# zouyunkai/MedicalSemSeg

Measured on AMD Instinct MI355X. Metric: 96^3 vols/sec fwd+bwd (train), higher is better.
Workload: dtype bf16; 1 GPU; UNet base (MONAI BasicUNet 32-32-64-128-256-32) 1->3cls, 96^3 patches, DiceCE + AdamW, per-GPU batch 2; global_batch=2, parallelism=dp1, grad_sync=none (single rank)

## Files before the change

### include/msseg.h

```cpp
#ifndef MSSEG_H_
#define MSSEG_H_

#include <stddef.h>
#include <stdint.h>

#ifdef __cplusplus
extern "C" {
#endif

#define MSSEG_ABI_VERSION 1

#define MSSEG_OK 0
#define MSSEG_EINVAL (-1)
#define MSSEG_ELAUNCH (-2)
#define MSSEG_EWORKSPACE (-3)

#define MSSEG_F32 0
#define MSSEG_BF16 1

typedef void* msseg_stream_t;

int msseg_abi_version(void);
const char* msseg_last_error(void);
int msseg_num_cus(void);

int msseg_ktimer_enable(int on);
int msseg_ktimer_reset(void);
int msseg_ktimer_count(void);
int msseg_ktimer_get(int i, char* name, int cap, float* ms);

size_t msseg_packed_weight_bytes(int M, int T, int K, int cout_block, int dtype);
int msseg_pack_weights(const float* src, void* dst, int dtype, int M, int M0, int T, int K, int K0,
                       long long s_m1, long long s_m0, long long s_t, long long s_k1, long long s_k0,
                       int flip, int cout_block, msseg_stream_t stream);
typedef struct msseg_pack_job {
    const float* src;
    void* dst;
    long long s_m1, s_m0, s_t, s_k1, s_k0;
    long long total;
    int M, M0, T, K, K0, flip, cout_block, nkb;
} msseg_pack_job;
int msseg_pack_weights_batch(const msseg_pack_job* jobs_dev, int njobs, long long max_total, long long sum_total, int dtype,
                             msseg_stream_t stream);
int msseg_cout_block(int M);
int msseg_conv3d_k3_cout_block(int N, int D, int H, int W, int Cout);
int msseg_conv3d_k3_variant(int N, int D, int H, int W, int Cout);
int msseg_conv3d_k3_kernel(int N, int D, int H, int W, int Cin, int Cout, int dtype);

int msseg_conv3d_k3_fwd(const void* x, long long ldx, const void* wp, const float* bias, void* y, long long ldy,
                        int N, int D, int H, int W, int Cin, int Cout, float* stats ,
                        void* scratch, size_t scratch_bytes, int dtype, msseg_stream_t stream);
int msseg_conv3d_k3_fwd_accumulate(const void* x, long long ldx, const void* wp, void* y, long long ldy, int N, int D, int H,
                                   int W, int Cin, int Cout, float* stats, void* scratch, size_t scratch_bytes, int dtype,
                                   msseg_stream_t stream);
int msseg_conv3d_k3_dgrad_inbwd(const void* dy, long long lddy, const void* wp, void* da, long long ldda, int N, int D,
                                int H, int W, int Cin, int Cout, const void* yraw, long long ldyraw, const void* act,
                                long long ldact, const float* fwd_stats, float slope, float eps, float* red,
                                float* dgamma, float* dbeta, int accumulate, void* scratch, size_t scratch_bytes,
                                int dtype, msseg_stream_t stream);
int msseg_conv3d_k3s2_fwd(const void* x, long long ldx, const void* wp, const float* bias, void* y, long long ldy,
                          int N, int ID, int IH, int IW, int Cin, int Cout, int dtype, msseg_stream_t stream);
int msseg_zero_stuff2(const void* dy, long long lddy, void* out, long long ldo, int N, int OD, int OH, int OW, int ID,
                      int IH, int IW, int C, int dtype, msseg_stream_t stream);
int msseg_conv3d_stem_fwd(const void* x, long long ldx, const void* wp, const float* bias, void* y, long long ldy,
                          int N, int D, int H, int W, int Cout, float* stats, void* scratch, size_t scratch_bytes,
                          int dtype, msseg_stream_t stream);
int msseg_conv3d_stem_k1_fwd(const void* x, long long ldx, const void* wp, const float* bias, void* y, long long ldy,
                             int N, int D, int H, int W, int Cout, float* stats, void* scratch, size_t scratch_bytes,
                             int dtype, msseg_stream_t stream);
int msseg_conv3d_stem_norm_fwd(const void* x, long long ldx, const void* wp, const float* bias, const float* stats,
                               const float* gamma, const float* beta, float eps, float slope, void* y, long long ldy, int N,
                               int D, int H, int W, int Cout, int dtype, msseg_stream_t stream);
int msseg_conv3d_k1_fwd(const void* x, long long ldx, const void* wp, const float* bias, void* y, long long ldy,
                        long long NV, int Cin, int Cout, int dtype, msseg_stream_t stream);
int msseg_conv3d_k1_head_fwd(const void* x, long long ldx, const float* w, const float* bias, void* y, long long ldy,
                             long long NV, int Cin, int Cout, int dtype, msseg_stream_t stream);
int msseg_conv3d_k1_head_dgrad_inbwd(const void* dy, long long lddy, const float* w, void* da, long long ldda, int N,
                                     long long S, int C, int Cout, const void* yraw, long long ldyraw,
                                     const float* fwd_stats, const float* gamma, const float* beta, float slope, float eps,
                                     float* red, float* dgamma, float* dbeta, int accumulate, void* scratch,
                                     size_t scratch_bytes, int dtype, msseg_stream_t stream);
int msseg_conv3d_k1_head_norm_fwd(const void* x, long long ldx, const float* stats, const float* gamma, const float* beta,
                                  float slope, float eps, const float* w, const float* bias, void* y, long long ldy, int N,
                                  long long S, int Cin, int Cout, int dtype, msseg_stream_t stream);
int msseg_conv3d_k1_head_bwd_fused(const void* dy, long long lddy, const float* w, void* da, long long ldda, int N,
                                   long long S, int C, int Cout, const void* yraw, long long ldyraw, const float* fwd_stats,
                                   const float* gamma, const float* beta, float slope, float eps, float* red, float* dgamma,
                                   float* dbeta, int accumulate, float* dw, int dw_accumulate, void* scratch,
                                   size_t scratch_bytes, int dtype, msseg_stream_t stream);

int msseg_conv3d_gather_fwd(const void* x, long long ldx, const void* wp, const float* bias, void* y, long long ldy,
                            int N, int ID, int IH, int IW, int Cin, int Cout, int k, int s, int p, int dtype,
                            msseg_stream_t stream);
int msseg_deconv_k2s2_fwd(const void* x, long long ldx, const void* wp, const float* bias, void* y, long long ldy,
                          int N, int D, int H, int W, int Cin, int Cout, int dtype, msseg_stream_t stream);
int msseg_deconv_k2s2_bwd_data(const void* dy, long long lddy, const void* wp, void* dx, long long lddx,
                               int N, int D, int H, int W, int Cin, int Cout, int dtype, msseg_stream_t stream);
int msseg_deconv_k4s4_fwd(const void* x, long long ldx, const void* wp, const float* bias, void* y, long long ldy,
                          int N, int D, int H, int W, int Cin, int Cout, int dtype, msseg_stream_t stream);
int msseg_deconv_k4s4_bwd_data(const void* dy, long long lddy, const void* wp, void* dx, long long lddx,
                               int N, int D, int H, int W, int Cin, int Cout, int dtype, msseg_stream_t stream);
int msseg_conv3d_k1_dgrad_inbwd(const void* dy, long long lddy, const void* wp, void* da, long long ldda, int N,
                                long long S, int Cin, int Cout, const void* yraw, long long ldyraw, const void* act,
                                long long ldact, const float* fwd_stats, float slope, float eps, float* red,
                                float* dgamma, float* dbeta, int accumulate, void* scratch, size_t scratch_bytes,
                                int dtype, msseg_stream_t stream);
int msseg_deconv_k2s2_bwd_data_inbwd(const void* dy, long long lddy, const void* wp, void* dx, long long lddx, int N,
                                     int D, int H, int W, int Cin, int Cout, const void* yraw, long long ldyraw,
                                     const void* act, long long ldact, const float* fwd_stats, float slope, float eps,
                                     float* red, float* dgamma, float* dbeta, int accumulate, void* scratch,
                                     size_t scratch_bytes, int dtype, msseg_stream_t stream);
int msseg_deconv_k2s2_bwd_fused(const void* dy, long long lddy, const void* wp, void* dx, long long lddx, int N,
                                int D, int H, int W, int Cin, int Cout, const void* yraw, long long ldyraw,
                                const void* act, long long ldact, const float* fwd_stats, float slope, float eps,
                                float* red, float* dgamma, float* dbeta, int accumulate, float* dbias, int dbias_accumulate,
                                void* scratch, size_t scratch_bytes, int dtype, msseg_stream_t stream);

int msseg_deconv_k2s2_bwd_partials_ok(int Cin, int Cout, int dtype);
int msseg_deconv_k2s2_bwd_partials(const void* dy, long long lddy, const void* wp, float* part, size_t part_bytes, int N,
                                   int D, int H, int W, int Cin, int Cout, int dtype, msseg_stream_t stream);


size_t msseg_wgrad_workspace_bytes(int M, int T, int K);
int msseg_conv3d_k3_wgrad_kernel(int N, int D, int H, int W, int Cin, int Cout, int dtype);
int msseg_conv3d_k3_wgrad(const void* x, long long ldx, const void* dy, long long lddy, float* dw,
                          int N, int D, int H, int W, int Cin, int Cout, int accumulate,
                          void* workspace, size_t workspace_bytes, int dtype, msseg_stream_t stream);
int msseg_conv3d_k1_wgrad(const void* x, long long ldx, const void* dy, long long lddy, float* dw,
                          long long NV, int Cin, int Cout, int accumulate,
                          void* workspace, size_t workspace_bytes, int dtype, msseg_stream_t stream);
int msseg_linear_wgrad_ok(long long NV, int Cin, int Cout, int dtype);
int msseg_linear_wgrad(const void* x, long long ldx, const void* dy, long long lddy, float* dw, float* dbias, long long NV,
                       int Cin, int Cout, int accumulate_w, int accumulate_b, void* workspace, size_t workspace_bytes,
                       int dtype, msseg_stream_t stream);
int msseg_conv3d_gather_wgrad(const void* x, long long ldx, const void* dy, long long lddy, float* dw,
                              int N, int ID, int IH, int IW, int Cin, int Cout, int k, int s, int p, int accumulate,
                              void* workspace, size_t workspace_bytes, int dtype, msseg_stream_t stream);
int msseg_deconv_k2s2_wgrad(const void* x, long long ldx, const void* dy, long long lddy, float* dw,
                            int N, int D, int H, int W, int Cin, int Cout, int accumulate,
                            void* workspace, size_t workspace_bytes, int dtype, msseg_stream_t stream);
int msseg_deconv_k4s4_wgrad(const void* x, long long ldx, const void* dy, long long lddy, float* dw,
                            int N, int D, int H, int W, int Cin, int Cout, int accumulate,
                            void* workspace, size_t workspace_bytes, int dtype, msseg_stream_t stream);

int msseg_conv3d_k3_small_ok(int N, int D, int H, int W, int Cin, int Cout, int dtype);
int msseg_conv3d_k3_small_stage_groups(int N, int D, int H, int W, int Cin, int Cout);
size_t msseg_conv3d_k3_small_workspace_bytes(int N, int D, int H, int W, int Cin, int Cout);
int msseg_conv3d_k3_small_partials(const void* x, long long ldx, const void* wp, float* part, size_t part_bytes, int N,
                                   int D, int H, int W, int Cin, int Cout, msseg_stream_t stream);
int msseg_conv3d_k3_small_fwd_finish(const float* part, int nstages, const float* bias, const float* gamma,
                                     const float* beta, float eps, float slope, void* yraw, long long ldy, void* act,
                                     long long lda, void* pooled, long long ldp, float* stats, int N, int D, int H, int W,
                                     int Cout, msseg_stream_t stream);
int msseg_conv3d_k3_small_fwd_finish_res(const float* part, int nstages, const float* bias, const float* gamma,
                                         const float* beta, float eps, float slope, void* yraw, long long ldy, void* act,
                                         long long lda, const void* residual, long long ldr, void* pooled, long long ldp,
                                         float* stats, int N, int D, int H, int W, int Cout, msseg_stream_t stream);
int msseg_conv3d_k3_small_bwd_finish(const float* part, int nstages, void* dx, long long lddx, const void* unit_yraw,
                                     long long lduy, const float* unit_stats, const float* unit_gamma,
                                     const float* unit_beta, float eps, float slope, float* dgamma, float* dbeta,
                                     int accumulate, int N, int D, int H, int W, int Cin, msseg_stream_t stream);

int msseg_dwconv3d_k3_fwd(const void* x, long long ldx, const void* w_taps, const float* bias, void* y, long long ldy, int N,
                          int D, int H, int W, int C, int flip, int dtype, msseg_stream_t stream);
int msseg_avgpool3d_k3(const void* x, long long ldx, void* y, long long ldy, int N, int D, int H, int W, int C, int dtype,
                       msseg_stream_t stream);
int msseg_dwconv3d_k3_wgrad(const void* x, long long ldx, const void* dy, long long lddy, float* dw, float* dbias,
                            int accumulate_w, int accumulate_b, int N, int D, int H, int W, int C, void* scratch,
                            size_t scratch_bytes, int dtype, msseg_stream_t stream);

int msseg_interp_trilinear_fwd(const void* x, long long ldx, void* y, long long ldy, int N, int ID, int IH, int IW, int OD,
                               int OH, int OW, int C, int dtype, msseg_stream_t stream);
size_t msseg_interp_trilinear_bwd_workspace_bytes(int N, int ID, int IH, int IW, int OD, int OH, int OW, int C);
int msseg_interp_trilinear_bwd(const void* dy, long long lddy, void* dx, long long lddx, int N, int ID, int IH, int IW, int OD,
                               int OH, int OW, int C, void* workspace, size_t workspace_bytes, int dtype, msseg_stream_t stream);
int msseg_kv_attention_fwd(const void* q, const void* kv, void* o, float* lse, int B, int N, int M, int heads, int head_dim,
                           float scale, int dtype, msseg_stream_t stream);
size_t msseg_kv_attention_bwd_workspace_bytes(int B, int N, int M, int heads, int head_dim);
int msseg_kv_attention_bwd(const void* q, const void* kv, const void* o, const float* lse, const void* dout, void* dq, void* dkv,
                           int B, int N, int M, int heads, int head_dim, float scale, void* workspace, size_t workspace_bytes,
                           int dtype, msseg_stream_t stream);
int msseg_scale_channels(const void* x, const float* scale, void* y, int N, long long S, int C, int dtype, msseg_stream_t stream);

size_t msseg_reduce_scratch_bytes(void);
int msseg_channel_stats(const void* x, long long ldx, float* stats, int N, long long S, int C, void* scratch,
                        size_t scratch_bytes, int dtype, msseg_stream_t stream);
int msseg_instnorm_act_fwd(const void* x, long long ldx, const float* stats, const float* gamma, const float* beta,
                           const void* residual, long long ldr, void* y, long long ldy, int N, long long S, int C,
                           float eps, float slope, int dtype, msseg_stream_t stream);
int msseg_instnorm_act_pool_fwd(const void* x, long long ldx, const float* stats, const float* gamma, const float* beta,
                                void* y, long long ldy, void* pooled, long long ldp, int N, int D, int H, int W, int C,
                                float eps, float slope, int dtype, msseg_stream_t stream);
int msseg_instnorm_act_poolbwd_reduce(const void* x, long long ldx, const float* stats, const float* gamma,
                                      const float* beta, const void* skip, long long lds, const void* g, long long ldg,
                                      void* da, long long ldda, float* red, float* dgamma, float* dbeta, int accumulate,
                                      int N, int D, int H, int W, int C, float eps, float slope, void* scratch,
                                      size_t scratch_bytes, int dtype, msseg_stream_t stream);
int msseg_instnorm_act_bwd_reduce(const void* x, long long ldx, const float* stats, const float* gamma,
                                  const float* beta, const void* y, long long ldy,
                                  const void* dy, long long lddy, float* red, float* dgamma, float* dbeta,
                                  int accumulate, int N, long long S, int C, float eps, float slope, void* scratch,
                                  size_t scratch_bytes, int dtype, msseg_stream_t stream);
int msseg_instnorm_act_bwd_apply(const void* x, long long ldx, const float* stats, const float* gamma,
                                 const float* beta, const void* y, long long ldy, const void* dy, long long lddy, const float* red, void* dx,
                                 long long lddx, void* dres, long long lddres, int N, long long S, int C, float eps,
                                 float slope, int dtype, msseg_stream_t stream);
int msseg_maxpool2_fwd(const void* x, long long ldx, void* y, long long ldy, int N, int D, int H, int W, int C,
                       int dtype, msseg_stream_t stream);
int msseg_maxpool2_bwd(const void* x, long long ldx, const void* dy, long long lddy, void* dx, long long lddx,
                       int N, int D, int H, int W, int C, int accumulate, int dtype, msseg_stream_t stream);
int msseg_ncdhw_to_ndhwc(const void* src, int src_dtype, void* dst, long long ldd, int dst_dtype, int N, int C,
                         long long S, msseg_stream_t stream);
int msseg_ndhwc_to_ncdhw(const void* src, long long lds, int src_dtype, void* dst, int dst_dtype, int N, int C,
                         long long S, msseg_stream_t stream);
int msseg_channel_sum(const void* x, long long ldx, float* out, long long rows, int C, int accumulate, void* scratch,
                      size_t scratch_bytes, int dtype, msseg_stream_t stream);
int msseg_add(const void* a, long long lda, const void* b, long long ldb, void* y, long long ldy, long long rows,
              int C, int dtype, msseg_stream_t stream);
int msseg_axpy_rows(const void* a, const void* b, const float* scale, void* y, int N, long long elems_per_sample, int dtype,
                    msseg_stream_t stream);


int msseg_window_attention_fwd(const void* qkv, const float* qkv_bias, const float* table, void* out, float* lse, int B,
                               int S, int H, int W, int C, int heads, int ws, int shift, int dtype,
                               msseg_stream_t stream);
int msseg_window_attention_bwd(const void* qkv, const float* qkv_bias, const float* table, const void* out,
                               const float* lse, const void* dout, void* dqkv, float* dtable, int B, int S, int H, int W,
                               int C, int heads, int ws, int shift, int dtype, msseg_stream_t stream);
size_t msseg_window_attention_bwd_workspace_bytes(int B, int S, int H, int W, int C, int heads, int ws, int shift, int dtype);
int msseg_window_attention_fwd2(const void* qkv, const float* qkv_bias, const float* table, void* out, float* lse, int B,
                                int S, int H, int W, int C, int heads, int ws, int shift, int bias_ws, int dtype,
                                msseg_stream_t stream);
int msseg_window_attention_bwd2(const void* qkv, const float* qkv_bias, const float* table, const void* out,
                                const float* lse, const void* dout, void* dqkv, float* dtable, int B, int S, int H, int W,
                                int C, int heads, int ws, int shift, int bias_ws, int dtype, void* workspace,
                                size_t workspace_bytes, msseg_stream_t stream);
int msseg_window_attention_bwd_ws(const void* qkv, const float* qkv_bias, const float* table, const void* out,
                                  const float* lse, const void* dout, void* dqkv, float* dtable, int B, int S, int H, int W,
                                  int C, int heads, int ws, int shift, int dtype, void* workspace, size_t workspace_bytes,
                                  msseg_stream_t stream);
int msseg_window_attention_fwd3(const void* qkv, const float* qkv_bias, const float* table, void* out, float* lse, int B,
                                int S, int H, int W, int C, int heads, int ws, int shift, int bias_ws, long long table_stride,
                                int dtype, msseg_stream_t stream);
int msseg_window_attention_bwd3(const void* qkv, const float* qkv_bias, const float* table, const void* out,
                                const float* lse, const void* dout, void* dqkv, float* dtable, int B, int S, int H, int W,
                                int C, int heads, int ws, int shift, int bias_ws, long long table_stride, int dtype,
                                void* workspace, size_t workspace_bytes, msseg_stream_t stream);
size_t msseg_window_attention_bwd3_workspace_bytes(int B, int S, int H, int W, int C, int heads, int ws, int shift,
                                                   int bias_ws, long long table_stride, int dtype);
int msseg_rel_bias_affine_fold(const float* table, const float* emb, const float* lin_w, const float* lin_b,
                               const float* aff, float* T, int B, int M3, int heads, msseg_stream_t stream);
size_t msseg_rel_bias_affine_grad_workspace_bytes(int M3, int heads);
#define MSSEG_AFFINE_ACC_TABLE 1
#define MSSEG_AFFINE_ACC_EMB 2
#define MSSEG_AFFINE_ACC_LIN_W 4
#define MSSEG_AFFINE_ACC_LIN_B 8
int msseg_rel_bias_affine_grad(const float* dT, const float* emb, const float* lin_w, const float* aff, float* dtable,
                               float* demb, float* dlin_w, float* dlin_b, int B, int M3, int heads, int flags,
                               void* workspace, size_t workspace_bytes, msseg_stream_t stream);
int msseg_layernorm_fwd(const void* x, long long ldx, const float* gamma, const float* beta, void* y, long long ldy,
                        float* mean, float* rstd, long long rows, int C, float eps, int dtype, msseg_stream_t stream);
int msseg_layernorm_bwd(const void* x, long long ldx, const float* gamma, const float* mean, const float* rstd,
                        const void* dy, long long lddy, void* dx, long long lddx, long long rows, int C, int dtype,
                        msseg_stream_t stream);
int msseg_layernorm_bwd_add(const void* x, long long ldx, const float* gamma, const float* mean, const float* rstd,
                            const void* dy, long long lddy, const void* add, long long ldadd, void* dx, long long lddx,
                            long long rows, int C, int dtype, msseg_stream_t stream);
int msseg_layernorm_param_grad(const void* x, long long ldx, const float* mean, const float* rstd, const void* dy,
                               long long lddy, float* dgamma, float* dbeta, int accumulate, long long rows, int C,
                               void* scratch, size_t scratch_bytes, int dtype, msseg_stream_t stream);
int msseg_gelu_fwd(const void* x, void* y, long long n, int dtype, msseg_stream_t stream);
int msseg_gelu_bwd(const void* x, const void* dy, void* dx, long long n, int dtype, msseg_stream_t stream);
int msseg_linear_gelu_ok(long long NV, int Cin, int Cout, int dtype);
int msseg_linear_gelu_fwd(const void* x, long long ldx, const void* wp, const float* bias, void* pre, long long ldpre, void* act,
                          long long ldact, long long NV, int Cin, int Cout, int dtype, msseg_stream_t stream);
int msseg_linear_gelu_bwd(const void* dy, long long lddy, const void* wp, const void* pre, long long ldpre, void* dpre,
                          long long lddpre, long long NV, int Cin, int Cout, int dtype, msseg_stream_t stream);
int msseg_linear_add_ok(long long NV, int Cin, int Cout, int dtype);
int msseg_linear_add_fwd(const void* x, long long ldx, const void* wp, const float* bias, const void* res, long long ldres,
                         void* y, long long ldy, long long NV, int Cin, int Cout, int dtype, msseg_stream_t stream);
// ... 74 lines not shown
```

### medicalsemseg_amd/csrc/conv3d_k3_wgrad_pp.hip

```cpp
#include "k3pp.h"

#include <stdlib.h>

#include <type_traits>

namespace {

constexpr int TD = 4, TH = 4, TW = 16;
constexpr int PD = TD + 2, PH = TH + 2, PW = TW + 2;
constexpr int PWP = PW;
constexpr int HV = PD * PH * PWP;
constexpr int TV = TD * TH * TW;
constexpr int Q_BYTES = HV * 64;
constexpr int P_BYTES = TV * 64;
constexpr int GRP_BYTES = Q_BYTES + P_BYTES;
constexpr int NIQ = (HV + 15) / 16;
constexpr int NIP = TV / 16;
constexpr int NIQ_W = (NIQ + 3) / 4, NIP_W = NIP / 4;
constexpr int NKS = TV / 16;
constexpr int TAPW = 7;
constexpr int NTHREADS = 512;
constexpr int SLAB_FLOATS = 27 * 32 * 32;

__device__ u32x4_t g_wg_zero_chunk;
__device__ unsigned long long g_k3wg_cycles[8];

MSSEG_DEVFN void glds16(const void* g, void* l) {
    __builtin_amdgcn_global_load_lds((const __attribute__((address_space(1))) void*)g,
                                     (__attribute__((address_space(3))) void*)l, 16, 0, 0);
}

typedef __attribute__((address_space(3))) unsigned char lds_u8;
typedef __attribute__((ext_vector_type(16))) float f32x16_t;

MSSEG_DEVFN bf16x4_t lds_tr(lds_u8* p) {
    return __builtin_amdgcn_ds_read_tr16_b64_v4bf16((__attribute__((address_space(3))) bf16x4_t*)p);
}

MSSEG_DEVFN u32x4_t tr_frag(lds_u8* r0, lds_u8* r1) {
    const bf16x4_t lo = lds_tr(r0), hi = lds_tr(r1);
    const bf16x8_t f = {lo[0], lo[1], lo[2], lo[3], hi[0], hi[1], hi[2], hi[3]};
    return __builtin_bit_cast(u32x4_t, f);
}

struct TileCo { int n, d0, h0, w0; };

constexpr int ks_row(int ks) { return ((ks / TH) * PH + ks % TH) * PWP; }

template <int TIMING>
__global__ __launch_bounds__(NTHREADS, 1) void k3wg_pp_kernel(const K3WgParams p) {
    extern __shared__ __attribute__((aligned(256))) unsigned char smem[];
    const int tid = threadIdx.x, lane = tid & 63;
    const int wave = __builtin_amdgcn_readfirstlane(tid >> 6);
    const int grp = wave >> 2, wq = wave & 3;
    lds_u8* smem3 = (lds_u8*)smem;
    unsigned char* ldsQ = smem + grp * GRP_BYTES;
    unsigned char* ldsP = ldsQ + Q_BYTES;
    const int mblk = blockIdx.y / p.kblks, kblk = blockIdx.y % p.kblks;
    const unsigned char* pg = (const unsigned char*)p.pten + mblk * 64;
    const unsigned char* qg = (const unsigned char*)p.qten + kblk * 64;

    const int tiles_w = (p.W + TW - 1) / TW, tiles_h = (p.H + TH - 1) / TH, tiles_d = (p.D + TD - 1) / TD;
    const int ntiles = p.N * tiles_d * tiles_h * tiles_w;
    int t_first, t_step, t_end;
    if ((gridDim.x & 7) == 0) {
        const int chunk = (ntiles + 7) >> 3, xcd = blockIdx.x & 7;
        t_first = xcd * chunk + (blockIdx.x >> 3);
        t_step = gridDim.x >> 3;
        t_end = min(ntiles, (xcd + 1) * chunk);
    } else {
        t_first = blockIdx.x; t_step = gridDim.x; t_end = ntiles;
    }
    const int n_my = t_first < t_end ? (t_end - t_first + t_step - 1) / t_step : 0;
    auto tile_of = [&](int k) {
        int t = t_first + k * t_step;
        TileCo tc;
        tc.w0 = (t % tiles_w) * TW; t /= tiles_w;
        tc.h0 = (t % tiles_h) * TH; t /= tiles_h;
        tc.d0 = (t % tiles_d) * TD; t /= tiles_d;
        tc.n = t;
        return tc;
    };

    const int lrow = lane >> 2;
    const int lchunk = lane & 3;
    constexpr unsigned SKIP = 0xffffffffu;
    unsigned q_off[NIQ_W], p_off[NIP_W];
#pragma unroll
    for (int j = 0; j < NIQ_W; ++j) {
        const int hv = (wq + 4 * j) * 16 + lrow;
        const int hd = hv / (PH * PWP), rem = hv - hd * (PH * PWP), hh = rem / PWP, hw = rem - hh * PWP;
        q_off[j] = (hv < HV && hw < PW) ? (unsigned)((((long long)hd * p.H + hh) * p.W + hw) * p.ldq * 2 + lchunk * 16) : SKIP;
    }
#pragma unroll
    for (int j = 0; j < NIP_W; ++j) {
        const int tv = (wq + 4 * j) * 16 + lrow;
        const int td = tv / (TH * TW), th = (tv / TW) % TH, tw = tv % TW;
        p_off[j] = (unsigned)((((long long)td * p.H + th) * p.W + tw) * p.ldp * 2 + lchunk * 16);
    }
    const bool p_cok = mblk * 32 + lchunk * 8 < p.M, q_cok = kblk * 32 + lchunk * 8 < p.K;
    const bool chunks_full = (mblk + 1) * 32 <= p.M && (kblk + 1) * 32 <= p.K;
    auto load_tile = [&](const TileCo& tc) {
        const int dB = tc.d0 - 1, hB = tc.h0 - 1, wB = tc.w0 - 1;
        const long long qvox = (((long long)tc.n * p.D + dB) * p.H + hB) * p.W + wB;
        const long long pvox = (((long long)tc.n * p.D + tc.d0) * p.H + tc.h0) * p.W + tc.w0;
        const unsigned char* qb = qg + qvox * p.ldq * 2;
        const unsigned char* pb = pg + pvox * p.ldp * 2;
        const bool interior = chunks_full && dB >= 0 && dB + PD <= p.D && hB >= 0 && hB + PH <= p.H && wB >= 0 && wB + PW <= p.W;
        if (interior) {
#pragma unroll
            for (int j = 0; j < NIQ_W; ++j) {
                if (q_off[j] != SKIP) glds16(qb + q_off[j], ldsQ + (wq + 4 * j) * 1024);
            }
#pragma unroll
            for (int j = 0; j < NIP_W; ++j) glds16(pb + p_off[j], ldsP + (wq + 4 * j) * 1024);
        } else {
            const unsigned char* zsrc = (const unsigned char*)&g_wg_zero_chunk;
#pragma unroll
            for (int j = 0; j < NIQ_W; ++j) {
                const int it = wq + 4 * j;
                const int hv = it * 16 + lrow;
                const int hd = hv / (PH * PWP), rem = hv - hd * (PH * PWP), hh = rem / PWP, hw = rem - hh * PWP;
                const bool inb = q_cok && (unsigned)(dB + hd) < (unsigned)p.D && (unsigned)(hB + hh) < (unsigned)p.H &&
                                 (unsigned)(wB + hw) < (unsigned)p.W;
                const unsigned char* src = inb ? qb + q_off[j] : zsrc;
                if (q_off[j] != SKIP) glds16(src, ldsQ + it * 1024);
            }
#pragma unroll
            for (int j = 0; j < NIP_W; ++j) {
                const int tv = (wq + 4 * j) * 16 + lrow;
                const int td = tv / (TH * TW), th = (tv / TW) % TH, tw = tv % TW;
                const bool inb = p_cok && tc.d0 + td < p.D && tc.h0 + th < p.H && tc.w0 + tw < p.W;
                const unsigned char* src = inb ? pb + p_off[j] : zsrc;
                glds16(src, ldsP + (wq + 4 * j) * 1024);
            }
        }
    };

    const int G = lane >> 4, qr = (lane >> 2) & 3, pc = lane & 3;
    const unsigned qbase = grp * GRP_BYTES, pbase = qbase + Q_BYTES;
    unsigned p_rd[2], q_rd[TAPW][2];
#pragma unroll
    for (int i = 0; i < 2; ++i) {
        const int lrow = 8 * (G >> 1) + 4 * i + qr;
        p_rd[i] = pbase + lrow * 64 + ((G & 1) << 5) + pc * 8;
#pragma unroll
        for (int tt = 0; tt < TAPW; ++tt) {
            int tap = wq * TAPW + tt;
            if (tap > 26) tap = 26;
            const int row = ((tap / 9) * PH + ((tap / 3) % 3)) * PWP + (tap % 3) + lrow;
            q_rd[tt][i] = qbase + row * 64 + ((G & 1) << 5) + pc * 8;
        }
    }

    f32x16_t acc[TAPW];
#pragma unroll
    for (int t = 0; t < TAPW; ++t)
#pragma unroll
        for (int e = 0; e < 16; ++e) acc[t][e] = 0.f;

    auto compute = [&]() {
        constexpr int NSTEP = NKS * TAPW;
        constexpr int QA = 2;
        u32x4_t pf[2], qf[QA + 1];
        auto ldp = [&](int ks) { pf[ks & 1] = tr_frag(smem3 + p_rd[0] + ks * 1024, smem3 + p_rd[1] + ks * 1024); };
        auto ldq = [&](int s) {
            const int ks = s / TAPW, tt = s % TAPW;
            qf[s % (QA + 1)] = tr_frag(smem3 + q_rd[tt][0] + ks_row(ks) * 64, smem3 + q_rd[tt][1] + ks_row(ks) * 64);
        };
        ldp(0);
#pragma unroll
        for (int s = 0; s < QA; ++s) ldq(s);
#pragma unroll
        for (int ks = 0; ks < NKS; ++ks) {
#pragma unroll
            for (int tt = 0; tt < TAPW; ++tt) {
                const int s = ks * TAPW + tt;
                if (s + QA < NSTEP) ldq(s + QA);
                if (tt == 0 && ks + 1 < NKS) ldp(ks + 1);
                __builtin_amdgcn_sched_barrier(0);
                acc[tt] = __builtin_amdgcn_mfma_f32_32x32x16_bf16(__builtin_bit_cast(bf16x8_t, pf[ks & 1]),
                                                                  __builtin_bit_cast(bf16x8_t, qf[s % (QA + 1)]),
                                                                  acc[tt], 0, 0, 0);
                __builtin_amdgcn_sched_barrier(0);
            }
        }
    };

    if (grp == 0 && n_my > 0) load_tile(tile_of(0));
    asm volatile("s_waitcnt vmcnt(0)" ::: "memory");
    __syncthreads();

    unsigned long long tcyc[4] = {0, 0, 0, 0};
    for (int ph = 0; ph < n_my; ++ph) {
        unsigned long long t0 = 0;
        if constexpr (TIMING) t0 = __builtin_readcyclecounter();
        if ((ph & 1) == grp) {
            compute();
            if constexpr (TIMING) tcyc[0] += __builtin_readcyclecounter() - t0;
        } else {
            if (ph + 1 < n_my && !(TIMING && p.dbg_noload)) load_tile(tile_of(ph + 1));
            if constexpr (TIMING) tcyc[1] += __builtin_readcyclecounter() - t0;
        }
        if constexpr (TIMING) t0 = __builtin_readcyclecounter();
        asm volatile("s_waitcnt vmcnt(0)" ::: "memory");
        if constexpr (TIMING) { tcyc[2] += __builtin_readcyclecounter() - t0; t0 = __builtin_readcyclecounter(); }
        __syncthreads();
        if constexpr (TIMING) tcyc[3] += __builtin_readcyclecounter() - t0;
    }
    if constexpr (TIMING) {
        if (blockIdx.x == 0 && blockIdx.y == 0 && lane == 0 && wave == 0) {
#pragma unroll
            for (int k = 0; k < 4; ++k) g_k3wg_cycles[k] = tcyc[k];
        }
    }

    float* xch = (float*)smem;
    const int col = lane & 31, rb = 4 * (lane >> 5);
    const int tap0 = wq * TAPW;
    if (grp == 1) {
#pragma unroll
        for (int tt = 0; tt < TAPW; ++tt) {
            if (tap0 + tt < 27) {
#pragma unroll
                for (int e = 0; e < 16; ++e)
                    xch[((tap0 + tt) * 32 + (e & 3) + 8 * (e >> 2) + rb) * 32 + col] = acc[tt][e];
            }
        }
    }
    __syncthreads();
    if (grp == 0) {
        float* slab = p.slabs + ((long long)blockIdx.y * gridDim.x + blockIdx.x) * SLAB_FLOATS;
#pragma unroll
        for (int tt = 0; tt < TAPW; ++tt) {
            if (tap0 + tt < 27) {
#pragma unroll
                for (int e = 0; e < 16; ++e) {
                    const int idx = ((tap0 + tt) * 32 + (e & 3) + 8 * (e >> 2) + rb) * 32 + col;
                    slab[idx] = acc[tt][e] + xch[idx];
                }
            }
        }
    }
}

}

bool msseg_k3wg_pp_eligible(const K3WgParams& p) {
    static const bool off = getenv("MSSEG_NO_K3PP") != nullptr;
    if (off) return false;
    if (p.M % 8 || p.K % 8) return false;
    if ((p.ldp % 8) || (p.ldq % 8) || ((uintptr_t)p.pten & 15) || ((uintptr_t)p.qten & 15)) return false;
    const long long ldm = p.ldp > p.ldq ? p.ldp : p.ldq;
    if ((long long)(PD + 1) * p.H * p.W * ldm * 2 >= 0x7fffffffLL) return false;
    const long long tiles = (long long)p.N * ceil_div(p.D, TD) * ceil_div(p.H, TH) * ceil_div(p.W, TW);
    if (tiles > 0x7fffffffLL) return false;
    return tiles * ceil_div(p.M, 32) * ceil_div(p.K, 32) >= 2LL * msseg_num_cus();
}

int msseg_k3wg_pp_grid(const K3WgParams& p) {
    const int pairs = ceil_div(p.M, 32) * ceil_div(p.K, 32);
    const int tiles = p.N * ceil_div(p.D, TD) * ceil_div(p.H, TH) * ceil_div(p.W, TW);
    int gx = msseg_num_cus() / pairs;
    gx &= ~7;
    if (gx < 8) gx = 8;
    if (gx > tiles) gx = tiles;
    return gx;
}

int msseg_k3wg_pp_launch(const K3WgParams& p, int gx, hipStream_t stream) {
    static const bool timing = getenv("MSSEG_K3PP_TIMING") != nullptr;
    static const bool noload = getenv("MSSEG_K3PP_NOLOAD") != nullptr;
    K3WgParams pl = p;
    pl.dbg_noload = noload ? 1 : 0;
    const int lds = 2 * GRP_BYTES;
    static msseg_lds_attr_once attr[2];
    if (!attr[0].ensure((const void*)k3wg_pp_kernel<0>, lds) || !attr[1].ensure((const void*)k3wg_pp_kernel<1>, lds))
        MSSEG_FAIL(MSSEG_ELAUNCH, "conv3d_k3_wgrad_pp: cannot set dynamic LDS size %d", lds);
    const int pairs = ceil_div(p.M, 32) * ceil_div(p.K, 32);
    if (timing) hipLaunchKernelGGL(k3wg_pp_kernel<1>, dim3(gx, pairs, 1), dim3(NTHREADS), lds, stream, pl);
    else MSSEG_KTIMED("k3wg_pp_kernel", stream, hipLaunchKernelGGL(k3wg_pp_kernel<0>, dim3(gx, pairs, 1), dim3(NTHREADS), lds, stream, pl));
    MSSEG_CHECK_LAUNCH("conv3d_k3_wgrad_pp");
    return MSSEG_OK;
}

extern "C" int msseg_debug_k3wg_cycles(unsigned long long* out4) {
    return hipMemcpyFromSymbol(out4, HIP_SYMBOL(g_k3wg_cycles), 4 * sizeof(unsigned long long)) == hipSuccess ? 0 : -1;
}
```

### medicalsemseg_amd/csrc/elementwise.hip

```cpp
#include "common.h"

#include <stdarg.h>
#include <string.h>

static thread_local char g_err[512] = "";
void msseg_set_error(const char* fmt, ...) {
    va_list ap;
    va_start(ap, fmt);
    vsnprintf(g_err, sizeof(g_err), fmt, ap);
    va_end(ap);
}

extern "C" {
int msseg_abi_version(void) { return MSSEG_ABI_VERSION; }
const char* msseg_last_error(void) { return g_err; }
int msseg_num_cus(void) {
    static int cus = 0;
    if (cus == 0) {
        int dev = 0;
        hipDeviceProp_t prop;
        if (hipGetDevice(&dev) == hipSuccess && hipGetDeviceProperties(&prop, dev) == hipSuccess)
            cus = prop.multiProcessorCount;
        if (cus <= 0) cus = 256;
    }
    return cus;
}
}

namespace {

template <typename T> struct Chunk {
    static constexpr int EPC = DT<T>::EPC;
    float v[EPC];
    MSSEG_DEVFN void load(const T* p) {
        if constexpr (sizeof(T) == 4) {
            f32x4_t t = *(const f32x4_t*)p;
#pragma unroll
            for (int e = 0; e < 4; ++e) v[e] = t[e];
        } else {
            bf16x8_t t = *(const bf16x8_t*)p;
#pragma unroll
            for (int e = 0; e < 8; ++e) v[e] = (float)t[e];
        }
    }
    MSSEG_DEVFN void store(T* p) const {
        if constexpr (sizeof(T) == 4) {
            f32x4_t t = {v[0], v[1], v[2], v[3]};
            *(f32x4_t*)p = t;
        } else {
            bf16x8_t t;
#pragma unroll
            for (int e = 0; e < 8; ++e) t[e] = (bf16_t)v[e];
            *(bf16x8_t*)p = t;
        }
    }
};

inline bool vec_ok(const void* p, long long ld, int C, int esz) {
    const int epc = 16 / esz;
    return (C % epc) == 0 && (ld % epc) == 0 && (((uintptr_t)p) & 15) == 0;
}

struct RowMap {
    int groups;
    int rows_par;
};
inline RowMap row_map(int C, int width, int nthr = 256) {
    RowMap m;
    m.groups = ceil_div(C, width);
    if (m.groups > nthr) m.groups = nthr;
    m.rows_par = nthr / m.groups;
    if (m.rows_par < 1) m.rows_par = 1;
    return m;
}

MSSEG_DEVFN void finalize_channels(const float* ws, int N, int nblk, int C, int nper, int mode, float* out,
                                   float* dp0, float* dp1, int accumulate) {
    __shared__ float fin[256];
    const int L = C * nper;
    const int cols = L < 256 ? L : 256;
    const int G = 256 / cols;
    const int col = threadIdx.x % cols, rg = threadIdx.x / cols;
    const bool in256 = threadIdx.x < 256;
    const int n_step = mode == 0 ? (int)gridDim.y : 1, n_first = mode == 0 ? (int)blockIdx.y : 0;
    for (int c0 = blockIdx.x * cols; c0 < L; c0 += gridDim.x * cols) {
        const int o = c0 + col;
        const bool ok = in256 && o < L && rg < G;
        float tot = 0.f;
        for (int n = n_first; n < N; n += n_step) {
            float s = 0.f;
            if (ok) {
                const float* src = ws + (long long)n * nblk * L + o;
#pragma unroll 16
                for (int bb = rg; bb < nblk; bb += G) s += src[(long long)bb * L];
            }
            __syncthreads();
            if (in256) fin[threadIdx.x] = s;
            __syncthreads();
            if (ok && rg == 0) {
                float t = 0.f;
                for (int g = 0; g < G; ++g) t += fin[g * cols + col];
                if (mode != 1) out[(long long)n * L + o] = t;
                tot += t;
            }
        }
        if (ok && rg == 0) {
            if (mode == 1) {
                out[o] = accumulate ? out[o] + tot : tot;
            } else if (mode == 2) {
                const int c = o / nper, k = o % nper;
                float* dp = (k == 0) ? dp0 : dp1;
                if (dp) dp[c] = accumulate ? dp[c] + tot : tot;
            }
        }
    }
}

struct FinalizeArgs {
    const float* ws; int N, nblk, C, nper, mode; float* out; float* dp0; float* dp1; int accumulate;
};
__global__ __launch_bounds__(256) void channels_finalize_kernel(const FinalizeArgs a) {
    finalize_channels(a.ws, a.N, a.nblk, a.C, a.nper, a.mode, a.out, a.dp0, a.dp1, a.accumulate);
}

static inline dim3 channels_finalize_grid(const FinalizeArgs& a) {
    const int L = a.C * a.nper;
    int gx = (L + 255) / 256;
    if (gx > 64) gx = 64;
    if (gx < 1) gx = 1;
    return dim3((unsigned)gx, a.mode == 0 ? (unsigned)(a.N < 1 ? 1 : a.N) : 1u);
}

constexpr int RED_THREADS = 512;
constexpr int RED_STAGE2 = 16;

template <int W>
MSSEG_DEVFN void block_rows_reduce(float* red, int groups, int rows_par, int g, int rl, bool act) {
    if (act && rl < RED_STAGE2 && rl < rows_par) {
#pragma unroll
        for (int e = 0; e < W; ++e) {
            float a = 0.f, b = 0.f;
            for (int k = rl; k < rows_par; k += RED_STAGE2) {
                a += red[((k * groups + g) * W + e) * 2 + 0];
                b += red[((k * groups + g) * W + e) * 2 + 1];
            }
            red[((rl * groups + g) * W + e) * 2 + 0] = a;
            red[((rl * groups + g) * W + e) * 2 + 1] = b;
        }
    }
    __syncthreads();
}

template <typename T, bool VEC>
// ... 44 lines not shown
#pragma unroll
            for (int e = 0; e < W; ++e) {
                float a = 0.f, b = 0.f;
                for (int k = 0; k < kmax; ++k) {
                    a += red[((k * groups + g) * W + e) * 2 + 0];
                    b += red[((k * groups + g) * W + e) * 2 + 1];
                }
                const int c = gg * W + e;
                wsb[c * nacc + 0] = a;
                if (nacc == 2) wsb[c * nacc + 1] = b;
            }
        }
    }
}

template <typename T, bool VEC>
__global__ __launch_bounds__(256) void ln_param_grad_kernel(const T* __restrict__ x, long long ldx,
                                                            const T* __restrict__ dy, long long lddy,
                                                            const float* __restrict__ mean, const float* __restrict__ rstd,
                                                            long long rows, int C, int groups, int rows_par,
                                                            long long rows_per_block, float* ws, unsigned int* counter,
                                                            float* dgamma, float* dbeta, int accumulate) {
    constexpr int W = VEC ? DT<T>::EPC : 1;
    __shared__ float red[256 * 2 * (VEC ? DT<T>::EPC : 1)];
    __shared__ int lflag;
    const int g = threadIdx.x % groups, rl = threadIdx.x / groups;
    const long long r0 = (long long)blockIdx.x * rows_per_block;
    long long r1 = r0 + rows_per_block;
    if (r1 > rows) r1 = rows;
    float* wsb = ws + (long long)blockIdx.x * C * 2;
    for (int gbase = 0; gbase * W < C; gbase += groups) {
        const int gg = gbase + g;
        const bool act = gg * W < C;
        float s[W], s2[W];
#pragma unroll
        for (int e = 0; e < W; ++e) s[e] = s2[e] = 0.f;
        if (act && rl < rows_par) {
#pragma unroll 4
            for (long long r = r0 + rl; r < r1; r += rows_par) {
                const float mu = mean[r], rs = rstd[r];
                if constexpr (VEC) {
                    Chunk<T> cx, cd;
                    cx.load(x + r * ldx + gg * W);
                    cd.load(dy + r * lddy + gg * W);
#pragma unroll
                    for (int e = 0; e < W; ++e) { s[e] += cd.v[e] * (cx.v[e] - mu) * rs; s2[e] += cd.v[e]; }
                } else {
                    const float d = DT<T>::ld(dy + r * lddy + gg);
                    s[0] += d * (DT<T>::ld(x + r * ldx + gg) - mu) * rs;
                    s2[0] += d;
                }
            }
        }
        __syncthreads();
#pragma unroll
        for (int e = 0; e < W; ++e) {
            red[(threadIdx.x * W + e) * 2 + 0] = s[e];
            red[(threadIdx.x * W + e) * 2 + 1] = s2[e];
        }
        __syncthreads();
        if (act && rl == 0) {
#pragma unroll
            for (int e = 0; e < W; ++e) {
                float a = 0.f, b = 0.f;
                for (int k = 0; k < rows_par; ++k) {
                    a += red[((k * groups + g) * W + e) * 2 + 0];
                    b += red[((k * groups + g) * W + e) * 2 + 1];
                }
                wsb[(gg * W + e) * 2 + 0] = a;
                wsb[(gg * W + e) * 2 + 1] = b;
            }
        }
    }
}

inline long long reduce_blocks(long long S, int rows_par, int N, int C, int nper);

template <typename T>
int launch_ln_param_grad(const void* x, long long ldx, const void* dy, long long lddy, const float* mean, const float* rstd,
                         float* dgamma, float* dbeta, int accumulate, long long rows, int C, void* scratch, hipStream_t st) {
    const bool vec = vec_ok(x, ldx, C, sizeof(T)) && vec_ok(dy, lddy, C, sizeof(T));
    const RowMap m = row_map(C, vec ? DT<T>::EPC : 1);
    long long blocks = reduce_blocks(rows, m.rows_par, 1, C, 2);
    const long long rpb = ceil_div_ll(rows, blocks);
    blocks = ceil_div_ll(rows, rpb);
    unsigned int* counter = (unsigned int*)scratch;
    float* ws = (float*)((unsigned char*)scratch + MSSEG_SCRATCH_COUNTER_BYTES);
    if (vec)
        hipLaunchKernelGGL((ln_param_grad_kernel<T, true>), dim3((unsigned)blocks), dim3(256), 0, st, (const T*)x, ldx,
                           (const T*)dy, lddy, mean, rstd, rows, C, m.groups, m.rows_par, rpb, ws, counter, dgamma, dbeta, accumulate);
    else
        hipLaunchKernelGGL((ln_param_grad_kernel<T, false>), dim3((unsigned)blocks), dim3(256), 0, st, (const T*)x, ldx,
                           (const T*)dy, lddy, mean, rstd, rows, C, m.groups, m.rows_par, rpb, ws, counter, dgamma, dbeta, accumulate);
    MSSEG_CHECK_LAUNCH("ln_param_grad");
    {
        FinalizeArgs a{ws, 1, (int)blocks, C, 2, 2, ws + blocks * C * 2, dgamma, dbeta, accumulate};
        hipLaunchKernelGGL(channels_finalize_kernel, channels_finalize_grid(a), dim3(256), 0, st, a);
        MSSEG_CHECK_LAUNCH("channels_finalize");
    }
    return MSSEG_OK;
}

inline long long reduce_blocks(long long S, int rows_par, int N, int C, int nper) {
    long long blocks = ceil_div_ll(S, (long long)rows_par * 8);
    long long cap = (long long)msseg_num_cus() / (N > 0 ? N : 1);
    if (cap < 1) cap = 1;
    const long long fit = (long long)(((size_t)16 << 20) / ((size_t)N * C * nper * 4));
    if (cap > fit) cap = fit;
    if (blocks > cap) blocks = cap;
    if (blocks < 1) blocks = 1;
    return blocks;
}

template <typename T>
int launch_stats(const void* x, long long ldx, float* out, int N, long long S, int C, int nacc, int accumulate,
                 void* scratch, hipStream_t st) {
    const bool vec = vec_ok(x, ldx, C, sizeof(T));
    const RowMap m = row_map(C, vec ? DT<T>::EPC : 1, RED_THREADS);
    long long blocks = reduce_blocks(S, m.rows_par, N, C, nacc);
    const long long rpb = ceil_div_ll(S, blocks);
    blocks = ceil_div_ll(S, rpb);
    dim3 grid((unsigned)blocks, N);
    unsigned int* counter = (unsigned int*)scratch;
    float* ws = (float*)((unsigned char*)scratch + MSSEG_SCRATCH_COUNTER_BYTES);
    if (vec)
        hipLaunchKernelGGL((channel_stats_kernel<T, true>), grid, dim3(RED_THREADS), 0, st, (const T*)x, ldx, out, S, C,
                           m.groups, m.rows_par, rpb, nacc, accumulate, ws, counter);
    else
        hipLaunchKernelGGL((channel_stats_kernel<T, false>), grid, dim3(RED_THREADS), 0, st, (const T*)x, ldx, out, S, C,
                           m.groups, m.rows_par, rpb, nacc, accumulate, ws, counter);
    MSSEG_CHECK_LAUNCH("channel_stats");
    {
        FinalizeArgs a{ws, N, (int)blocks, C, nacc, nacc == 2 ? 0 : 1, out, nullptr, nullptr, accumulate};
        hipLaunchKernelGGL(channels_finalize_kernel, channels_finalize_grid(a), dim3(256), 0, st, a);
        MSSEG_CHECK_LAUNCH("channels_finalize");
    }
    return MSSEG_OK;
}

struct NormParams {
    const void* x; long long ldx;
    const float* stats; const float* gamma; const float* beta;
    const void* res; long long ldr;
    void* y; long long ldy;
    const void* dy; long long lddy;
    float* red;
    void* dx; long long lddx;
    void* dres; long long lddres;
    long long S; int C; float eps, slope;
    long long rows_per_block; int groups, rows_par;
    float* ws; unsigned int* counter; float* dgamma; float* dbeta; int accumulate;
};

MSSEG_DEVFN void mean_rstd(const float* stats, int n, int C, int c, long long S, float eps, float& mean, float& rstd) {
    const float inv = 1.0f / (float)S;
    const float s = stats[((long long)n * C + c) * 2 + 0], s2 = stats[((long long)n * C + c) * 2 + 1];
    mean = s * inv;
    float var = s2 * inv - mean * mean;
    var = var > 0.f ? var : 0.f;
    rstd = rsqrtf(var + eps);
}

template <typename T, bool VEC, int MODE>
__global__ __launch_bounds__(MODE == 1 ? RED_THREADS : 256) void instnorm_kernel(const NormParams p) {
    constexpr int W = VEC ? DT<T>::EPC : 1;
    __shared__ float red[(MODE == 1) ? RED_THREADS * 2 * W : 1];
    __shared__ int lflag;
    const int n = blockIdx.y;
    const int g = threadIdx.x % p.groups, rl = threadIdx.x / p.groups;
    const long long r0 = (long long)blockIdx.x * p.rows_per_block;
    long long r1 = r0 + p.rows_per_block;
    if (r1 > p.S) r1 = p.S;
    const T* xn = (const T*)p.x + (long long)n * p.S * p.ldx;
    const T* yn = (MODE != 0 && p.y != nullptr) ? (const T*)p.y + (long long)n * p.S * p.ldy : nullptr;
    T* yo = (MODE == 0) ? (T*)p.y + (long long)n * p.S * p.ldy : nullptr;
    const T* dyn = (MODE != 0) ? (const T*)p.dy + (long long)n * p.S * p.lddy : nullptr;
    const T* resn = (MODE == 0 && p.res) ? (const T*)p.res + (long long)n * p.S * p.ldr : nullptr;
    T* dxn = (MODE == 2) ? (T*)p.dx + (long long)n * p.S * p.lddx : nullptr;
    T* drn = (MODE == 2 && p.dres) ? (T*)p.dres + (long long)n * p.S * p.lddres : nullptr;
    const float invS = 1.0f / (float)p.S;

    for (int gbase = 0; gbase * W < p.C; gbase += p.groups) {
        const int gg = gbase + g;
        const bool act = gg * W < p.C;
        float mean[W], rstd[W], sc[W], sh[W], k0[W], k1[W], a0[W], a1[W];
#pragma unroll
        for (int e = 0; e < W; ++e) {
            const int c = act ? gg * W + e : 0;
            mean_rstd(p.stats, n, p.C, c, p.S, p.eps, mean[e], rstd[e]);
            const float ga = p.gamma ? p.gamma[c] : 1.f;
            sc[e] = rstd[e] * ga;
            sh[e] = (p.beta ? p.beta[c] : 0.f) - mean[e] * sc[e];
            a0[e] = a1[e] = 0.f;
            if constexpr (MODE == 2) {
                k0[e] = p.red[((long long)n * p.C + c) * 2 + 0] * invS;
                k1[e] = p.red[((long long)n * p.C + c) * 2 + 1] * invS;
            }
        }
        if (act && rl < p.rows_par) {
#pragma unroll 4
            for (long long r = r0 + rl; r < r1; r += p.rows_par) {
                float xv[W], o[W], yv[W], dv[W];
                if constexpr (VEC) {
                    Chunk<T> c; c.load(xn + r * p.ldx + gg * W);
#pragma unroll
                    for (int e = 0; e < W; ++e) xv[e] = c.v[e];
                } else {
                    xv[0] = DT<T>::ld(xn + r * p.ldx + gg);
                }
                if constexpr (MODE == 0) {
                    float rv[W];
#pragma unroll
                    for (int e = 0; e < W; ++e) rv[e] = 0.f;
                    if (resn) {
                        if constexpr (VEC) {
                            Chunk<T> c; c.load(resn + r * p.ldr + gg * W);
#pragma unroll
                            for (int e = 0; e < W; ++e) rv[e] = c.v[e];
                        } else {
                            rv[0] = DT<T>::ld(resn + r * p.ldr + gg);
                        }
                    }
#pragma unroll
                    for (int e = 0; e < W; ++e) {
                        const float z = xv[e] * sc[e] + sh[e] + rv[e];
                        o[e] = z > 0.f ? z : z * p.slope;
                    }
                    if constexpr (VEC) {
                        Chunk<T> c;
#pragma unroll
                        for (int e = 0; e < W; ++e) c.v[e] = o[e];
                        c.store(yo + r * p.ldy + gg * W);
                    } else {
                        DT<T>::st(yo + r * p.ldy + gg, o[0]);
                    }
                } else {
                    if constexpr (VEC) {
                        Chunk<T> d; d.load(dyn + r * p.lddy + gg * W);
#pragma unroll
                        for (int e = 0; e < W; ++e) dv[e] = d.v[e];
                        if (yn != nullptr) {
                            Chunk<T> c; c.load(yn + r * p.ldy + gg * W);
#pragma unroll
                            for (int e = 0; e < W; ++e) yv[e] = c.v[e];
                        } else {
#pragma unroll
                            for (int e = 0; e < W; ++e) yv[e] = xv[e] * sc[e] + sh[e];
                        }
                    } else {
                        dv[0] = DT<T>::ld(dyn + r * p.lddy + gg);
                        yv[0] = (yn != nullptr) ? DT<T>::ld(yn + r * p.ldy + gg) : xv[0] * sc[0] + sh[0];
                    }
#pragma unroll
                    for (int e = 0; e < W; ++e) {
                        const float dz = yv[e] > 0.f ? dv[e] : dv[e] * p.slope;
                        const float xh = (xv[e] - mean[e]) * rstd[e];
                        if constexpr (MODE == 1) {
                            a0[e] += dz;
                            a1[e] += dz * xh;
                        } else {
                            o[e] = sc[e] * (dz - k0[e] - xh * k1[e]);
                            dv[e] = dz;
                        }
                    }
                    if constexpr (MODE == 2) {
                        if constexpr (VEC) {
                            Chunk<T> c;
#pragma unroll
                            for (int e = 0; e < W; ++e) c.v[e] = o[e];
                            c.store(dxn + r * p.lddx + gg * W);
                            if (drn) {
#pragma unroll
                                for (int e = 0; e < W; ++e) c.v[e] = dv[e];
                                c.store(drn + r * p.lddres + gg * W);
                            }
                        } else {
                            DT<T>::st(dxn + r * p.lddx + gg, o[0]);
                            if (drn) DT<T>::st(drn + r * p.lddres + gg, dv[0]);
                        }
                    }
                }
            }
        }
        if constexpr (MODE == 1) {
            __syncthreads();
#pragma unroll
            for (int e = 0; e < W; ++e) {
                red[(threadIdx.x * W + e) * 2 + 0] = a0[e];
                red[(threadIdx.x * W + e) * 2 + 1] = a1[e];
            }
            __syncthreads();
            block_rows_reduce<W>(red, p.groups, p.rows_par, g, rl, act);
            if (act && rl == 0) {
                const int kmax = p.rows_par < RED_STAGE2 ? p.rows_par : RED_STAGE2;
#pragma unroll
                for (int e = 0; e < W; ++e) {
                    float a = 0.f, b = 0.f;
                    for (int k = 0; k < kmax; ++k) {
                        a += red[((k * p.groups + g) * W + e) * 2 + 0];
                        b += red[((k * p.groups + g) * W + e) * 2 + 1];
                    }
                    const int c = gg * W + e;
                    float* wsb = p.ws + ((long long)n * gridDim.x + blockIdx.x) * p.C * 2;
                    wsb[c * 2 + 0] = a;
                    wsb[c * 2 + 1] = b;
                }
            }
        }
    }
}

struct NormPoolParams {
    const void* x; long long ldx;
    const float* stats; const float* gamma; const float* beta;
    void* y; long long ldy;
    void* pooled; long long ldp;
    int N, D, H, W, C; float eps, slope;
};

template <typename T>
__global__ __launch_bounds__(256) void instnorm_pool_fwd_kernel(const NormPoolParams p) {
    constexpr int WD = DT<T>::EPC;
    const int OD = p.D / 2, OH = p.H / 2, OW = p.W / 2;
    const unsigned ug = (unsigned)(p.C / WD);
    const unsigned total = (unsigned)((long long)p.N * OD * OH * OW * ug);
    const long long S = (long long)p.D * p.H * p.W;
    for (unsigned i = blockIdx.x * 256u + threadIdx.x; i < total; i += gridDim.x * 256u) {
        unsigned t = i / ug;
        const int g = (int)(i - t * ug);
        unsigned t2 = t / (unsigned)OW;
        const int ow = (int)(t - t2 * (unsigned)OW);
        t = t2 / (unsigned)OH;
        const int oh = (int)(t2 - t * (unsigned)OH);
        const int n = (int)(t / (unsigned)OD);
        const int od = (int)(t - (unsigned)n * (unsigned)OD);
        float sc[WD], sh[WD], best[WD];
#pragma unroll
        for (int e = 0; e < WD; ++e) {
            const int c = g * WD + e;
            float mean, rstd;
            mean_rstd(p.stats, n, p.C, c, S, p.eps, mean, rstd);
            sc[e] = rstd * (p.gamma ? p.gamma[c] : 1.f);
            sh[e] = (p.beta ? p.beta[c] : 0.f) - mean * sc[e];
            best[e] = -INFINITY;
        }
        Chunk<T> in[8];
#pragma unroll
        for (int k = 0; k < 8; ++k) {
            const long long vox = (((long long)n * p.D + 2 * od + (k >> 2)) * p.H + 2 * oh + ((k >> 1) & 1)) * p.W + 2 * ow + (k & 1);
            in[k].load((const T*)p.x + vox * p.ldx + g * WD);
        }
#pragma unroll
        for (int k = 0; k < 8; ++k) {
            const long long vox = (((long long)n * p.D + 2 * od + (k >> 2)) * p.H + 2 * oh + ((k >> 1) & 1)) * p.W + 2 * ow + (k & 1);
            Chunk<T> o;
#pragma unroll
            for (int e = 0; e < WD; ++e) {
                const float z = in[k].v[e] * sc[e] + sh[e];
                const float a = (float)(T)(z > 0.f ? z : z * p.slope);
                o.v[e] = a;
                if (a > best[e] || a != a) best[e] = a;
            }
            o.store((T*)p.y + vox * p.ldy + g * WD);
        }
        Chunk<T> b;
#pragma unroll
        for (int e = 0; e < WD; ++e) b.v[e] = best[e];
        const long long ovox = (((long long)n * OD + od) * OH + oh) * OW + ow;
        b.store((T*)p.pooled + ovox * p.ldp + g * WD);
    }
}

struct NormPoolBwdParams {
    const void* x; long long ldx;
    const float* stats; const float* gamma; const float* beta;
    const void* skip; long long lds;
    const void* g; long long ldg;
    void* da; long long ldda;
    int N, D, H, W, C; float eps, slope;
    int groups, rows_par; long long cells_per_block;
    float* ws;
};

template <typename T>
__global__ __launch_bounds__(RED_THREADS) void instnorm_poolbwd_reduce_kernel(const NormPoolBwdParams p) {
    constexpr int WD = DT<T>::EPC;
    __shared__ float red[RED_THREADS * 2 * WD];
    const int n = blockIdx.y;
    const int g = threadIdx.x % p.groups, rl = threadIdx.x / p.groups;
    const int OD = p.D / 2, OH = p.H / 2, OW = p.W / 2;
    const long long cells = (long long)OD * OH * OW, S = (long long)p.D * p.H * p.W;
    const long long c0 = (long long)blockIdx.x * p.cells_per_block;
    long long c1 = c0 + p.cells_per_block;
    if (c1 > cells) c1 = cells;
    const T* xn = (const T*)p.x + (long long)n * S * p.ldx;
    const T* sn = (const T*)p.skip + (long long)n * S * p.lds;
    const T* gn = (const T*)p.g + (long long)n * cells * p.ldg;
    T* dn = (T*)p.da + (long long)n * S * p.ldda;
    for (int gbase = 0; gbase * WD < p.C; gbase += p.groups) {
        const int gg = gbase + g;
        const bool act = gg * WD < p.C;
        float mean[WD], rstd[WD], sc[WD], sh[WD], a0[WD], a1[WD];
#pragma unroll
        for (int e = 0; e < WD; ++e) {
            const int c = act ? gg * WD + e : 0;
            mean_rstd(p.stats, n, p.C, c, S, p.eps, mean[e], rstd[e]);
            sc[e] = rstd[e] * (p.gamma ? p.gamma[c] : 1.f);
            sh[e] = (p.beta ? p.beta[c] : 0.f) - mean[e] * sc[e];
            a0[e] = a1[e] = 0.f;
        }
        if (act && rl < p.rows_par) {
            for (long long cell = c0 + rl; cell < c1; cell += p.rows_par) {
                const int ow = (int)(cell % OW), oh = (int)((cell / OW) % OH), od = (int)(cell / ((long long)OW * OH));
                Chunk<T> xin[8], gv;
// ... 1082 lines not shown
```

### medicalsemseg_amd/csrc/igemm_wgrad.hip

```cpp
#include "common.h"
#include "k3pp.h"

#include <stdlib.h>

namespace {

enum { Q_DIRECT = 0, Q_GATHER = 1, Q_DECONV = 2 };

struct WgradParams {
    const void* pten;
    long long ldp;
    const void* qten;
    long long ldq;
    float* slabs;
    int N, D, H, W;
    int ID, IH, IW;
    int OD, OH, OW;
    int M, K;
    int mblks, kblks;
    int tiles_d, tiles_h, tiles_w, ntiles;
    int cin, k, s, p;
    int creal;
    int rel32_ok;
};
// ... 407 lines not shown
    const int nk = min(32, p.K - kb * 32);
    float* dst = p.dw + (long long)m * p.s_m0 + (long long)kb * 32 * T;
    for (int o = threadIdx.x; o < nk * T; o += 256) {
        const int k = o / T, t = o - k * T;
        dst[o] = p.accumulate ? dst[o] + tile[t][k] : tile[t][k];
    }
}

int launch_reduce(const ReduceParams& rp, hipStream_t stream) {
    const long long total = (long long)rp.M * rp.T * rp.K;
    if (total >= 0x7fffffffLL) MSSEG_FAIL(MSSEG_EINVAL, "wgrad: weight tensor too large");
    const bool conv_layout = rp.s_t == 1 && rp.s_k0 == rp.T && rp.K0 == rp.K && rp.M0 == rp.M && rp.T > 1 && rp.T <= 32 &&
                             rp.s_m0 == (long long)rp.K * rp.T && (rp.cbw == 32 || rp.cbw == 16);
    static const bool no_rows = getenv("MSSEG_NO_REDUCE_ROWS") != nullptr;
    if (rp.nslots <= 32 && conv_layout && !no_rows && ceil_div(rp.K, 32) <= 65535) {
        hipLaunchKernelGGL(wgrad_reduce_rows_kernel, dim3(rp.M, ceil_div(rp.K, 32)), dim3(256), 0, stream, rp);
    } else if (rp.nslots <= 32) {
        int rb = (int)((total + 255) / 256);
        if (rb > 8192) rb = 8192;
        hipLaunchKernelGGL(wgrad_reduce_small_kernel, dim3(rb), dim3(256), 0, stream, rp);
    } else {
        int rb = (int)((total + 31) / 32);
        if (rb > 4096) rb = 4096;
        hipLaunchKernelGGL(wgrad_reduce_kernel, dim3(rb), dim3(256), 0, stream, rp);
    }
    MSSEG_CHECK_LAUNCH("wgrad_reduce");
    return MSSEG_OK;
}

template <typename T, int NTAPS, int QSRC, int TD, int TH, int TW>
int launch_wg(WgradParams& p, ReduceParams& rp, void* workspace, size_t ws_bytes, hipStream_t stream) {
    using C = WgCfg<T, NTAPS, TD, TH, TW>;
    p.tiles_d = ceil_div(p.D, TD);
    p.tiles_h = ceil_div(p.H, TH);
    p.tiles_w = ceil_div(p.W, TW);
    const long long nt = (long long)p.N * p.tiles_d * p.tiles_h * p.tiles_w;
    if (nt > 0x7fffffffLL) MSSEG_FAIL(MSSEG_EINVAL, "wgrad: too many tiles");
    p.ntiles = (int)nt;
    p.mblks = ceil_div(p.M, C::CBW);
    p.kblks = ceil_div(p.K, C::CBW);
    {
        const long long ldm = p.ldp > p.ldq ? p.ldp : p.ldq;
        p.rel32_ok = ((long long)(C::PD + 1) * p.H * p.W * ldm < 0x7fffffffLL) ? 1 : 0;
    }
    const int pairs = p.mblks * p.kblks;
    const int wave_slots = 1;
    const size_t slab_bytes = (size_t)C::SLAB_FLOATS * 4;
    long long gx = msseg_num_cus() * ((C::LDS_BYTES > 80 * 1024) ? 1 : 2);
    static const int flat_per_cu = getenv("MSSEG_WG_FLAT_PER_CU") ? atoi(getenv("MSSEG_WG_FLAT_PER_CU")) : 3;
    if (NTAPS == 1 && C::LDS_BYTES * flat_per_cu <= 160 * 1024) gx = (long long)msseg_num_cus() * flat_per_cu;
    static const int wgs_env = getenv("MSSEG_WG_TOTAL") ? atoi(getenv("MSSEG_WG_TOTAL")) : 0;
    if (NTAPS == 27 && (long long)p.ntiles * pairs <= 4LL * msseg_num_cus()) gx = wgs_env > 0 ? wgs_env : msseg_num_cus() / 2;
    if (pairs > 1) gx = (gx + pairs - 1) / pairs;
    if (gx > p.ntiles) gx = p.ntiles;
    const long long fit = (long long)(ws_bytes / (slab_bytes * pairs * wave_slots));
    if (fit < 1) MSSEG_FAIL(MSSEG_EWORKSPACE, "wgrad: workspace %zu B too small (need >= %zu)", ws_bytes,
                            slab_bytes * pairs * wave_slots);
    if (gx > fit) gx = fit;
    if (gx < 1) gx = 1;
    p.slabs = (float*)workspace;
    auto kern = igemm_wgrad_kernel<T, NTAPS, QSRC, TD, TH, TW>;
    static msseg_lds_attr_once attr;
    if (!attr.ensure((const void*)kern, C::LDS_BYTES)) MSSEG_FAIL(MSSEG_ELAUNCH, "wgrad: cannot set dynamic LDS size %d", C::LDS_BYTES);
    MSSEG_KTIMED(NTAPS == 27 ? "igemm_wgrad_kernel<27>" : "igemm_wgrad_kernel<flat>", stream,
                 hipLaunchKernelGGL(kern, dim3((unsigned)gx, pairs, 1), dim3(256), C::LDS_BYTES, stream, p));
    MSSEG_CHECK_LAUNCH("igemm_wgrad");
    rp.slabs = p.slabs;
    rp.mblks = p.mblks; rp.kblks = p.kblks; rp.nslots = (int)gx * wave_slots; rp.cbw = C::CBW;
    return launch_reduce(rp, stream);
}

template <typename T> int launch_wg_k3(WgradParams& p, ReduceParams& rp, void* ws, size_t wsb, hipStream_t st) {
    if constexpr (sizeof(T) == 2) {
        K3WgParams pp{};
        pp.pten = p.pten; pp.ldp = p.ldp; pp.qten = p.qten; pp.ldq = p.ldq;
        pp.N = p.N; pp.D = p.D; pp.H = p.H; pp.W = p.W; pp.M = p.M; pp.K = p.K; pp.kblks = ceil_div(p.K, 32);
        static const int pp_min_dim = getenv("MSSEG_K3WG_MINDIM") ? atoi(getenv("MSSEG_K3WG_MINDIM")) : 8;
        const int mnd = p.D < p.H ? (p.D < p.W ? p.D : p.W) : (p.H < p.W ? p.H : p.W);
        if (mnd >= pp_min_dim && msseg_k3wg_pp_eligible(pp)) {
            const int pairs = ceil_div(p.M, 32) * ceil_div(p.K, 32);
            int gx = msseg_k3wg_pp_grid(pp);
            const long long fit = (long long)(wsb / ((size_t)27 * 32 * 32 * 4 * pairs));
            if (fit >= 8) {
                if (gx > fit) gx = (int)(fit & ~7LL);
                pp.slabs = (float*)ws;
                const int rc = msseg_k3wg_pp_launch(pp, gx, st);
                if (rc) return rc;
                rp.slabs = pp.slabs;
                rp.mblks = ceil_div(p.M, 32); rp.kblks = ceil_div(p.K, 32); rp.nslots = gx; rp.cbw = 32;
                return launch_reduce(rp, st);
            }
        }
    }
    const int mn = p.D < p.H ? (p.D < p.W ? p.D : p.W) : (p.H < p.W ? p.H : p.W);
    if (mn >= 32) {
        static const bool two_wg = getenv("MSSEG_WGRAD_2WG") != nullptr;
        if (two_wg) return launch_wg<T, 27, Q_DIRECT, 2, 8, 16>(p, rp, ws, wsb, st);
        return launch_wg<T, 27, Q_DIRECT, 4, 8, 16>(p, rp, ws, wsb, st);
    }
    if (mn >= 12) return launch_wg<T, 27, Q_DIRECT, 4, 4, 8>(p, rp, ws, wsb, st);
    return launch_wg<T, 27, Q_DIRECT, 2, 4, 8>(p, rp, ws, wsb, st);
}

int wg_check(const void* a, long long lda, const void* b, long long ldb, const void* dw, const void* ws, int dtype) {
    if (!a || !b || !dw || !ws) MSSEG_FAIL(MSSEG_EINVAL, "wgrad: null pointer");
    if (dtype != MSSEG_F32 && dtype != MSSEG_BF16) MSSEG_FAIL(MSSEG_EINVAL, "wgrad: bad dtype");
    const int esz = dtype == MSSEG_F32 ? 4 : 2;
    if ((((uintptr_t)a | (uintptr_t)b | (uintptr_t)ws) & 15) || (lda * esz) % 16 || (ldb * esz) % 16)
        MSSEG_FAIL(MSSEG_EINVAL, "wgrad: operands must be 16-byte aligned with 16-byte row strides");
    return MSSEG_OK;
}

}

bool msseg_lwg_deconv_ok(int dtype, long long NV, int Cin, int Cout, const void* x, long long ldx, const void* dy, long long lddy);
int msseg_lwg_deconv_wgrad(const void* x, long long ldx, const void* dy, long long lddy, float* dw, int N, int D, int H, int W,
                           int Cin, int Cout, int accumulate, void* workspace, size_t workspace_bytes, hipStream_t stream);

extern "C" {

size_t msseg_wgrad_workspace_bytes(int M, int T, int K) {
    const size_t padM = (size_t)((M + 31) / 32) * 32, padK = (size_t)((K + 31) / 32) * 32;
    const size_t per_slot = padM * padK * (size_t)T * 4;
    size_t slots = 256;
    while (slots > 8 && per_slot * slots * (T == 1 ? 4 : 1) > ((size_t)256 << 20)) slots /= 2;
    return per_slot * slots * (T == 1 ? 4 : 1);
}

int msseg_conv3d_k3_wgrad_kernel(int N, int D, int H, int W, int Cin, int Cout, int dtype) {
    if (dtype != MSSEG_BF16) return 0;
    K3WgParams pp{};
    pp.pten = (const void*)256; pp.ldp = Cout; pp.qten = (const void*)256; pp.ldq = Cin;
    pp.N = N; pp.D = D; pp.H = H; pp.W = W; pp.M = Cout; pp.K = Cin; pp.kblks = ceil_div(Cin, 32);
    return msseg_k3wg_pp_eligible(pp) ? 3 : 0;
}

int msseg_conv3d_k3_wgrad(const void* x, long long ldx, const void* dy, long long lddy, float* dw, int N, int D, int H,
                          int W, int Cin, int Cout, int accumulate, void* workspace, size_t workspace_bytes, int dtype,
                          msseg_stream_t stream) {
    int rc = wg_check(x, ldx, dy, lddy, dw, workspace, dtype);
    if (rc) return rc;
    const int esz = dtype == MSSEG_F32 ? 4 : 2;
    if (Cin % (16 / esz)) MSSEG_FAIL(MSSEG_EINVAL, "conv3d_k3_wgrad: Cin %% %d != 0", 16 / esz);
    WgradParams p{};
    p.pten = dy; p.ldp = lddy; p.qten = x; p.ldq = ldx;
    p.N = N; p.D = D; p.H = H; p.W = W; p.M = Cout; p.K = Cin;
    ReduceParams rp{};
    rp.dw = dw; rp.M = Cout; rp.M0 = Cout; rp.T = 27; rp.K = Cin; rp.K0 = Cin;
    rp.s_m1 = 0; rp.s_m0 = (long long)Cin * 27; rp.s_t = 1; rp.s_k1 = 0; rp.s_k0 = 27; rp.accumulate = accumulate;
    return dtype == MSSEG_F32 ? launch_wg_k3<float>(p, rp, workspace, workspace_bytes, (hipStream_t)stream)
                              : launch_wg_k3<bf16_t>(p, rp, workspace, workspace_bytes, (hipStream_t)stream);
}

int msseg_conv3d_k1_wgrad(const void* x, long long ldx, const void* dy, long long lddy, float* dw, long long NV, int Cin,
                          int Cout, int accumulate, void* workspace, size_t workspace_bytes, int dtype,
                          msseg_stream_t stream) {
    int rc = wg_check(x, ldx, dy, lddy, dw, workspace, dtype);
    if (rc) return rc;
    const int esz = dtype == MSSEG_F32 ? 4 : 2;
    if (Cin % (16 / esz) || NV < 1 || NV > 0x7fffffffLL) MSSEG_FAIL(MSSEG_EINVAL, "conv3d_k1_wgrad: bad shape");
    WgradParams p{};
    p.pten = dy; p.ldp = lddy; p.qten = x; p.ldq = ldx;
    p.N = 1; p.D = 1; p.H = 1; p.W = (int)NV; p.M = Cout; p.K = Cin;
    ReduceParams rp{};
    rp.dw = dw; rp.M = Cout; rp.M0 = Cout; rp.T = 1; rp.K = Cin; rp.K0 = Cin;
    rp.s_m0 = Cin; rp.s_k0 = 1; rp.accumulate = accumulate;
    return dtype == MSSEG_F32
               ? launch_wg<float, 1, Q_DIRECT, 1, 1, 256>(p, rp, workspace, workspace_bytes, (hipStream_t)stream)
               : launch_wg<bf16_t, 1, Q_DIRECT, 1, 1, 256>(p, rp, workspace, workspace_bytes, (hipStream_t)stream);
}

int msseg_conv3d_gather_wgrad(const void* x, long long ldx, const void* dy, long long lddy, float* dw, int N, int ID,
                              int IH, int IW, int Cin, int Cout, int k, int s, int pd, int accumulate, void* workspace,
                              size_t workspace_bytes, int dtype, msseg_stream_t stream) {
    if (!x || !dy || !dw || !workspace) MSSEG_FAIL(MSSEG_EINVAL, "conv3d_gather_wgrad: null pointer");
    if (dtype != MSSEG_F32 && dtype != MSSEG_BF16) MSSEG_FAIL(MSSEG_EINVAL, "conv3d_gather_wgrad: bad dtype");
    const int esz = dtype == MSSEG_F32 ? 4 : 2;
    if (((uintptr_t)dy & 15) || (lddy * esz) % 16) MSSEG_FAIL(MSSEG_EINVAL, "conv3d_gather_wgrad: dy alignment");
    if (k < 1 || s < 1 || pd < 0) MSSEG_FAIL(MSSEG_EINVAL, "conv3d_gather_wgrad: bad kernel");
    const int OD = (ID + 2 * pd - k) / s + 1, OH = (IH + 2 * pd - k) / s + 1, OW = (IW + 2 * pd - k) / s + 1;
    const long long NV = (long long)N * OD * OH * OW;
    if (OD < 1 || OH < 1 || OW < 1 || NV > 0x7fffffffLL) MSSEG_FAIL(MSSEG_EINVAL, "conv3d_gather_wgrad: bad shape");
    const int KT = k * k * k;
    if (msseg_stem_eligible(dtype, Cin, Cout, k, s, pd, ldx, lddy, dy) && (lddy % 8) == 0 &&
        workspace_bytes >= (size_t)8 * 4096 * ceil_div(Cout, 32)) {
        StemWgParams sp{};
        sp.x = x; sp.ldx = ldx; sp.dy = dy; sp.lddy = lddy; sp.N = N; sp.D = ID; sp.H = IH; sp.W = IW; sp.M = Cout;
        int gx = msseg_stem_wgrad_grid(sp);
        const long long fit = (long long)(workspace_bytes / ((size_t)4096 * ceil_div(Cout, 32)));
        if (gx > fit) gx = (int)(fit & ~7LL);
        sp.slabs = (float*)workspace;
        int rc = msseg_stem_wgrad_launch(sp, gx, (hipStream_t)stream);
        if (rc) return rc;
        ReduceParams rq{};
        rq.dw = dw; rq.M = Cout; rq.M0 = Cout; rq.T = 1; rq.K = KT; rq.K0 = 1;
        rq.s_m0 = KT; rq.s_k1 = 1; rq.s_k0 = KT; rq.accumulate = accumulate;
        rq.slabs = sp.slabs + (k == 1 ? 13 : 0); rq.mblks = ceil_div(Cout, 32); rq.kblks = 1; rq.nslots = gx; rq.cbw = 32;
        return launch_reduce(rq, (hipStream_t)stream);
    }
    WgradParams p{};
    p.pten = dy; p.ldp = lddy; p.qten = x; p.ldq = ldx;
    p.N = 1; p.D = 1; p.H = 1; p.W = (int)NV; p.M = Cout; p.K = Cin * KT;
    p.ID = ID; p.IH = IH; p.IW = IW; p.OD = OD; p.OH = OH; p.OW = OW; p.cin = Cin; p.k = k; p.s = s; p.p = pd;
    ReduceParams rp{};
    rp.dw = dw; rp.M = Cout; rp.M0 = Cout; rp.T = 1; rp.K = Cin * KT; rp.K0 = Cin;
    rp.s_m0 = (long long)Cin * KT; rp.s_k1 = 1; rp.s_k0 = KT; rp.accumulate = accumulate;
    return dtype == MSSEG_F32
               ? launch_wg<float, 1, Q_GATHER, 1, 1, 256>(p, rp, workspace, workspace_bytes, (hipStream_t)stream)
               : launch_wg<bf16_t, 1, Q_GATHER, 1, 1, 256>(p, rp, workspace, workspace_bytes, (hipStream_t)stream);
}

int msseg_deconv_k2s2_wgrad(const void* x, long long ldx, const void* dy, long long lddy, float* dw, int N, int D, int H,
                            int W, int Cin, int Cout, int accumulate, void* workspace, size_t workspace_bytes,
                            int dtype, msseg_stream_t stream) {
    int rc = wg_check(x, ldx, dy, lddy, dw, workspace, dtype);
    if (rc) return rc;
    const int esz = dtype == MSSEG_F32 ? 4 : 2;
    const long long NV = (long long)N * D * H * W;
    if (Cout % (16 / esz) || NV < 1 || NV > 0x7fffffffLL / 8) MSSEG_FAIL(MSSEG_EINVAL, "deconv_k2s2_wgrad: bad shape");
    if (msseg_lwg_deconv_ok(dtype, NV, Cin, Cout, x, ldx, dy, lddy))
        return msseg_lwg_deconv_wgrad(x, ldx, dy, lddy, dw, N, D, H, W, Cin, Cout, accumulate, workspace, workspace_bytes,
                                      (hipStream_t)stream);
    WgradParams p{};
    p.pten = x; p.ldp = ldx; p.qten = dy; p.ldq = lddy;
    p.N = 1; p.D = 1; p.H = 1; p.W = (int)NV; p.M = Cin; p.K = 8 * Cout;
    p.OD = D; p.OH = H; p.OW = W; p.creal = Cout;
    ReduceParams rp{};
    rp.dw = dw; rp.M = Cin; rp.M0 = Cin; rp.T = 1; rp.K = 8 * Cout; rp.K0 = Cout;
    rp.s_m0 = (long long)Cout * 8; rp.s_k1 = 1; rp.s_k0 = 8; rp.accumulate = accumulate;
    return dtype == MSSEG_F32
               ? launch_wg<float, 1, Q_DECONV, 1, 1, 256>(p, rp, workspace, workspace_bytes, (hipStream_t)stream)
               : launch_wg<bf16_t, 1, Q_DECONV, 1, 1, 256>(p, rp, workspace, workspace_bytes, (hipStream_t)stream);
}

}
```

### medicalsemseg_amd/csrc/k3pp.h

```cpp
#pragma once
#include "common.h"

struct K3ppParams {
    const void* x;
    long long ldx;
    const void* wp;
    const float* bias;
    void* y;
    long long ldy;
    int N, D, H, W, K, M;
    float* stats;
    float* stats_ws;
    unsigned int* counter;
    const void* nb_y; long long nb_ldy;
    const void* nb_a; long long nb_lda;
    const float* nb_stats;
    float nb_slope, nb_eps; long long nb_S;
    float* nb_dgamma; float* nb_dbeta; int nb_acc;
    int accumulate;
};

bool msseg_k3pp_eligible(const K3ppParams& p);
int msseg_k3pp_launch(const K3ppParams& p, hipStream_t stream);

bool msseg_k3c48_shape_ok(int N, int D, int H, int W, int M);
bool msseg_k3c48_eligible(const K3ppParams& p);
int msseg_k3c48_launch(const K3ppParams& p, hipStream_t stream);

struct K3FinParams {
    const float* ws;
    int R, N, coutb, M;
    float* stats;
    const float* nb_stats;
    float nb_eps; long long nb_S;
    float* nb_dgamma; float* nb_dbeta; int nb_acc;
};
int msseg_k3_stats_finalize(const K3FinParams& f, int ncb, hipStream_t stream);

struct K3WgParams {
    const void* pten; long long ldp;
    const void* qten; long long ldq;
    float* slabs;
    int N, D, H, W, M, K, kblks;
    int dbg_noload;
};
bool msseg_k3wg_pp_eligible(const K3WgParams& p);
int msseg_k3wg_pp_grid(const K3WgParams& p);
int msseg_k3wg_pp_launch(const K3WgParams& p, int gx, hipStream_t stream);

struct StemParams {
    const void* x; long long ldx;
    const void* wp;
    const float* bias;
    void* y; long long ldy;
    int N, D, H, W, M;
    float* stats; float* stats_ws;
    int taps;
    const float* nstats; const float* gamma; const float* beta; float eps, slope;
};
struct StemWgParams {
    const void* x; long long ldx;
    const void* dy; long long lddy;
    float* slabs;
    int N, D, H, W, M;
};
bool msseg_stem_eligible(int dtype, int Cin, int Cout, int k, int s, int pd, long long ldx, long long ldy, const void* y);
int msseg_stem_fwd_launch(const StemParams& p, hipStream_t stream);
int msseg_stem_wgrad_grid(const StemWgParams& p);
int msseg_stem_wgrad_launch(const StemWgParams& p, int gx, hipStream_t stream);

bool msseg_deconv2_fast_eligible(int dtype, int Cin, int Cout, const void* coarse, long long ldc, const void* fine,
                                 long long ldf, const float* bias);
int msseg_deconv2_fwd_launch(const void* x, long long ldx, const void* wp, const float* bias, void* y, long long ldy, int N,
                             int D, int H, int W, int Cin, int Cout, hipStream_t stream);
int msseg_deconv2_bwd_launch(const void* dy, long long lddy, const void* wp, void* dx, long long lddx, int N, int D, int H,
                             int W, int Cin, int Cout, const void* yraw, long long ldyraw, const void* act, long long ldact,
                             const float* fwd_stats, float slope, float eps, float* red, float* dgamma, float* dbeta,
                             int accumulate, float* dbias, int dbias_accumulate, void* scratch, size_t scratch_bytes,
                             hipStream_t stream);

bool msseg_deconv2g_fwd_eligible(int dtype, int Cin, int Cout, const void* coarse, long long ldc, const void* fine,
                                 long long ldf, const float* bias);
int msseg_deconv2g_fwd_launch(const void* x, long long ldx, const void* wp, const float* bias, void* y, long long ldy, int N,
                              int D, int H, int W, int Cin, int Cout, hipStream_t stream);
bool msseg_deconv2g_bwd_eligible(int dtype, int Cin, int Cout, const void* coarse, long long ldc, const void* fine,
                                 long long ldf);
int msseg_deconv2g_bwd_launch(const void* dy, long long lddy, const void* wp, void* dx, long long lddx, float* part, int N,
                              int D, int H, int W, int Cin, int Cout, hipStream_t stream);
bool msseg_linear_regw_eligible(int dtype, long long NV, int Cin, int Cout, const void* x, long long ldx, const void* y,
                                long long ldy, const float* bias);
int msseg_linear_regw_launch(const void* x, long long ldx, const void* wp, const float* bias, void* y, long long ldy,
                             long long NV, int Cin, int Cout, hipStream_t stream);
```

### medicalsemseg_amd/csrc/stem_conv.hip

```cpp
#include "k3pp.h"

namespace {

constexpr int TD = 4, TH = 4, TW = 16;
constexpr int PD = TD + 2, PH = TH + 2, PW = TW + 2;
constexpr int HV = PD * PH * PW;

typedef __attribute__((address_space(3))) unsigned char lds_u8;
typedef __attribute__((ext_vector_type(16))) float f32x16_t;

struct TileCo { int n, d0, h0, w0; };

struct Sched {
    int tiles_w, tiles_h, tiles_d, t_first, t_step, n_my;
    MSSEG_DEVFN void init(int N, int D, int H, int W) {
        tiles_w = (W + TW - 1) / TW; tiles_h = (H + TH - 1) / TH; tiles_d = (D + TD - 1) / TD;
        const int ntiles = N * tiles_d * tiles_h * tiles_w;
        int t_end;
        if ((gridDim.x & 7) == 0) {
            const int chunk = (ntiles + 7) >> 3, xcd = blockIdx.x & 7;
            t_first = xcd * chunk + (blockIdx.x >> 3);
            t_step = gridDim.x >> 3;
            t_end = min(ntiles, (xcd + 1) * chunk);
        } else {
            t_first = blockIdx.x; t_step = gridDim.x; t_end = ntiles;
        }
        n_my = t_first < t_end ? (t_end - t_first + t_step - 1) / t_step : 0;
    }
    MSSEG_DEVFN TileCo tile(int k) const {
        int t = t_first + k * t_step;
        TileCo tc;
        tc.w0 = (t % tiles_w) * TW; t /= tiles_w;
        tc.h0 = (t % tiles_h) * TH; t /= tiles_h;
        tc.d0 = (t % tiles_d) * TD; t /= tiles_d;
        tc.n = t;
        return tc;
    }
};

constexpr int F_THREADS = 512;
template <int STATS, int JT, int NORM = 0>
__global__ __launch_bounds__(F_THREADS) void stem_fwd_kernel(const StemParams p) {
    constexpr int CBW = JT * 16;
    constexpr int F_STAT_FLOATS = 8 * MSSEG_STATS_NMAX * CBW * 2;
    __shared__ __attribute__((aligned(16))) unsigned short halo[2][HV + 8];
    __shared__ float ldsS[STATS ? F_STAT_FLOATS : 1];
    const int tid = threadIdx.x, lane = tid & 63;
    const int wave = __builtin_amdgcn_readfirstlane(tid >> 6);
    const int r = lane & 15, q = lane >> 4;
    const int coutblk = blockIdx.y;
    const unsigned short* __restrict__ xg = (const unsigned short*)p.x;
    bf16_t* __restrict__ yg = (bf16_t*)p.y;
    Sched sc;
    sc.init(p.N, p.D, p.H, p.W);

    u32x4_t wf[JT];
#pragma unroll
    for (int jt = 0; jt < JT; ++jt)
        wf[jt] = *(const u32x4_t*)((const unsigned char*)p.wp + (long long)coutblk * (4 * CBW * 16) + (q * CBW + jt * 16 + r) * 16);
    f32x4_t bv[JT];
#pragma unroll
    for (int jt = 0; jt < JT; ++jt) {
        bv[jt] = f32x4_t{0.f, 0.f, 0.f, 0.f};
        if (p.bias) bv[jt] = *(const f32x4_t*)(p.bias + coutblk * CBW + jt * 16 + q * 4);
    }
    const int ntaps = p.taps == 1 ? 1 : 27;
    int toff[8];
#pragma unroll
    for (int j = 0; j < 8; ++j) {
        const int k = q * 8 + j;
        toff[j] = ntaps == 1 ? (PH + 1) * PW + 1 : ((k < 27) ? ((k / 9) * PH + ((k / 3) % 3)) * PW + (k % 3) : 0);
    }
    if (STATS) {
        for (int i = tid; i < F_STAT_FLOATS; i += F_THREADS) ldsS[i] = 0.f;
    }
    float nsc[NORM ? JT : 1][4], nsh[NORM ? JT : 1][4];
    int n_n = -1;
    auto load_norm = [&](int n) {
        if constexpr (NORM != 0) {
            const float inv = 1.0f / (float)((long long)p.D * p.H * p.W);
#pragma unroll
            for (int jt = 0; jt < JT; ++jt)
#pragma unroll
                for (int e = 0; e < 4; ++e) {
                    const int c = coutblk * CBW + jt * 16 + q * 4 + e;
                    const float su = p.nstats[((long long)n * p.M + c) * 2 + 0], su2 = p.nstats[((long long)n * p.M + c) * 2 + 1];
                    const float mean = su * inv;
                    float var = su2 * inv - mean * mean;
                    var = var > 0.f ? var : 0.f;
                    const float rstd = rsqrtf(var + p.eps);
                    nsc[jt][e] = rstd * (p.gamma ? p.gamma[c] : 1.f);
                    nsh[jt][e] = (p.beta ? p.beta[c] : 0.f) - mean * nsc[jt][e];
                }
        }
    };
    float s1[JT][4], s2[JT][4];
    int s_n = -1;
#pragma unroll
    for (int jt = 0; jt < JT; ++jt)
#pragma unroll
        for (int e = 0; e < 4; ++e) s1[jt][e] = s2[jt][e] = 0.f;
    auto flush_stats = [&]() {
        if (s_n < 0) return;
        float* slot = ldsS + ((wave * MSSEG_STATS_NMAX + s_n) * CBW) * 2;
#pragma unroll
        for (int jt = 0; jt < JT; ++jt)
#pragma unroll
            for (int e = 0; e < 4; ++e) {
                float a = s1[jt][e], b = s2[jt][e];
#pragma unroll
                for (int o = 1; o < 16; o <<= 1) {
                    a += __shfl_xor(a, o);
                    b += __shfl_xor(b, o);
                }
                if (r == 0) {
                    float* sp = slot + (jt * 16 + q * 4 + e) * 2;
                    sp[0] += a;
                    sp[1] += b;
                }
                s1[jt][e] = s2[jt][e] = 0.f;
            }
    };

    unsigned short st[2];
    auto fetch = [&](const TileCo& tc) {
#pragma unroll
        for (int it = 0; it < 2; ++it) {
            const int hv = tid + it * F_THREADS;
            const int hd = hv / (PH * PW), rem = hv - hd * (PH * PW), hh = rem / PW, hw = rem - hh * PW;
            const int d = tc.d0 - 1 + hd, h = tc.h0 - 1 + hh, w = tc.w0 - 1 + hw;
            const bool inb = hv < HV && (unsigned)d < (unsigned)p.D && (unsigned)h < (unsigned)p.H && (unsigned)w < (unsigned)p.W;
            st[it] = inb ? xg[((((long long)tc.n * p.D + d) * p.H + h) * p.W + w) * p.ldx] : (unsigned short)0;
        }
    };
    auto commit = [&](int buf) {
#pragma unroll
        for (int it = 0; it < 2; ++it) {
            const int hv = tid + it * F_THREADS;
            if (hv < HV) halo[buf][hv] = st[it];
        }
    };

    if (sc.n_my > 0) {
        fetch(sc.tile(0));
        commit(0);
    }
    __syncthreads();
    const int dw = wave >> 1, h2 = (wave & 1) * 2;
    for (int k = 0; k < sc.n_my; ++k) {
        const TileCo tc = sc.tile(k);
        if (k + 1 < sc.n_my) fetch(sc.tile(k + 1));
        const unsigned short* hb = halo[k & 1];
        if constexpr (STATS != 0) {
            if (tc.n != s_n) { flush_stats(); s_n = tc.n; }
        }
        if constexpr (NORM != 0) {
            if (tc.n != n_n) { load_norm(tc.n); n_n = tc.n; }
        }
#pragma unroll
        for (int m = 0; m < 2; ++m) {
            const int hrow = h2 + m;
            const int base = (dw * PH + hrow) * PW + r;
            unsigned short v[8];
#pragma unroll
            for (int j = 0; j < 8; ++j) v[j] = hb[base + toff[j]];
            u32x4_t xf;
#pragma unroll
            for (int j = 0; j < 4; ++j) xf[j] = (unsigned)v[2 * j] | ((unsigned)v[2 * j + 1] << 16);
            const int d = tc.d0 + dw, h = tc.h0 + hrow, w = tc.w0 + r;
            const bool ok = d < p.D && h < p.H && w < p.W;
            const long long vox = (((long long)tc.n * p.D + d) * p.H + h) * p.W + w;
#pragma unroll
            for (int jt = 0; jt < JT; ++jt) {
                f32x4_t acc = {0.f, 0.f, 0.f, 0.f};
                mma_chunk<bf16_t>(acc, wf[jt], xf);
                const f32x4_t o = acc + bv[jt];
                const bf16x4_t ob = {(bf16_t)o[0], (bf16_t)o[1], (bf16_t)o[2], (bf16_t)o[3]};
                if constexpr (NORM != 0) {
                    bf16x4_t oa;
#pragma unroll
                    for (int e = 0; e < 4; ++e) {
                        const float z = (float)ob[e] * nsc[jt][e] + nsh[jt][e];
                        oa[e] = (bf16_t)(z > 0.f ? z : z * p.slope);
                    }
                    if (ok) *(bf16x4_t*)(yg + vox * p.ldy + coutblk * CBW + jt * 16 + q * 4) = oa;
                } else {
                    if (ok && yg != nullptr) *(bf16x4_t*)(yg + vox * p.ldy + coutblk * CBW + jt * 16 + q * 4) = ob;
                }
                if constexpr (STATS != 0) {
#pragma unroll
                    for (int e = 0; e < 4; ++e) {
                        const float rv = ok ? (float)ob[e] : 0.f;
                        s1[jt][e] += rv;
                        s2[jt][e] += rv * rv;
                    }
                }
            }
        }
        if (k + 1 < sc.n_my) commit((k + 1) & 1);
        __syncthreads();
    }
    if constexpr (STATS != 0) {
        flush_stats();
        __syncthreads();
        const int PN = p.N * CBW * 2;
        float* wsp = p.stats_ws + ((long long)blockIdx.y * gridDim.x + blockIdx.x) * PN;
        for (int i = tid; i < PN; i += F_THREADS) {
            float s = 0.f;
#pragma unroll
            for (int wv = 0; wv < 8; ++wv) s += ldsS[wv * MSSEG_STATS_NMAX * CBW * 2 + i];
            wsp[i] = s;
        }
    }
}

constexpr int W_THREADS = 256;
constexpr int XP = 24;
constexpr int XS_ELEMS = PD * PH * XP;
constexpr int P_BYTES = TD * TH * TW * 64;

__device__ u32x4_t g_stem_zero_chunk;

MSSEG_DEVFN void glds16(const void* g, void* l) {
    __builtin_amdgcn_global_load_lds((const __attribute__((address_space(1))) void*)g,
                                     (__attribute__((address_space(3))) void*)l, 16, 0, 0);
}
MSSEG_DEVFN bf16x4_t lds_tr(lds_u8* p) {
    return __builtin_amdgcn_ds_read_tr16_b64_v4bf16((__attribute__((address_space(3))) bf16x4_t*)p);
}

__global__ __launch_bounds__(W_THREADS) void stem_wgrad_kernel(const StemWgParams p) {
    extern __shared__ __attribute__((aligned(256))) unsigned char smem[];
    constexpr int BUF_BYTES = P_BYTES + 3 * XS_ELEMS * 2 + 64;
    lds_u8* smem3 = (lds_u8*)smem;
    const int tid = threadIdx.x, lane = tid & 63;
    const int wave = __builtin_amdgcn_readfirstlane(tid >> 6);
    const int mblk = blockIdx.y;
    const unsigned char* dyg = (const unsigned char*)p.dy + mblk * 64;
    const unsigned short* __restrict__ xg = (const unsigned short*)p.x;
    Sched sc;
    sc.init(p.N, p.D, p.H, p.W);

    unsigned p_off[4];
#pragma unroll
    for (int j = 0; j < 4; ++j) {
        const int tv = (wave + 4 * j) * 16 + (lane >> 2);
        const int td = tv / (TH * TW), th = (tv / TW) % TH, tw = tv % TW;
        p_off[j] = (unsigned)((((long long)td * p.H + th) * p.W + tw) * p.lddy * 2 + (lane & 3) * 16);
    }
    unsigned short st[3];
    auto load_tile = [&](const TileCo& tc, int buf) {
        unsigned char* base = smem + buf * BUF_BYTES;
        const long long pvox = (((long long)tc.n * p.D + tc.d0) * p.H + tc.h0) * p.W + tc.w0;
        const unsigned char* pb = dyg + pvox * p.lddy * 2;
        const bool full = tc.d0 + TD <= p.D && tc.h0 + TH <= p.H && tc.w0 + TW <= p.W;
        const unsigned char* zsrc = (const unsigned char*)&g_stem_zero_chunk;
        const bool ch_ok = mblk * 32 + (lane & 3) * 8 < p.M;
#pragma unroll
        for (int j = 0; j < 4; ++j) {
            const unsigned char* src = pb + p_off[j];
            if (!ch_ok) src = zsrc;
            if (!full) {
                const int tv = (wave + 4 * j) * 16 + (lane >> 2);
                const int td = tv / (TH * TW), th = (tv / TW) % TH, tw = tv % TW;
                if (!(tc.d0 + td < p.D && tc.h0 + th < p.H && tc.w0 + tw < p.W)) src = zsrc;
            }
            glds16(src, base + (wave + 4 * j) * 1024);
        }
#pragma unroll
        for (int it = 0; it < 3; ++it) {
            const int hv = tid + it * W_THREADS;
            const int hd = hv / (PH * PW), rem = hv - hd * (PH * PW), hh = rem / PW, hw = rem - hh * PW;
            const int d = tc.d0 - 1 + hd, h = tc.h0 - 1 + hh, w = tc.w0 - 1 + hw;
            const bool inb = hv < HV && (unsigned)d < (unsigned)p.D && (unsigned)h < (unsigned)p.H && (unsigned)w < (unsigned)p.W;
            st[it] = inb ? xg[((((long long)tc.n * p.D + d) * p.H + h) * p.W + w) * p.ldx] : (unsigned short)0;
        }
    };
    auto commit_x = [&](int buf) {
        unsigned short* xs = (unsigned short*)(smem + buf * BUF_BYTES + P_BYTES);
#pragma unroll
        for (int it = 0; it < 3; ++it) {
            const int hv = tid + it * W_THREADS;
            if (hv < HV) {
                const int hd = hv / (PH * PW), rem = hv - hd * (PH * PW), hh = rem / PW, hw = rem - hh * PW;
#pragma unroll
                for (int c = 0; c < 3; ++c) {
                    const int slot = hw - c;
                    if (slot >= 0 && slot < TW) xs[c * XS_ELEMS + (hd * PH + hh) * XP + slot] = st[it];
                }
            }
        }
    };

    const int G = lane >> 4, qr = (lane >> 2) & 3, pc = lane & 3;
    unsigned a_rd[2];
#pragma unroll
    for (int i = 0; i < 2; ++i) a_rd[i] = (8 * (G >> 1) + 4 * i + qr) * 64 + ((G & 1) << 5) + pc * 8;
    const int tap = lane & 31;
    const bool tap_ok = tap < 27;
    const int tkd = tap / 9, tkh = (tap / 3) % 3, tkw = tap % 3;
    const unsigned b_rd = tap_ok ? (unsigned)(P_BYTES + (tkw * XS_ELEMS + (tkd * PH + tkh) * XP + 8 * (lane >> 5)) * 2) : 0u;

    f32x16_t acc;
#pragma unroll
    for (int e = 0; e < 16; ++e) acc[e] = 0.f;

    if (sc.n_my > 0) {
        load_tile(sc.tile(0), 0);
        commit_x(0);
    }
    asm volatile("s_waitcnt vmcnt(0)" ::: "memory");
    __syncthreads();
    for (int k = 0; k < sc.n_my; ++k) {
        const int buf = k & 1;
        if (k + 1 < sc.n_my) load_tile(sc.tile(k + 1), buf ^ 1);
        lds_u8* bb = smem3 + buf * BUF_BYTES;
#pragma unroll
        for (int i4 = 0; i4 < 4; ++i4) {
            const int row = wave * 4 + i4;
            const int td = row >> 2, th = row & 3;
            const bf16x4_t lo = lds_tr(bb + a_rd[0] + row * 1024), hi = lds_tr(bb + a_rd[1] + row * 1024);
            const bf16x8_t af = {lo[0], lo[1], lo[2], lo[3], hi[0], hi[1], hi[2], hi[3]};
            u32x4_t bfr = *(const u32x4_t*)(smem + buf * BUF_BYTES + b_rd + ((td * PH + th) * XP) * 2);
            if (!tap_ok) bfr = u32x4_t{0u, 0u, 0u, 0u};
            acc = __builtin_amdgcn_mfma_f32_32x32x16_bf16(af, __builtin_bit_cast(bf16x8_t, bfr), acc, 0, 0, 0);
        }
        if (k + 1 < sc.n_my) commit_x(buf ^ 1);
        asm volatile("s_waitcnt vmcnt(0)" ::: "memory");
        __syncthreads();
    }
    float* xch = (float*)smem;
    const int col = lane & 31, rb = 4 * (lane >> 5);
#pragma unroll
    for (int e = 0; e < 16; ++e) xch[(wave * 32 + (e & 3) + 8 * (e >> 2) + rb) * 32 + col] = acc[e];
    __syncthreads();
    float* slab = p.slabs + ((long long)blockIdx.y * gridDim.x + blockIdx.x) * 1024;
    for (int i = tid; i < 1024; i += W_THREADS) slab[i] = xch[i] + xch[1024 + i] + xch[2048 + i] + xch[3072 + i];
}

}

bool msseg_stem_eligible(int dtype, int Cin, int Cout, int k, int s, int pd, long long ldx, long long ldy, const void* y) {
    static const bool off = getenv("MSSEG_NO_STEM") != nullptr;
    return !off && dtype == MSSEG_BF16 && Cin == 1 && ((k == 3 && pd == 1) || (k == 1 && pd == 0)) && s == 1 &&
           (Cout % 32 == 0 || Cout % 48 == 0) && Cout <= 256 &&
           ldx >= 1 && (ldy % 4) == 0 && (((uintptr_t)y) & 7) == 0;
}

int msseg_stem_fwd_launch(const StemParams& p, hipStream_t stream) {
    const int cbw = (p.M % 32 == 0) ? 32 : 48;
    const int ncb = p.M / cbw;
    const int tiles = p.N * ceil_div(p.D, TD) * ceil_div(p.H, TH) * ceil_div(p.W, TW);
    int gx = msseg_num_cus() * 2 / ncb;
    gx &= ~7;
    if (gx < 8) gx = 8;
    if (gx > tiles) gx = tiles;
    if (p.nstats != nullptr && p.stats != nullptr) MSSEG_FAIL(MSSEG_EINVAL, "stem_fwd: the normalised form emits no statistics");
    if (p.y == nullptr && p.stats == nullptr) MSSEG_FAIL(MSSEG_EINVAL, "stem_fwd: nothing to produce");
    if (cbw == 32) {
        if (p.nstats) hipLaunchKernelGGL((stem_fwd_kernel<0, 2, 1>), dim3(gx, ncb), dim3(F_THREADS), 0, stream, p);
        else if (p.stats) hipLaunchKernelGGL((stem_fwd_kernel<1, 2>), dim3(gx, ncb), dim3(F_THREADS), 0, stream, p);
        else hipLaunchKernelGGL((stem_fwd_kernel<0, 2>), dim3(gx, ncb), dim3(F_THREADS), 0, stream, p);
    } else {
        if (p.nstats) hipLaunchKernelGGL((stem_fwd_kernel<0, 3, 1>), dim3(gx, ncb), dim3(F_THREADS), 0, stream, p);
        else if (p.stats) hipLaunchKernelGGL((stem_fwd_kernel<1, 3>), dim3(gx, ncb), dim3(F_THREADS), 0, stream, p);
        else hipLaunchKernelGGL((stem_fwd_kernel<0, 3>), dim3(gx, ncb), dim3(F_THREADS), 0, stream, p);
    }
    MSSEG_CHECK_LAUNCH("stem_fwd");
    if (p.stats) {
        K3FinParams f{};
        f.ws = p.stats_ws; f.R = gx; f.N = p.N; f.coutb = cbw; f.M = p.M; f.stats = p.stats;
        return msseg_k3_stats_finalize(f, ncb, stream);
    }
    return MSSEG_OK;
}

int msseg_stem_wgrad_grid(const StemWgParams& p) {
    const int tiles = p.N * ceil_div(p.D, TD) * ceil_div(p.H, TH) * ceil_div(p.W, TW);
    int gx = msseg_num_cus() * 2 / ceil_div(p.M, 32);
    gx &= ~7;
    if (gx < 8) gx = 8;
    if (gx > tiles) gx = tiles;
    return gx;
}

int msseg_stem_wgrad_launch(const StemWgParams& p, int gx, hipStream_t stream) {
    const int lds = 2 * (P_BYTES + 3 * XS_ELEMS * 2 + 64);
    static msseg_lds_attr_once attr;
    if (!attr.ensure((const void*)stem_wgrad_kernel, lds)) MSSEG_FAIL(MSSEG_ELAUNCH, "stem_wgrad: cannot set dynamic LDS size %d", lds);
    hipLaunchKernelGGL(stem_wgrad_kernel, dim3(gx, ceil_div(p.M, 32)), dim3(W_THREADS), lds, stream, p);
    MSSEG_CHECK_LAUNCH("stem_wgrad");
    return MSSEG_OK;
}
```

### medicalsemseg_amd/hip.py

```python
from __future__ import annotations

import ctypes as C
import os
from typing import Optional

import torch

_HERE = os.path.dirname(os.path.abspath(__file__))
LIB_PATH = os.environ.get("MSSEG_LIB") or os.path.join(_HERE, "libmsseg_hip.so")

F32, BF16 = 0, 1
_DT = {torch.float32: F32, torch.bfloat16: BF16}
_LAB = {torch.float32: 0, torch.bfloat16: 1, torch.uint8: 2, torch.int64: 3}

_lib = None

_vp, _ll, _i, _f, _sz = C.c_void_p, C.c_longlong, C.c_int, C.c_float, C.c_size_t

SIGNATURES = {
    "msseg_abi_version": ([], _i),
    "msseg_last_error": ([], C.c_char_p),
    "msseg_num_cus": ([], _i),
    "msseg_packed_weight_bytes": ([_i, _i, _i, _i, _i], _sz),
    "msseg_pack_weights": ([_vp, _vp, _i, _i, _i, _i, _i, _i, _ll, _ll, _ll, _ll, _ll, _i, _i, _vp], _i),
    "msseg_pack_weights_batch": ([_vp, _i, _ll, _ll, _i, _vp], _i),
    "msseg_cout_block": ([_i], _i),
    "msseg_conv3d_k3_cout_block": ([_i, _i, _i, _i, _i], _i),
    "msseg_conv3d_k3_variant": ([_i, _i, _i, _i, _i], _i),
    "msseg_conv3d_k3_kernel": ([_i, _i, _i, _i, _i, _i, _i], _i),
    "msseg_conv3d_k3_fwd": ([_vp, _ll, _vp, _vp, _vp, _ll, _i, _i, _i, _i, _i, _i, _vp, _vp, _sz, _i, _vp], _i),
    "msseg_conv3d_k3_fwd_accumulate": ([_vp, _ll, _vp, _vp, _ll, _i, _i, _i, _i, _i, _i, _vp, _vp, _sz, _i, _vp], _i),
    "msseg_dwconv3d_k3_fwd": ([_vp, _ll, _vp, _vp, _vp, _ll, _i, _i, _i, _i, _i, _i, _i, _vp], _i),
    "msseg_dwconv3d_k3_wgrad": ([_vp, _ll, _vp, _ll, _vp, _vp, _i, _i, _i, _i, _i, _i, _i, _vp, _sz, _i, _vp], _i),
    "msseg_interp_trilinear_fwd": ([_vp, _ll, _vp, _ll, _i, _i, _i, _i, _i, _i, _i, _i, _i, _vp], _i),
    "msseg_interp_trilinear_bwd_workspace_bytes": ([_i, _i, _i, _i, _i, _i, _i, _i], _sz),
    "msseg_interp_trilinear_bwd": ([_vp, _ll, _vp, _ll, _i, _i, _i, _i, _i, _i, _i, _i, _vp, _sz, _i, _vp], _i),
    "msseg_kv_attention_fwd": ([_vp, _vp, _vp, _vp, _i, _i, _i, _i, _i, _f, _i, _vp], _i),
    "msseg_kv_attention_bwd_workspace_bytes": ([_i, _i, _i, _i, _i], _sz),
    "msseg_kv_attention_bwd": ([_vp, _vp, _vp, _vp, _vp, _vp, _vp, _i, _i, _i, _i, _i, _f, _vp, _sz, _i, _vp], _i),
    "msseg_scale_channels": ([_vp, _vp, _vp, _i, _ll, _i, _i, _vp], _i),
    "msseg_reduce_scratch_bytes": ([], _sz),
    "msseg_conv3d_k3_dgrad_inbwd": ([_vp, _ll, _vp, _vp, _ll, _i, _i, _i, _i, _i, _i, _vp, _ll, _vp, _ll, _vp, _f, _f, _vp,
                                     _vp, _vp, _i, _vp, _sz, _i, _vp], _i),
    "msseg_conv3d_k1_dgrad_inbwd": ([_vp, _ll, _vp, _vp, _ll, _i, _ll, _i, _i, _vp, _ll, _vp, _ll, _vp, _f, _f, _vp,
                                     _vp, _vp, _i, _vp, _sz, _i, _vp], _i),
    "msseg_deconv_k2s2_bwd_data_inbwd": ([_vp, _ll, _vp, _vp, _ll, _i, _i, _i, _i, _i, _i, _vp, _ll, _vp, _ll, _vp, _f, _f,
                                          _vp, _vp, _vp, _i, _vp, _sz, _i, _vp], _i),
    "msseg_deconv_k2s2_bwd_fused": ([_vp, _ll, _vp, _vp, _ll, _i, _i, _i, _i, _i, _i, _vp, _ll, _vp, _ll, _vp, _f, _f,
                                     _vp, _vp, _vp, _i, _vp, _i, _vp, _sz, _i, _vp], _i),
    "msseg_conv3d_k3s2_fwd": ([_vp, _ll, _vp, _vp, _vp, _ll, _i, _i, _i, _i, _i, _i, _i, _vp], _i),
    "msseg_zero_stuff2": ([_vp, _ll, _vp, _ll, _i, _i, _i, _i, _i, _i, _i, _i, _i, _vp], _i),
    "msseg_window_attention_fwd": ([_vp, _vp, _vp, _vp, _vp, _i, _i, _i, _i, _i, _i, _i, _i, _i, _vp], _i),
    "msseg_window_attention_bwd": ([_vp, _vp, _vp, _vp, _vp, _vp, _vp, _vp, _i, _i, _i, _i, _i, _i, _i, _i, _i, _vp], _i),
    "msseg_window_attention_bwd_ws": ([_vp, _vp, _vp, _vp, _vp, _vp, _vp, _vp, _i, _i, _i, _i, _i, _i, _i, _i, _i, _vp,
                                       _sz, _vp], _i),
    "msseg_window_attention_fwd2": ([_vp, _vp, _vp, _vp, _vp, _i, _i, _i, _i, _i, _i, _i, _i, _i, _i, _vp], _i),
    "msseg_window_attention_bwd2": ([_vp, _vp, _vp, _vp, _vp, _vp, _vp, _vp, _i, _i, _i, _i, _i, _i, _i, _i, _i, _i, _vp,
                                     _sz, _vp], _i),
    "msseg_window_attention_bwd_workspace_bytes": ([_i, _i, _i, _i, _i, _i, _i, _i, _i], _sz),
    "msseg_window_attention_fwd3": ([_vp, _vp, _vp, _vp, _vp, _i, _i, _i, _i, _i, _i, _i, _i, _i, _ll, _i, _vp], _i),
    "msseg_window_attention_bwd3": ([_vp, _vp, _vp, _vp, _vp, _vp, _vp, _vp, _i, _i, _i, _i, _i, _i, _i, _i, _i, _ll, _i,
                                     _vp, _sz, _vp], _i),
    "msseg_window_attention_bwd3_workspace_bytes": ([_i, _i, _i, _i, _i, _i, _i, _i, _i, _ll, _i], _sz),
    "msseg_rel_bias_affine_fold": ([_vp, _vp, _vp, _vp, _vp, _vp, _i, _i, _i, _vp], _i),
    "msseg_rel_bias_affine_grad_workspace_bytes": ([_i, _i], _sz),
    "msseg_rel_bias_affine_grad": ([_vp, _vp, _vp, _vp, _vp, _vp, _vp, _vp, _i, _i, _i, _i, _vp, _sz, _vp], _i),
    "msseg_layernorm_fwd": ([_vp, _ll, _vp, _vp, _vp, _ll, _vp, _vp, _ll, _i, _f, _i, _vp], _i),
    "msseg_layernorm_bwd": ([_vp, _ll, _vp, _vp, _vp, _vp, _ll, _vp, _ll, _ll, _i, _i, _vp], _i),
    "msseg_layernorm_bwd_add": ([_vp, _ll, _vp, _vp, _vp, _vp, _ll, _vp, _ll, _vp, _ll, _ll, _i, _i, _vp], _i),
    "msseg_layernorm_param_grad": ([_vp, _ll, _vp, _vp, _vp, _ll, _vp, _vp, _i, _ll, _i, _vp, _sz, _i, _vp], _i),
    "msseg_gelu_fwd": ([_vp, _vp, _ll, _i, _vp], _i),
    "msseg_gelu_bwd": ([_vp, _vp, _vp, _ll, _i, _vp], _i),
    "msseg_linear_wgrad_ok": ([_ll, _i, _i, _i], _i),
    "msseg_linear_wgrad": ([_vp, _ll, _vp, _ll, _vp, _vp, _ll, _i, _i, _i, _i, _vp, _sz, _i, _vp], _i),
    "msseg_linear_gelu_ok": ([_ll, _i, _i, _i], _i),
    "msseg_linear_gelu_fwd": ([_vp, _ll, _vp, _vp, _vp, _ll, _vp, _ll, _ll, _i, _i, _i, _vp], _i),
    "msseg_linear_gelu_bwd": ([_vp, _ll, _vp, _vp, _ll, _vp, _ll, _ll, _i, _i, _i, _vp], _i),
    "msseg_linear_add_ok": ([_ll, _i, _i, _i], _i),
    "msseg_linear_add_fwd": ([_vp, _ll, _vp, _vp, _vp, _ll, _vp, _ll, _ll, _i, _i, _i, _vp], _i),
    "msseg_conv3d_stem_fwd": ([_vp, _ll, _vp, _vp, _vp, _ll, _i, _i, _i, _i, _i, _vp, _vp, _sz, _i, _vp], _i),
    "msseg_conv3d_stem_k1_fwd": ([_vp, _ll, _vp, _vp, _vp, _ll, _i, _i, _i, _i, _i, _vp, _vp, _sz, _i, _vp], _i),
    "msseg_conv3d_stem_norm_fwd": ([_vp, _ll, _vp, _vp, _vp, _vp, _vp, _f, _f, _vp, _ll, _i, _i, _i, _i, _i, _i, _vp], _i),
    "msseg_conv3d_k1_head_dgrad_inbwd": ([_vp, _ll, _vp, _vp, _ll, _i, _ll, _i, _i, _vp, _ll, _vp, _vp, _vp, _f, _f, _vp, _vp,
                                          _vp, _i, _vp, _sz, _i, _vp], _i),
    "msseg_conv3d_k1_head_norm_fwd": ([_vp, _ll, _vp, _vp, _vp, _f, _f, _vp, _vp, _vp, _ll, _i, _ll, _i, _i, _i, _vp], _i),
    "msseg_conv3d_k1_head_bwd_fused": ([_vp, _ll, _vp, _vp, _ll, _i, _ll, _i, _i, _vp, _ll, _vp, _vp, _vp, _f, _f, _vp, _vp,
                                        _vp, _i, _vp, _i, _vp, _sz, _i, _vp], _i),
    "msseg_conv3d_k1_head_fwd": ([_vp, _ll, _vp, _vp, _vp, _ll, _ll, _i, _i, _i, _vp], _i),
    "msseg_conv3d_k1_fwd": ([_vp, _ll, _vp, _vp, _vp, _ll, _ll, _i, _i, _i, _vp], _i),
    "msseg_conv3d_gather_fwd": ([_vp, _ll, _vp, _vp, _vp, _ll, _i, _i, _i, _i, _i, _i, _i, _i, _i, _i, _vp], _i),
    "msseg_deconv_k2s2_fwd": ([_vp, _ll, _vp, _vp, _vp, _ll, _i, _i, _i, _i, _i, _i, _i, _vp], _i),
    "msseg_deconv_k2s2_bwd_data": ([_vp, _ll, _vp, _vp, _ll, _i, _i, _i, _i, _i, _i, _i, _vp], _i),
    "msseg_deconv_k4s4_fwd": ([_vp, _ll, _vp, _vp, _vp, _ll, _i, _i, _i, _i, _i, _i, _i, _vp], _i),
    "msseg_deconv_k4s4_bwd_data": ([_vp, _ll, _vp, _vp, _ll, _i, _i, _i, _i, _i, _i, _i, _vp], _i),
    "msseg_wgrad_workspace_bytes": ([_i, _i, _i], _sz),
    "msseg_conv3d_k3_wgrad_kernel": ([_i, _i, _i, _i, _i, _i, _i], _i),
    "msseg_conv3d_k3_wgrad": ([_vp, _ll, _vp, _ll, _vp, _i, _i, _i, _i, _i, _i, _i, _vp, _sz, _i, _vp], _i),
    "msseg_conv3d_k1_wgrad": ([_vp, _ll, _vp, _ll, _vp, _ll, _i, _i, _i, _vp, _sz, _i, _vp], _i),
    "msseg_conv3d_gather_wgrad": ([_vp, _ll, _vp, _ll, _vp, _i, _i, _i, _i, _i, _i, _i, _i, _i, _i, _vp, _sz, _i, _vp], _i),
    "msseg_deconv_k2s2_wgrad": ([_vp, _ll, _vp, _ll, _vp, _i, _i, _i, _i, _i, _i, _i, _vp, _sz, _i, _vp], _i),
    "msseg_deconv_k4s4_wgrad": ([_vp, _ll, _vp, _ll, _vp, _i, _i, _i, _i, _i, _i, _i, _vp, _sz, _i, _vp], _i),
    "msseg_channel_stats": ([_vp, _ll, _vp, _i, _ll, _i, _vp, _sz, _i, _vp], _i),
    "msseg_instnorm_act_fwd": ([_vp, _ll, _vp, _vp, _vp, _vp, _ll, _vp, _ll, _i, _ll, _i, _f, _f, _i, _vp], _i),
    "msseg_instnorm_act_poolbwd_reduce": ([_vp, _ll, _vp, _vp, _vp, _vp, _ll, _vp, _ll, _vp, _ll, _vp, _vp, _vp, _i,
                                           _i, _i, _i, _i, _i, _f, _f, _vp, _sz, _i, _vp], _i),
    "msseg_instnorm_act_pool_fwd": ([_vp, _ll, _vp, _vp, _vp, _vp, _ll, _vp, _ll, _i, _i, _i, _i, _i, _f, _f, _i, _vp], _i),
    "msseg_instnorm_act_bwd_reduce": ([_vp, _ll, _vp, _vp, _vp, _vp, _ll, _vp, _ll, _vp, _vp, _vp, _i, _i, _ll, _i, _f, _f, _vp, _sz, _i, _vp], _i),
    "msseg_instnorm_act_bwd_apply": ([_vp, _ll, _vp, _vp, _vp, _vp, _ll, _vp, _ll, _vp, _vp, _ll, _vp, _ll, _i, _ll, _i, _f, _f, _i, _vp], _i),
    "msseg_maxpool2_fwd": ([_vp, _ll, _vp, _ll, _i, _i, _i, _i, _i, _i, _vp], _i),
    "msseg_maxpool2_bwd": ([_vp, _ll, _vp, _ll, _vp, _ll, _i, _i, _i, _i, _i, _i, _i, _vp], _i),
    "msseg_ncdhw_to_ndhwc": ([_vp, _i, _vp, _ll, _i, _i, _i, _ll, _vp], _i),
    "msseg_ndhwc_to_ncdhw": ([_vp, _ll, _i, _vp, _i, _i, _i, _ll, _vp], _i),
    "msseg_channel_sum": ([_vp, _ll, _vp, _ll, _i, _i, _vp, _sz, _i, _vp], _i),
    "msseg_axpy_rows": ([_vp, _vp, _vp, _vp, _i, _ll, _i, _vp], _i),
    "msseg_add": ([_vp, _ll, _vp, _ll, _vp, _ll, _ll, _i, _i, _vp], _i),
    "msseg_dice_ce_partials": ([_vp, _ll, _i, _vp, _i, _vp, _vp, _i, _ll, _i, _vp], _i),
    "msseg_dice_ce_fwd": ([_vp, _ll, _i, _vp, _i, _vp, _vp, _vp, _i, _ll, _i, _f, _f, _vp, _sz, _vp], _i),
    "msseg_dice_ce_finalize": ([_vp, _vp, _i, _ll, _i, _f, _f, _vp], _i),
    "msseg_dice_ce_bwd": ([_vp, _ll, _i, _vp, _i, _vp, _vp, _vp, _ll, _i, _ll, _i, _f, _f, _vp], _i),
    "msseg_adamw_step": ([_vp, _vp, _vp, _vp, _vp, _ll, _f, _f, _f, _f, _f, _i, _vp, _vp, _vp], _i),
    "msseg_sumsq": ([_vp, _ll, _vp, _vp, _i, _vp], _i),
    "msseg_sw_blend": ([_vp, _ll, _i, _vp, _vp, _vp, _i, _i, _i, _i, _i, _i, _i, _i, _i, _i, _vp], _i),
    "msseg_sw_normalize": ([_vp, _vp, _i, _ll, _vp], _i),
    "msseg_sw_gather": ([_vp, _vp, _i, _i, _i, _i, _i, _i, _i, _i, _i, _i, _i, _f, _vp], _i),
    "msseg_box_copy": ([_vp, _ll, _i, _i, _i, _vp, _ll, _i, _i, _i, _i, _i, _i, _vp], _i),
    "msseg_merge_gather_fwd": ([_vp, _ll, _i, _i, _i, _vp, _ll, _i, _i, C.c_uint, _i, _vp], _i),
    "msseg_merge_gather_bwd": ([_vp, _ll, _vp, _ll, _i, _i, _i, _i, _i, C.c_uint, _i, _vp], _i),
    "msseg_argmax_u8": ([_vp, _i, _ll, _vp, _vp], _i),
    "msseg_resample_nearest_u8": ([_vp, _i, _i, _i, _vp, _i, _i, _i, _vp], _i),
    "msseg_majority_vote_u8": ([_vp, _i, _ll, _i, _vp, _vp], _i),
    "msseg_aug_crop_batch": ([_vp, _vp, _i, _i, _i, _i, _vp, _i, _vp, _i, _vp, _i, _vp], _i),
    "msseg_intensity_prep": ([_vp, _i, _i, _i, _i, _i, _i, _f, _f, _i, _f, _f, _vp, _vp, _vp], _i),
    "msseg_resample_spacing": ([_vp, _i, _i, _i, _i, _i, _vp, _i, _i, _i, C.c_double, C.c_double, C.c_double, _vp], _i),
    "msseg_crop_pad_copy": ([_vp, _i, _i, _i, _i, _i, _vp, _vp, _i, _i, _i, _vp, _f, _i, _vp], _i),
    "msseg_slab_counts": ([_vp, _vp, _i, _i, _i, _f, _vp, _vp], _i),
    "msseg_pick_voxels": ([_vp, _i, _vp, _i, _i, _f, _vp, _vp], _i),
    "msseg_aug_crop_multi": ([_vp, _i, _vp, _vp, _i, _i, _vp, _i, _vp, _i, _vp], _i),
    "msseg_sw_gather_batch": ([_vp, _ll, _vp, _ll, _i, _vp, _i, _i, _i, _i, _i, _i, _i, _i, _f, _vp], _i),
    "msseg_sw_blend_batch": ([_vp, _ll, _i, _vp, _vp, _ll, _vp, _ll, _vp, _i, _i, _i, _i, _i, _i, _i, _i, _vp], _i),
    "msseg_deconv_k2s2_bwd_partials_ok": ([_i, _i, _i], _i),
    "msseg_deconv_k2s2_bwd_partials": ([_vp, _ll, _vp, _vp, _sz, _i, _i, _i, _i, _i, _i, _i, _vp], _i),
    "msseg_conv3d_k3_small_ok": ([_i, _i, _i, _i, _i, _i, _i], _i),
    "msseg_conv3d_k3_small_workspace_bytes": ([_i, _i, _i, _i, _i, _i], _sz),
    "msseg_conv3d_k3_small_stage_groups": ([_i, _i, _i, _i, _i, _i], _i),
    "msseg_conv3d_k3_small_partials": ([_vp, _ll, _vp, _vp, _sz, _i, _i, _i, _i, _i, _i, _vp], _i),
    "msseg_conv3d_k3_small_fwd_finish": ([_vp, _i, _vp, _vp, _vp, _f, _f, _vp, _ll, _vp, _ll, _vp, _ll, _vp, _i, _i, _i, _i,
                                          _i, _vp], _i),
    "msseg_conv3d_k3_small_fwd_finish_res": ([_vp, _i, _vp, _vp, _vp, _f, _f, _vp, _ll, _vp, _ll, _vp, _ll, _vp, _ll, _vp, _i, _i, _i, _i,
                                              _i, _vp], _i),
    "msseg_conv3d_k3_small_bwd_finish": ([_vp, _i, _vp, _ll, _vp, _ll, _vp, _vp, _vp, _f, _f, _vp, _vp, _i, _i, _i, _i, _i,
                                          _i, _vp], _i),
    "msseg_avgpool3d_k3": ([_vp, _ll, _vp, _ll, _i, _i, _i, _i, _i, _i, _vp], _i),
    "msseg_hd_edges": ([_vp, _vp, _i, _i, _i, _i, _vp, _vp, _vp, _vp], _i),
    "msseg_hd_directed_workspace_bytes": ([_i, _i, _i], _sz),
    "msseg_hd_directed_hist": ([_vp, _vp, _i, _i, _i, _i, _vp, _vp, _sz, _vp, _i, _vp], _i),
    "msseg_ktimer_enable": ([_i], _i),
    "msseg_ktimer_reset": ([], _i),
    "msseg_ktimer_count": ([], _i),
    "msseg_ktimer_get": ([_i, C.c_char_p, _i, C.POINTER(C.c_float)], _i),
}


def load_library(path: Optional[str] = None):
    global _lib
    if _lib is not None and path is None:
        return _lib
    p = path or LIB_PATH
    if not os.path.exists(p):
        raise RuntimeError(
            f"{p} not found: build it with `python -c 'import __graft_entry__ as g; g.build()'` "
            f"(or `make -C medicalsemseg_amd/csrc`).  There is no CPU fallback.")
    lib = C.CDLL(p)
    for name, (args, res) in SIGNATURES.items():
        fn = getattr(lib, name)
        fn.argtypes = args
        fn.restype = res
    if lib.msseg_abi_version() != 1:
        raise RuntimeError("libmsseg_hip.so ABI version mismatch")
    _lib = lib
    return lib


def lib():
    real = _lib if _lib is not None else load_library()
    if TIMER.enabled:
        return _TimedLib(real)
    return real


class MssegError(RuntimeError):
    pass


def _ck(rc: int, what: str):
    if rc != 0:
        raise MssegError(f"{what} failed ({rc}): {lib().msseg_last_error().decode()}")


def _stream() -> int:
    return torch.cuda.current_stream().cuda_stream


def _need_gpu(*ts):
    for t in ts:
        if t is not None and not t.is_cuda:
            raise RuntimeError("medicalsemseg_amd kernels run on the GPU only (got a CPU tensor); "
                               "there is no CPU fallback")


def dt(t: torch.Tensor) -> int:
    try:
        return _DT[t.dtype]
    except KeyError:
        raise TypeError(f"unsupported dtype {t.dtype} (float32 / bfloat16 only)")


def ld(t: torch.Tensor) -> int:
    C = t.shape[-1]
    if C > 1 and t.stride(-1) != 1:
        raise ValueError("channels-last tensor must have unit channel stride")
    l = None
    exp = None
    for d in range(t.dim() - 2, -1, -1):
        if t.shape[d] > 1:
            if l is None:
                l = t.stride(d)
                exp = l * t.shape[d]
            else:
                if t.stride(d) != exp:
                    raise ValueError(f"tensor is not a dense channels-last volume: shape {tuple(t.shape)} "
                                     f"stride {t.stride()}")
                exp *= t.shape[d]
    if l is None:
        l = C
    if l < C:
        raise ValueError("voxel stride smaller than the channel count")
    return l


def _nbytes(*ts) -> float:
    return float(sum(t.numel() * t.element_size() for t in ts if t is not None))


def _p(t: Optional[torch.Tensor]):
    return None if t is None else t.data_ptr()


def cout_block(M: int) -> int:
    return lib().msseg_cout_block(M)

# ... 361 lines not shown
    nv = x.numel() // x.shape[-1]
    _ck(lib().msseg_conv3d_k1_fwd(_p(x), ld(x), _p(wp), _p(bias), _p(y), ld(y), nv, cin, cout, dt(x), _stream()),
        "conv3d_k1_fwd")
    return y


def conv3d_k1_dgrad_inbwd(dy, wp, da, cin, cout, yraw, act, fwd_stats, slope, eps, dgamma=None, dbeta=None,
                          accumulate=False):
    _need_gpu(dy, wp, da, yraw, act, fwd_stats)
    N = da.shape[0]
    S = da.numel() // (N * da.shape[-1])
    red = torch.empty(N, cout, 2, dtype=torch.float32, device=dy.device)
    sc = scratch(dy.device)
    _ck(lib().msseg_conv3d_k1_dgrad_inbwd(_p(dy), ld(dy), _p(wp), _p(da), ld(da), N, S, cin, cout, _p(yraw), ld(yraw),
                                          _p(act), ld(act), _p(fwd_stats), slope, eps, _p(red), _p(dgamma), _p(dbeta),
                                          int(accumulate), _p(sc), sc.numel(), dt(dy), _stream()), "conv3d_k1_dgrad_inbwd")
    return red


def deconv_k2s2_bwd_data_inbwd(dy, wp, dx, cin, cout, yraw, act, fwd_stats, slope, eps, dgamma=None, dbeta=None,
                               accumulate=False):
    _need_gpu(dy, wp, dx, yraw, act, fwd_stats)
    N, D, H, W = dx.shape[:4]
    red = torch.empty(N, cin, 2, dtype=torch.float32, device=dy.device)
    sc = scratch(dy.device)
    _ck(lib().msseg_deconv_k2s2_bwd_data_inbwd(_p(dy), ld(dy), _p(wp), _p(dx), ld(dx), N, D, H, W, cin, cout, _p(yraw),
                                               ld(yraw), _p(act), ld(act), _p(fwd_stats), slope, eps, _p(red),
                                               _p(dgamma), _p(dbeta), int(accumulate), _p(sc), sc.numel(), dt(dy),
                                               _stream()), "deconv_k2s2_bwd_data_inbwd")
    return red


def deconv_k2s2_bwd_fused(dy, wp, dx, cin, cout, next_norm=None, dbias=None, dbias_accumulate=False, dgamma=None, dbeta=None,
                          accumulate=False):
    _need_gpu(dy, wp, dx)
    N, D, H, W = dx.shape[:4]
    red = None
    yraw = act = stats = None
    slope = eps = 0.0
    if next_norm is not None:
        yraw, act, stats, slope, eps = next_norm
        red = torch.empty(N, cin, 2, dtype=torch.float32, device=dy.device)
    sc = scratch(dy.device)
    _ck(lib().msseg_deconv_k2s2_bwd_fused(_p(dy), ld(dy), _p(wp), _p(dx), ld(dx), N, D, H, W, cin, cout, _p(yraw),
                                          ld(yraw) if yraw is not None else 0, _p(act), ld(act) if act is not None else 0,
                                          _p(stats), slope, eps, _p(red), _p(dgamma), _p(dbeta), int(accumulate), _p(dbias),
                                          int(dbias_accumulate), _p(sc), sc.numel(), dt(dy), _stream()),
        "deconv_k2s2_bwd_fused")
    return red


def conv3d_gather(x, wp, bias, y, cin, cout, k, s, p):
    _need_gpu(x, wp, y)
    N, D, H, W = x.shape[:4]
    _ck(lib().msseg_conv3d_gather_fwd(_p(x), ld(x), _p(wp), _p(bias), _p(y), ld(y), N, D, H, W, cin, cout, k, s, p,
                                      dt(x), _stream()), "conv3d_gather_fwd")
    return y


def conv3d_stem_norm(x, wp, bias, stats, gamma, beta, eps, slope, y, cout):
    _need_gpu(x, wp, y, stats)
    N, D, H, W = x.shape[:4]
    _ck(lib().msseg_conv3d_stem_norm_fwd(_p(x), ld(x), _p(wp), _p(bias), _p(stats), _p(gamma), _p(beta), eps, slope, _p(y), ld(y),
                                         N, D, H, W, cout, dt(x), _stream()), "conv3d_stem_norm_fwd")
    return y


def conv3d_stem(x, wp, bias, y, cout, stats=None, k=3):
    _need_gpu(x, wp)
    N, D, H, W = x.shape[:4]
    sc = scratch(x.device) if stats is not None else None
    fn = lib().msseg_conv3d_stem_fwd if k == 3 else lib().msseg_conv3d_stem_k1_fwd
    _ck(fn(_p(x), ld(x), _p(wp), _p(bias), _p(y), ld(y) if y is not None else 0, N, D, H, W, cout, _p(stats), _p(sc),
                                    sc.numel() if sc is not None else 0, dt(x), _stream()), "conv3d_stem_fwd")
    return y


def deconv_k2s2(x, wp, bias, y, cin, cout):
    _need_gpu(x, wp, y)
    N, D, H, W = x.shape[:4]
    _ck(lib().msseg_deconv_k2s2_fwd(_p(x), ld(x), _p(wp), _p(bias), _p(y), ld(y), N, D, H, W, cin, cout, dt(x),
                                    _stream()), "deconv_k2s2_fwd")
    return y


def deconv_k2s2_bwd_data(dy, wp, dx, cin, cout):
    _need_gpu(dy, wp, dx)
    N, D, H, W = dx.shape[:4]
    _ck(lib().msseg_deconv_k2s2_bwd_data(_p(dy), ld(dy), _p(wp), _p(dx), ld(dx), N, D, H, W, cin, cout, dt(dy),
                                         _stream()), "deconv_k2s2_bwd_data")
    return dx


def deconv_k4s4(x, wp, bias, y, cin, cout):
    _need_gpu(x, wp, y)
    N, D, H, W = x.shape[:4]
    if tuple(y.shape) != (N, 4 * D, 4 * H, 4 * W, cout):
        raise ValueError(f"deconv_k4s4: output shape {tuple(y.shape)} for input {tuple(x.shape)}, cout {cout}")
    nv = N * D * H * W
    esz = x.element_size()
    TIMER.launch("deconv_k4s4_fwd", 2.0 * nv * 64 * cin * cout, nv * (cin + 64 * cout) * esz + 64 * cin * cout * esz,
                 lambda: _ck(lib().msseg_deconv_k4s4_fwd(_p(x), ld(x), _p(wp), _p(bias), _p(y), ld(y), N, D, H, W, cin, cout,
                                                         dt(x), _stream()), "deconv_k4s4_fwd"))
    return y


def deconv_k4s4_bwd_data(dy, wp, dx, cin, cout):
    _need_gpu(dy, wp, dx)
    N, D, H, W = dx.shape[:4]
    if tuple(dy.shape) != (N, 4 * D, 4 * H, 4 * W, cout):
        raise ValueError(f"deconv_k4s4_bwd_data: gradient shape {tuple(dy.shape)} for input {tuple(dx.shape)}, cout {cout}")
    nv = N * D * H * W
    esz = dy.element_size()
    TIMER.launch("deconv_k4s4_bwd_data", 2.0 * nv * 64 * cin * cout, nv * (cin + 64 * cout) * esz + 64 * cin * cout * esz,
                 lambda: _ck(lib().msseg_deconv_k4s4_bwd_data(_p(dy), ld(dy), _p(wp), _p(dx), ld(dx), N, D, H, W, cin, cout,
                                                              dt(dy), _stream()), "deconv_k4s4_bwd_data"))
    return dx


_ws_cache = {}
_ws_retired = []


def workspace(nbytes: int, device) -> torch.Tensor:
    key = (device.index if device.index is not None else torch.cuda.current_device())
    buf = _ws_cache.get(key)
    if buf is None or buf.numel() < nbytes:
        if buf is not None:
            _ws_retired.append(buf)
        buf = torch.empty(max(nbytes, 64 << 20), dtype=torch.uint8, device=device)
        _ws_cache[key] = buf
    return buf


def _wg_ws(M, T, K, device):
    return workspace(lib().msseg_wgrad_workspace_bytes(M, T, K), device)


def conv3d_k3_wgrad(x, dy, dw, cin, cout, accumulate=False):
    _need_gpu(x, dy, dw)
    N, D, H, W = x.shape[:4]
    ws = _wg_ws(cout, 27, cin, x.device)
    nv = N * D * H * W

    def go():
        _ck(lib().msseg_conv3d_k3_wgrad(_p(x), ld(x), _p(dy), ld(dy), _p(dw), N, D, H, W, cin, cout, int(accumulate),
                                        _p(ws), ws.numel(), dt(x), _stream()), "conv3d_k3_wgrad")
    key = "conv3d_k3_wgrad"
    if TIMER.enabled:
        key += "/v%d" % lib().msseg_conv3d_k3_wgrad_kernel(N, D, H, W, cin, cout, dt(x))
    TIMER.launch(key, 2.0 * nv * 27 * cin * cout, nv * (cin + cout) * x.element_size() + 27 * cin * cout * 4, go)


def conv3d_k1_wgrad(x, dy, dw, cin, cout, accumulate=False):
    _need_gpu(x, dy, dw)
    nv = x.numel() // x.shape[-1]
    ws = _wg_ws(cout, 1, cin, x.device)
    _ck(lib().msseg_conv3d_k1_wgrad(_p(x), ld(x), _p(dy), ld(dy), _p(dw), nv, cin, cout, int(accumulate), _p(ws),
                                    ws.numel(), dt(x), _stream()), "conv3d_k1_wgrad")


def linear_wgrad_ok(x, cin, cout) -> bool:
    return bool(x.is_cuda and x.dtype == torch.bfloat16 and
                lib().msseg_linear_wgrad_ok(x.numel() // x.shape[-1], cin, cout, BF16))


def linear_wgrad(x, dy, dw, dbias, cin, cout, accumulate_w=False, accumulate_b=False):
    _need_gpu(x, dy, dw)
    nv = x.numel() // x.shape[-1]
    ws = _wg_ws(cout, 1, cin, x.device)
    esz = x.element_size()
    TIMER.launch("linear_wgrad", 2.0 * nv * cin * cout, nv * (cin + cout) * esz + cin * cout * 4,
                 lambda: _ck(lib().msseg_linear_wgrad(_p(x), ld(x), _p(dy), ld(dy), _p(dw), _p(dbias), nv, cin, cout,
                                                      int(accumulate_w), int(accumulate_b), _p(ws), ws.numel(), dt(x),
                                                      _stream()), "linear_wgrad"))


def conv3d_gather_wgrad(x, dy, dw, cin, cout, k, s, p, accumulate=False):
    _need_gpu(x, dy, dw)
    N, D, H, W = x.shape[:4]
    ws = _wg_ws(cout, 1, cin * k ** 3, x.device)
    _ck(lib().msseg_conv3d_gather_wgrad(_p(x), ld(x), _p(dy), ld(dy), _p(dw), N, D, H, W, cin, cout, k, s, p,
                                        int(accumulate), _p(ws), ws.numel(), dt(x), _stream()), "conv3d_gather_wgrad")


def deconv_k2s2_wgrad(x, dy, dw, cin, cout, accumulate=False):
    _need_gpu(x, dy, dw)
    N, D, H, W = x.shape[:4]
    ws = _wg_ws(cin, 1, 8 * cout, x.device)
    _ck(lib().msseg_deconv_k2s2_wgrad(_p(x), ld(x), _p(dy), ld(dy), _p(dw), N, D, H, W, cin, cout, int(accumulate),
                                      _p(ws), ws.numel(), dt(x), _stream()), "deconv_k2s2_wgrad")


def deconv_k4s4_wgrad(x, dy, dw, cin, cout, accumulate=False):
    _need_gpu(x, dy, dw)
    N, D, H, W = x.shape[:4]
    if tuple(dy.shape) != (N, 4 * D, 4 * H, 4 * W, cout) or dw.numel() != cin * cout * 64 or not dw.is_contiguous():
        raise ValueError(f"deconv_k4s4_wgrad: shapes x {tuple(x.shape)}, dy {tuple(dy.shape)}, dw {tuple(dw.shape)}")
    ws = _wg_ws(cin, 1, 64 * cout, x.device)
    nv = N * D * H * W
    TIMER.launch("deconv_k4s4_wgrad", 2.0 * nv * 64 * cin * cout, nv * (cin + 64 * cout) * x.element_size() + 64 * cin * cout * 4,
                 lambda: _ck(lib().msseg_deconv_k4s4_wgrad(_p(x), ld(x), _p(dy), ld(dy), _p(dw), N, D, H, W, cin, cout,
                                                           int(accumulate), _p(ws), ws.numel(), dt(x), _stream()),
                             "deconv_k4s4_wgrad"))


def _nsc(x):
    N, C = x.shape[0], x.shape[-1]
    return N, x.numel() // (N * C), C


def dwconv3d_k3(x, w_taps, bias, y, flip=False):
    if w_taps.dtype != x.dtype:
        raise ValueError("dwconv3d_k3: the weight table must have the activation dtype")
    _need_gpu(x, w_taps, y)
    N, D, H, W, C = x.shape
    _ck(lib().msseg_dwconv3d_k3_fwd(_p(x), ld(x), _p(w_taps), _p(bias), _p(y), ld(y), N, D, H, W, C, int(flip), dt(x),
                                    _stream()), "dwconv3d_k3_fwd")
    return y


def avgpool3d_k3(x, y):
    _need_gpu(x, y)
    N, D, H, W, Cc = x.shape
    _ck(lib().msseg_avgpool3d_k3(_p(x), ld(x), _p(y), ld(y), N, D, H, W, Cc, dt(x), _stream()), "avgpool3d_k3")
    return y


def dwconv3d_k3_wgrad(x, dy, dw, dbias, acc_w=False, acc_b=False):
    _need_gpu(x, dy)
    N, D, H, W, C = x.shape
    sc = scratch(x.device)
    _ck(lib().msseg_dwconv3d_k3_wgrad(_p(x), ld(x), _p(dy), ld(dy), _p(dw), _p(dbias), int(acc_w), int(acc_b), N, D, H, W, C,
                                      _p(sc), sc.numel(), dt(x), _stream()), "dwconv3d_k3_wgrad")


def interp_trilinear(x, y):
    _need_gpu(x, y)
    N, ID, IH, IW, C = x.shape
    _ck(lib().msseg_interp_trilinear_fwd(_p(x), ld(x), _p(y), ld(y), N, ID, IH, IW, y.shape[1], y.shape[2], y.shape[3], C,
                                         dt(x), _stream()), "interp_trilinear_fwd")
    return y


def interp_trilinear_bwd(dy, dx):
    _need_gpu(dy, dx)
    N, ID, IH, IW, C = dx.shape
    OD, OH, OW = dy.shape[1:4]
    nb = lib().msseg_interp_trilinear_bwd_workspace_bytes(N, ID, IH, IW, OD, OH, OW, C)
    ws = torch.empty(nb, dtype=torch.uint8, device=dx.device)
    _ck(lib().msseg_interp_trilinear_bwd(_p(dy), ld(dy), _p(dx), ld(dx), N, ID, IH, IW, OD, OH, OW, C, _p(ws), nb, dt(dx),
                                         _stream()), "interp_trilinear_bwd")
    return dx


def kv_attention_fwd(q, kv, heads, scale):
    _need_gpu(q, kv)
    B, N, C = q.shape
    M = kv.shape[1]
    o = torch.empty_like(q)
    lse = torch.empty(B, heads, N, dtype=torch.float32, device=q.device)
    _ck(lib().msseg_kv_attention_fwd(_p(q), _p(kv), _p(o), _p(lse), B, N, M, heads, C // heads, scale, dt(q), _stream()),
        "kv_attention_fwd")
    return o, lse


def kv_attention_bwd(q, kv, o, lse, dout, heads, scale):
    _need_gpu(q, kv, o, lse, dout)
    B, N, C = q.shape
    M = kv.shape[1]
    dq, dkv = torch.empty_like(q), torch.empty_like(kv)
    nb = lib().msseg_kv_attention_bwd_workspace_bytes(B, N, M, heads, C // heads)
    ws = torch.empty(nb, dtype=torch.uint8, device=q.device)
    _ck(lib().msseg_kv_attention_bwd(_p(q), _p(kv), _p(o), _p(lse), _p(dout), _p(dq), _p(dkv), B, N, M, heads, C // heads,
                                     scale, _p(ws), nb, dt(q), _stream()), "kv_attention_bwd")
    return dq, dkv


def scale_channels(x, scale, y):
    _need_gpu(x, scale, y)
    N, C = x.shape[0], x.shape[-1]
    _ck(lib().msseg_scale_channels(_p(x), _p(scale), _p(y), N, x.numel() // (N * C), C, dt(x), _stream()), "scale_channels")
    return y


def channel_stats(x, stats=None):
    _need_gpu(x)
    N, S, Cc = _nsc(x)
    if stats is None:
        stats = torch.empty(N, Cc, 2, dtype=torch.float32, device=x.device)
    sc = scratch(x.device)
    _ck(lib().msseg_channel_stats(_p(x), ld(x), _p(stats), N, S, Cc, _p(sc), sc.numel(), dt(x), _stream()),
        "channel_stats")
    return stats


def instnorm_act_fwd(x, stats, gamma, beta, y, slope, eps=1e-5, residual=None):
    _need_gpu(x, stats, y)
    N, S, Cc = _nsc(x)
    TIMER.launch("instnorm_act_fwd", 0.0, _nbytes(x, y, residual), lambda: _ck(lib().msseg_instnorm_act_fwd(_p(x), ld(x), _p(stats), _p(gamma), _p(beta), _p(residual),
                                     ld(residual) if residual is not None else 0, _p(y), ld(y), N, S, Cc, eps, slope,
                                     dt(x), _stream()), "instnorm_act_fwd"))
    return y


def instnorm_pool_ok(x, y, pooled) -> bool:
# ... 577 lines not shown
```

### medicalsemseg_amd/layers.py

```python
from __future__ import annotations

import os

from typing import Optional

import torch

from . import hip

weights_epoch = 0


def bump_weights_epoch():
    global weights_epoch
    weights_epoch += 1


class _PackRegistry:

    def __init__(self):
        self.groups = {}

    def add(self, device, dtype, src, dst, job):
        g = self.groups.setdefault((device, dtype), {"jobs": [], "table": None, "keep": []})
# ... 112 lines not shown
        with torch.cuda.stream(st):
            fn()

    def run(self, fn, *tensors):
        if self.active is None or self.mode == self.INLINE:
            return fn()
        self.keep.extend(tensors)
        if self.mode == self.DEFER:
            self.deferred.append(fn)
        else:
            self._issue(fn)

    def flush(self):
        if self.active is not None:
            for fn in self.deferred:
                self._issue(fn)
        self.deferred = []

    def join(self):
        self.flush()
        st, self.active = self.active, None
        self.mode = self.INLINE
        if st is not None:
            torch.cuda.current_stream().wait_stream(st)
        self.keep.clear()


WGRAD_SIDE = _WgradSide()


INFERENCE_FORWARD = False


class _Applied:

    def __repr__(self):
        return "APPLIED"


APPLIED = _Applied()


def _grad_buf(p: torch.nn.Parameter):
    if p.grad is None:
        p.grad = torch.empty_like(p, memory_format=torch.contiguous_format)
        return p.grad, False
    owner = getattr(p, "_msseg_gowner", None)
    if owner is not None and not getattr(p, "_msseg_kgrad", False):
        p._msseg_kgrad = True
        p._msseg_gepoch = owner._gepoch
        return p.grad, True
    if owner is not None and getattr(p, "_msseg_gepoch", -1) != owner._gepoch:
        p._msseg_gepoch = owner._gepoch
        return p.grad, False
    return p.grad, True


def _empty_like_vol(x, C, dtype=None):
    return torch.empty(x.shape[:-1] + (C,), dtype=dtype or x.dtype, device=x.device)


def _norm_grad_bufs(nrm):
    if nrm.gamma is not None and nrm.gamma.requires_grad:
        dg, acc = _grad_buf(nrm.gamma)
        db, _ = _grad_buf(nrm.beta)
        return dg, db, acc
    return None, None, False


class Conv3:

    def __init__(self, weight: torch.nn.Parameter, bias: Optional[torch.nn.Parameter]):
        self.w, self.b = weight, bias
        self.cout, self.cin = weight.shape[0], weight.shape[1]
        self.cache = PackedCache()

    def _gather(self, dtype):
        return self.cin % (8 if dtype == torch.bfloat16 else 4) != 0

    def fwd(self, x, out=None, want_stats=False):
        dtype = x.dtype
        if want_stats and out is None and self.halves_ok(tuple(x.shape[:4]), dtype):
            return self.fwd_halves(x)
        y = out if out is not None else _empty_like_vol(x, self.cout)
        stats = None
        if self._gather(dtype):
            wp = self.cache.get(self.w, dtype, "g", lambda: hip.pack_conv_gather(self.w.detach(), dtype))
            if (self.cin == 1 and dtype == torch.bfloat16 and (self.cout % 32 == 0 or self.cout % 48 == 0) and self.cout <= 256
                    and not os.environ.get("MSSEG_NO_STEM")):
                if want_stats and x.shape[0] <= 8:
                    stats = torch.empty(x.shape[0], self.cout, 2, dtype=torch.float32, device=x.device)
                hip.conv3d_stem(x, wp, self.b, y, self.cout, stats)
            else:
                hip.conv3d_gather(x, wp, self.b, y, self.cin, self.cout, 3, 1, 1)
        else:
            vol = tuple(x.shape[:4])
            wp = self.cache.get(self.w, dtype, ("f", vol), lambda: hip.pack_conv_k3(self.w.detach(), dtype, vol=vol))
            if want_stats and x.shape[0] <= 8:
                stats = torch.empty(x.shape[0], self.cout, 2, dtype=torch.float32, device=x.device)
            hip.conv3d_k3(x, wp, self.b, y, self.cin, self.cout, stats)
        if want_stats:
            return y, (stats if stats is not None else hip.channel_stats(y))
        return y

    def halves_ok(self, vol, dtype) -> int:
        if dtype != torch.bfloat16 or os.environ.get("MSSEG_NO_SPLIT_CAT"):
            return 0
        if self.cin == 96 and hip.lib().msseg_conv3d_k3_kernel(*vol, 48, self.cout, hip.BF16) == 4:
            return 48
        if (INFERENCE_FORWARD and self.cin in (64, 128) and self.cout % 32 == 0 and not os.environ.get("MSSEG_NO_KSPLIT_INFER")
                and hip.lib().msseg_conv3d_k3_kernel(*vol, 32, self.cout, hip.BF16) == 3):
            return 32
        return 0

    def fwd_halves(self, x):
        dtype, vol = x.dtype, tuple(x.shape[:4])
        h = self.halves_ok(vol, dtype)
        y = _empty_like_vol(x, self.cout)
        stats = torch.empty(x.shape[0], self.cout, 2, dtype=torch.float32, device=x.device)
        for i in range(self.cin // h):
            wi = self.w.detach()[:, i * h:(i + 1) * h]
            pi = self.cache.get(wi, dtype, ("fp", i, h, vol), lambda wi=wi: hip.pack_conv_k3(wi, dtype, vol=vol))
            xi = x[..., i * h:(i + 1) * h]
            if i == 0:
                hip.conv3d_k3(xi, pi, self.b, y, h, self.cout)
            else:
                hip.conv3d_k3_accumulate(xi, pi, y, h, self.cout, stats)
        return y, stats

    def split_ok(self, vol, dtype, ca, cb_) -> bool:
        if (os.environ.get("MSSEG_NO_SPLIT_CAT") or dtype != torch.bfloat16 or ca + cb_ != self.cin or ca != 32 or cb_ != 32
                or self.cout % 32 or vol[0] > 8):
            return False
        return hip.lib().msseg_conv3d_k3_kernel(*vol, 32, self.cout, hip.BF16) == 3

    def fwd_split(self, xa, xb):
        dtype = xa.dtype
        vol = tuple(xa.shape[:4])
        wa, wb = self.w.detach()[:, :32], self.w.detach()[:, 32:]
        pa = self.cache.get(wa, dtype, ("fa", vol), lambda: hip.pack_conv_k3(wa, dtype, vol=vol))
        pb = self.cache.get(wb, dtype, ("fb", vol), lambda: hip.pack_conv_k3(wb, dtype, vol=vol))
        y = _empty_like_vol(xa, self.cout)
        hip.conv3d_k3(xa, pa, self.b, y, 32, self.cout)
        stats = torch.empty(xa.shape[0], self.cout, 2, dtype=torch.float32, device=xa.device)
        hip.conv3d_k3_accumulate(xb, pb, y, 32, self.cout, stats)
        return y, stats

    def dgrad_accumulate_ok(self, dy) -> bool:
        if dy.dtype != torch.bfloat16 or self.cout not in (32, 48) or dy.shape[0] > 4 or os.environ.get("MSSEG_NO_DGRAD_ACCUM"):
            return False
        vol = tuple(dy.shape[:4])
        return hip.lib().msseg_conv3d_k3_kernel(*vol, self.cout, self.cin, hip.BF16) == (4 if self.cout == 48 else 3)

    def bwd(self, x, dy, need_dx=True, dx_out=None, bias_grad_is_zero=False, next_norm=None, accumulate_dx=False):
        dtype = x.dtype
        if self.w.requires_grad:
            g, acc = _grad_buf(self.w)
            if self._gather(dtype):
                WGRAD_SIDE.run(lambda: hip.conv3d_gather_wgrad(x, dy, g, self.cin, self.cout, 3, 1, 1, acc), x, dy)
            else:
                WGRAD_SIDE.run(lambda: hip.conv3d_k3_wgrad(x, dy, g, self.cin, self.cout, acc), x, dy)
        if self.b is not None and self.b.requires_grad:
            g, acc = _grad_buf(self.b)
            if bias_grad_is_zero:
                if not acc and not getattr(self.b, "_msseg_grad_is_zero", False):
                    g.zero_()
                    self.b._msseg_grad_is_zero = getattr(self.b, "_msseg_gowner", None) is not None
            else:
                hip.channel_sum(dy, g, acc)
        if not need_dx:
            return None
        if self._gather(dtype):
            raise NotImplementedError("input gradient of a few-channel stem conv is never needed on this path")
        vol = tuple(dy.shape[:4])
        if accumulate_dx:
            assert dx_out is not None and next_norm is None and self.dgrad_accumulate_ok(dy)
            wp = self.cache.get(self.w, dtype, ("d", vol),
                                lambda: hip.pack_conv_k3(self.w.detach(), dtype, dgrad=True, vol=vol))
            unused = torch.empty(dy.shape[0], self.cin, 2, dtype=torch.float32, device=dy.device)
            hip.conv3d_k3_accumulate(dy, wp, dx_out, self.cout, self.cin, unused)
            return dx_out
        if hip.conv3d_k3_small_ok(dy, self.cout, self.cin):
            wp = self.cache.get(self.w, dtype, "ds", lambda: hip.pack_conv_k3(self.w.detach(), dtype, dgrad=True, cb=32))
            part, ng = hip.conv3d_k3_small_partials(dy, wp, self.cout, self.cin)
            dx = dx_out if dx_out is not None else _empty_like_vol(dy, self.cin)
            if next_norm is not None:
                nrm, yraw, stats, act = next_norm
                dg, db, acc = _norm_grad_bufs(nrm)
                hip.conv3d_k3_small_bwd_finish(part, ng, dx, (yraw, stats, nrm.gamma, nrm.beta, nrm.eps, nrm.slope),
                                               dg, db, acc)
                return dx, APPLIED
            return hip.conv3d_k3_small_bwd_finish(part, ng, dx)
        wp = self.cache.get(self.w, dtype, ("d", vol),
                            lambda: hip.pack_conv_k3(self.w.detach(), dtype, dgrad=True, vol=vol))
        dx = dx_out if dx_out is not None else _empty_like_vol(dy, self.cin)
        if next_norm is not None:
            nrm, yraw, stats, act = next_norm
            if dy.shape[0] <= 8 and self.cin % 4 == 0:
                dg = db = None
                acc = False
                if nrm.gamma is not None and nrm.gamma.requires_grad:
                    dg, acc = _grad_buf(nrm.gamma)
                    db, _ = _grad_buf(nrm.beta)
                red = hip.conv3d_k3_dgrad_inbwd(dy, wp, dx, self.cout, self.cin, yraw, act, stats, nrm.slope, nrm.eps,
                                                dg, db, acc)
                return dx, red
            hip.conv3d_k3(dy, wp, None, dx, self.cout, self.cin)
            return dx, None
        hip.conv3d_k3(dy, wp, None, dx, self.cout, self.cin)
        return dx


class Conv1:

    def __init__(self, weight, bias):
        self.w, self.b = weight, bias
        self.cout, self.cin = weight.shape[0], weight.shape[1]
        self.cache = PackedCache()

    def _gather(self, dtype):
        return self.cin % (8 if dtype == torch.bfloat16 else 4) != 0

    def fwd(self, x, out=None, want_stats=False):
        dtype = x.dtype
        y = out if out is not None else _empty_like_vol(x, self.cout)
        if self._gather(dtype):
            wp = self.cache.get(self.w, dtype, "g", lambda: hip.pack_conv_gather(self.w.detach(), dtype))
            if (want_stats and self.cin == 1 and dtype == torch.bfloat16 and x.dim() == 5 and x.shape[0] <= 8 and hip.ld(y) == self.cout
                    and (self.cout % 32 == 0 or self.cout % 48 == 0) and self.cout <= 256 and not os.environ.get("MSSEG_NO_STEM")):
                stats = torch.empty(x.shape[0], self.cout, 2, dtype=torch.float32, device=x.device)
                hip.conv3d_stem(x, wp, self.b, y, self.cout, stats, k=1)
                return y, stats
            hip.conv3d_gather(x, wp, self.b, y, self.cin, self.cout, 1, 1, 0)
        elif (self.cout <= 4 and self.cin <= 64 and x.shape[-1] == self.cin and self.w.is_contiguous()
              and not os.environ.get("MSSEG_NO_HEAD_KERNEL")):
            hip.conv3d_k1_head(x, self.w.detach(), self.b, y, self.cin, self.cout)
        else:
            wp = self.cache.get(self.w, dtype, "f",
                                lambda: hip.pack_conv_k1(self.w.detach().reshape(self.cout, self.cin), dtype))
            hip.conv3d_k1(x, wp, self.b, y, self.cin, self.cout)
        if want_stats:
            return y, hip.channel_stats(y)
        return y

    def head_norm_ok(self, yraw) -> bool:
        epc = 16 // yraw.element_size()
        return (self.cout <= 4 and self.cin <= 64 and self.cin % epc == 0 and yraw.shape[-1] == self.cin
                and hip.ld(yraw) % epc == 0 and yraw.data_ptr() % 16 == 0 and self.w.is_contiguous()
                and not os.environ.get("MSSEG_NO_HEAD_KERNEL") and not os.environ.get("MSSEG_NO_HEAD_FUSE"))

    def fwd_norm(self, yraw, stats, nrm, out):
        return hip.conv3d_k1_head_norm(yraw, stats, nrm.gamma, nrm.beta, nrm.slope, nrm.eps, self.w.detach(), self.b, out,
                                       self.cin, self.cout)

    def bwd_norm(self, dy, dy_channels, nrm, yraw, stats):
        dyk = dy[..., :dy_channels]
        dx = torch.empty(yraw.shape, dtype=yraw.dtype, device=yraw.device)
        dg, db, acc = _norm_grad_bufs(nrm)
        if self.b is not None and self.b.requires_grad:
            g, bacc = _grad_buf(self.b)
            hip.channel_sum(dy[..., :self.cout], g, bacc)
        if self.w.requires_grad:
            gw, wacc = _grad_buf(self.w)
            red = hip.conv3d_k1_head_bwd_fused(dyk, self.w.detach(), dx, self.cin, self.cout, yraw, stats, nrm.gamma, nrm.beta,
                                               nrm.slope, nrm.eps, gw, wacc, dg, db, acc)
        else:
            red = hip.conv3d_k1_head_dgrad_inbwd(dyk, self.w.detach(), dx, self.cin, self.cout, yraw, stats, nrm.gamma,
                                                 nrm.beta, nrm.slope, nrm.eps, dg, db, acc)
        return dx, red

    def bwd(self, x, dy, need_dx=True, dy_channels=None, next_norm=None):
        dtype = x.dtype
        fused_bias = False
        if self.w.requires_grad:
            g, acc = _grad_buf(self.w)
            if self._gather(dtype):
                WGRAD_SIDE.run(lambda: hip.conv3d_gather_wgrad(x, dy[..., :self.cout], g, self.cin, self.cout, 1, 1, 0, acc), x, dy)
            elif hip.linear_wgrad_ok(x, self.cin, self.cout):
                gb, bacc = _grad_buf(self.b) if (self.b is not None and self.b.requires_grad) else (None, False)
                WGRAD_SIDE.run(lambda: hip.linear_wgrad(x, dy[..., :self.cout], g.view(self.cout, self.cin), gb, self.cin,
                                                        self.cout, acc, bacc), x, dy)
                fused_bias = True
            else:
                WGRAD_SIDE.run(lambda: hip.conv3d_k1_wgrad(x, dy[..., :self.cout], g, self.cin, self.cout, acc), x, dy)
        if self.b is not None and self.b.requires_grad and not fused_bias:
            g, acc = _grad_buf(self.b)
            hip.channel_sum(dy[..., :self.cout], g, acc)
        if not need_dx:
            return None
        if self._gather(dtype):
            raise NotImplementedError("input gradient of a few-channel 1x1 conv is never needed on this path")
        dx = _empty_like_vol(dy, self.cin)
        kpad = dy_channels if dy_channels is not None else self.cout
        dyk = dy if dy_channels is None else dy[..., :kpad]
        epc = 16 // dy.element_size()
        if (next_norm is not None and self.cout <= 4 and kpad >= 4 and self.cin <= 64 and self.cin % epc == 0 and hip.ld(dyk) % epc == 0
                and dyk.data_ptr() % 16 == 0 and self.w.is_contiguous() and not os.environ.get("MSSEG_NO_HEAD_KERNEL")):
            nrm, yraw, stats, act = next_norm
            dg, db, acc = _norm_grad_bufs(nrm)
            red = hip.conv3d_k1_head_dgrad_inbwd(dyk, self.w.detach(), dx, self.cin, self.cout, yraw, stats, nrm.gamma,
                                                 nrm.beta, nrm.slope, nrm.eps, dg, db, acc)
            return dx, red
        wp = self.cache.get(self.w, dtype, "d",
                            lambda: hip.pack_conv_k1(self.w.detach().reshape(self.cout, self.cin), dtype, dgrad=True))
        if next_norm is not None:
            nrm, yraw, stats, act = next_norm
            if dy.shape[0] <= 8 and self.cin % 4 == 0:
                dg, db, acc = _norm_grad_bufs(nrm)
                red = hip.conv3d_k1_dgrad_inbwd(dyk, wp, dx, kpad, self.cin, yraw, act, stats, nrm.slope, nrm.eps, dg, db, acc)
# ... 12 lines not shown
        self.k = weight.shape[2]
        if tuple(weight.shape[2:]) not in ((2, 2, 2), (4, 4, 4)):
            raise NotImplementedError(f"transposed conv with kernel {tuple(weight.shape[2:])}: only k = s = 2 and k = s = 4 are implemented")
        self.cache = PackedCache()

    def fwd(self, x, out=None):
        dtype = x.dtype
        N, D, H, W, _ = x.shape
        k = self.k
        y = out if out is not None else torch.empty(N, k * D, k * H, k * W, self.cout, dtype=dtype, device=x.device)
        wp = self.cache.get(self.w, dtype, "f", lambda: hip.pack_deconv(self.w.detach(), dtype))
        if k == 4:
            hip.deconv_k4s4(x, wp, self.b, y, self.cin, self.cout)
        else:
            hip.deconv_k2s2(x, wp, self.b, y, self.cin, self.cout)
        return y

    def _bwd_k4(self, x, dy, need_dx, next_norm):
        dtype = x.dtype
        if self.w.requires_grad:
            g, acc = _grad_buf(self.w)
            WGRAD_SIDE.run(lambda: hip.deconv_k4s4_wgrad(x, dy, g, self.cin, self.cout, acc), x, dy)
        if self.b is not None and self.b.requires_grad:
            g, acc = _grad_buf(self.b)
            hip.channel_sum(dy, g, acc)
        if not need_dx:
            return None
        wp = self.cache.get(self.w, dtype, "d", lambda: hip.pack_deconv(self.w.detach(), dtype, bwd=True))
        dx = torch.empty_like(x, memory_format=torch.contiguous_format)
        hip.deconv_k4s4_bwd_data(dy, wp, dx, self.cin, self.cout)
        return (dx, None) if next_norm is not None else dx

    def bwd(self, x, dy, need_dx=True, next_norm=None):
        if self.k == 4:
            return self._bwd_k4(x, dy, need_dx, next_norm)
        dtype = x.dtype
        if self.w.requires_grad:
            g, acc = _grad_buf(self.w)
            WGRAD_SIDE.run(lambda: hip.deconv_k2s2_wgrad(x, dy, g, self.cin, self.cout, acc), x, dy)
        want_db = self.b is not None and self.b.requires_grad
        if not need_dx:
            if want_db:
                g, acc = _grad_buf(self.b)
                hip.channel_sum(dy, g, acc)
            return None
        wp = self.cache.get(self.w, dtype, "d", lambda: hip.pack_deconv(self.w.detach(), dtype, bwd=True))
        dx = torch.empty_like(x, memory_format=torch.contiguous_format)
        db, dbacc = _grad_buf(self.b) if want_db else (None, False)
        if next_norm is not None and hip.deconv_k2s2_small_unit_ok(tuple(x.shape), self.cin, self.cout, dtype):
            nrm, yraw, stats, act = next_norm
            part = hip.deconv_k2s2_bwd_partials(dy, wp, self.cin, self.cout)
            dg, dbt, nacc = _norm_grad_bufs(nrm)
            hip.conv3d_k3_small_bwd_finish(part, 1, dx, (yraw, stats, nrm.gamma, nrm.beta, nrm.eps, nrm.slope), dg, dbt, nacc)
            if want_db:
                hip.channel_sum(dy, db, dbacc)
            return dx, APPLIED
        nn_ = None
        dg = dbt = None
        nacc = False
        if next_norm is not None:
            nrm, yraw, stats, act = next_norm
            if dy.shape[0] <= 8 and self.cin % 4 == 0:
                dg, dbt, nacc = _norm_grad_bufs(nrm)
                nn_ = (yraw, act, stats, nrm.slope, nrm.eps)
        red = hip.deconv_k2s2_bwd_fused(dy, wp, dx, self.cin, self.cout, nn_, db, dbacc, dg, dbt, nacc)
        return (dx, red) if next_norm is not None else dx


Deconv4 = Deconv2


class InstNormAct:

    def __init__(self, gamma: Optional[torch.nn.Parameter], beta: Optional[torch.nn.Parameter], slope: float,
                 eps: float = 1e-5):
        self.gamma, self.beta, self.slope, self.eps = gamma, beta, float(slope), float(eps)

    def fwd(self, y_raw, out=None, residual=None, stats=None, pooled=None):
        if stats is None:
            stats = hip.channel_stats(y_raw)
        a = out if out is not None else torch.empty_like(y_raw, memory_format=torch.contiguous_format)
        if pooled is not None:
            if residual is None and hip.instnorm_pool_ok(y_raw, a, pooled) and not os.environ.get("MSSEG_NO_NORM_POOL"):
                hip.instnorm_act_pool_fwd(y_raw, stats, self.gamma, self.beta, a, pooled, self.slope, self.eps)
                return a, stats
            hip.instnorm_act_fwd(y_raw, stats, self.gamma, self.beta, a, self.slope, self.eps, residual)
            hip.maxpool2_fwd(a, pooled)
            return a, stats
        hip.instnorm_act_fwd(y_raw, stats, self.gamma, self.beta, a, self.slope, self.eps, residual)
        return a, stats

    def pool_bwd_reduce(self, y_raw, stats, skip_grad, pooled_grad):
        if (os.environ.get("MSSEG_NO_NORM_POOL") or os.environ.get("MSSEG_NO_POOL_BWD_FUSE")
                or not hip.instnorm_pool_ok(y_raw, skip_grad, pooled_grad)):
            return None
        da = torch.empty(y_raw.shape, dtype=y_raw.dtype, device=y_raw.device)
        dg, db, acc = _norm_grad_bufs(self)
        red = hip.instnorm_act_poolbwd_reduce(y_raw, stats, self.gamma, self.beta, skip_grad, pooled_grad, da, self.slope,
                                              self.eps, dg, db, acc)
        return da, red

    def bwd(self, y_raw, stats, a, da, want_dres=False, red=None):
        if red is APPLIED:
            if want_dres:
                raise RuntimeError("a residual unit cannot take an already-applied gradient")
            return da
        dy = torch.empty(y_raw.shape, dtype=y_raw.dtype, device=y_raw.device)
        dres = torch.empty(y_raw.shape, dtype=y_raw.dtype, device=y_raw.device) if want_dres else None
        a_in = a if want_dres else None
        if red is not None:
            hip.instnorm_act_bwd_apply(y_raw, stats, self.gamma, a_in, da, red, dy, self.slope, self.eps, dres, self.beta)
            return (dy, dres) if want_dres else dy
        dg = db = None
        acc = False
        if self.gamma is not None and self.gamma.requires_grad:
            dg, acc = _grad_buf(self.gamma)
            db, acc2 = _grad_buf(self.beta)
            assert acc == acc2
        hip.instnorm_act_bwd(y_raw, stats, self.gamma, a_in, da, dy, self.slope, self.eps, dres, dg, db, acc, self.beta)
        return (dy, dres) if want_dres else dy


class ConvNormAct:

    def __init__(self, conv: Conv3, norm: InstNormAct):
        self.conv, self.norm = conv, norm

    def fwd(self, x, out=None, pooled=None):
        cv, nm = self.conv, self.norm
        if (INFERENCE_FORWARD and pooled is None and cv.cin == 1 and x.dtype == torch.bfloat16 and x.shape[0] <= 8
                and (cv.cout % 32 == 0 or cv.cout % 48 == 0) and cv.cout <= 256 and not os.environ.get("MSSEG_NO_STEM")
                and not os.environ.get("MSSEG_NO_STEM_TWICE")):
            wp = cv.cache.get(cv.w, x.dtype, "g", lambda: hip.pack_conv_gather(cv.w.detach(), x.dtype))
            stats = torch.empty(x.shape[0], cv.cout, 2, dtype=torch.float32, device=x.device)
            hip.conv3d_stem(x, wp, cv.b, None, cv.cout, stats)
            a = out if out is not None else _empty_like_vol(x, cv.cout)
            hip.conv3d_stem_norm(x, wp, cv.b, stats, nm.gamma, nm.beta, nm.eps, nm.slope, a, cv.cout)
            return a, (x, None, stats, a)
        if (not cv._gather(x.dtype) and hip.conv3d_k3_small_ok(x, cv.cin, cv.cout)
                and (pooled is None or hip.instnorm_pool_ok(x, x, pooled))):
            wp = cv.cache.get(cv.w, x.dtype, "fs", lambda: hip.pack_conv_k3(cv.w.detach(), x.dtype, cb=32))
            part, ng = hip.conv3d_k3_small_partials(x, wp, cv.cin, cv.cout)
            y = _empty_like_vol(x, cv.cout)
            a = out if out is not None else _empty_like_vol(x, cv.cout)
            stats = torch.empty(x.shape[0], cv.cout, 2, dtype=torch.float32, device=x.device)
            hip.conv3d_k3_small_fwd_finish(part, ng, cv.b, nm.gamma, nm.beta, nm.eps, nm.slope, y, a, pooled, stats)
            return a, (x, y, stats, a)
        y, stats = self.conv.fwd(x, want_stats=True)
        a, stats = self.norm.fwd(y, out, stats=stats, pooled=pooled)
        return a, (x, y, stats, a)

    def bwd(self, saved, da, need_dx=True, red=None, next_saved=None, next_cna=None):
        x, y, stats, a = saved
        dy = self.norm.bwd(y, stats, a, da, red=red)
        if next_cna is not None and need_dx:
            nx, ny, nstats, na = next_saved
            return self.conv.bwd(x, dy, True, bias_grad_is_zero=True, next_norm=(next_cna.norm, ny, nstats, na))
        return self.conv.bwd(x, dy, need_dx, bias_grad_is_zero=True)


def maxpool_fwd(x):
    N, D, H, W, C = x.shape
    y = torch.empty(N, D // 2, H // 2, W // 2, C, dtype=x.dtype, device=x.device)
    return hip.maxpool2_fwd(x, y)


class ResBlock:

    def __init__(self, conv1_w, conv2_w, conv3_w=None, slope=0.01):
        self.c1, self.c2 = Conv3(conv1_w, None), Conv3(conv2_w, None)
        self.c3 = Conv1(conv3_w, None) if conv3_w is not None else None
        self.n1, self.n2 = InstNormAct(None, None, slope), InstNormAct(None, None, slope)
        self.n3 = InstNormAct(None, None, 1.0) if conv3_w is not None else None

    @staticmethod
    def _small_unit(conv, nrm, x, residual=None, out=None):
        wp = conv.cache.get(conv.w, x.dtype, "fs", lambda: hip.pack_conv_k3(conv.w.detach(), x.dtype, cb=32))
        part, ng = hip.conv3d_k3_small_partials(x, wp, conv.cin, conv.cout)
        y = _empty_like_vol(x, conv.cout)
        a = out if out is not None else _empty_like_vol(x, conv.cout)
        stats = torch.empty(x.shape[0], conv.cout, 2, dtype=torch.float32, device=x.device)
        hip.conv3d_k3_small_fwd_finish(part, ng, conv.b, nrm.gamma, nrm.beta, nrm.eps, nrm.slope, y, a, None, stats, residual)
        return a, y, stats

    def fwd(self, x, out=None):
        small = (not self.c1._gather(x.dtype) and hip.conv3d_k3_small_ok(x, self.c1.cin, self.c1.cout)
                 and hip.conv3d_k3_small_ok(x, self.c2.cin, self.c2.cout))
        if small:
            a1, y1, s1 = self._small_unit(self.c1, self.n1, x)
        else:
            y1, s1 = self.c1.fwd(x, want_stats=True)
            a1, s1 = self.n1.fwd(y1, stats=s1)
        if self.c3 is not None:
            y3, s3 = self.c3.fwd(x, want_stats=True)
            r, s3 = self.n3.fwd(y3, stats=s3)
        else:
            y3 = s3 = None
            r = x
        if small:
            o, y2, s2 = self._small_unit(self.c2, self.n2, a1, residual=r, out=out)
        else:
            y2, s2 = self.c2.fwd(a1, want_stats=True)
            o, s2 = self.n2.fwd(y2, out, residual=r, stats=s2)
        return o, (x, y1, s1, a1, y2, s2, y3, s3, r, o)

    def bwd(self, saved, do, need_dx=True):
        x, y1, s1, a1, y2, s2, y3, s3, r, o = saved
        dy2, dres = self.n2.bwd(y2, s2, o, do, want_dres=True)
        da1, red1 = self.c2.bwd(a1, dy2, True, next_norm=(self.n1, y1, s1, a1))
        dy1 = self.n1.bwd(y1, s1, a1, da1, red=red1)
        if need_dx and self.c1.dgrad_accumulate_ok(dy1):
            if self.c3 is not None:
                dy3 = self.n3.bwd(y3, s3, r, dres)
                dx3 = self.c3.bwd(x, dy3, True)
            else:
                dx3 = dres
            return self.c1.bwd(x, dy1, True, dx_out=dx3, accumulate_dx=True)
        dx = self.c1.bwd(x, dy1, need_dx)
        if self.c3 is not None:
            dy3 = self.n3.bwd(y3, s3, r, dres)
            dx3 = self.c3.bwd(x, dy3, need_dx)
        else:
            dx3 = dres
        if not need_dx:
            return None
        return hip.add(dx, dx3, dx)


class UpBlock:

    def __init__(self, transp_w, conv1_w, conv2_w, conv3_w, slope=0.01):
        self.up = Deconv2(transp_w, None)
        self.res = ResBlock(conv1_w, conv2_w, conv3_w, slope)
        self.cout = transp_w.shape[1]

    def alloc_cat(self, x):
        N, D, H, W, _ = x.shape
        k = self.up.k
        return torch.empty(N, k * D, k * H, k * W, 2 * self.cout, dtype=x.dtype, device=x.device)

    def fwd(self, x, cat):
        self.up.fwd(x, cat[..., :self.cout])
        o, s = self.res.fwd(cat)
        return o, (x, s)

    def bwd(self, saved, do):
        x, s = saved
        dcat = self.res.bwd(s, do, True)
        dx = self.up.bwd(x, dcat[..., :self.cout], True)
        return dx, dcat[..., self.cout:]


def _merge_batch(t):
    N, D, H, W, C = t.shape
    return t.view(1, N * D, H, W, C)


class BatchNormAct:

    def __init__(self, bn: torch.nn.BatchNorm3d, slope: float = 0.0, group=None):
        self.bn = bn
        self.inner = InstNormAct(bn.weight, bn.bias, slope, bn.eps)
        self.group = group

    def _all_reduce(self, t):
        import torch.distributed as dist
        dist.all_reduce(t, group=None if self.group is True else self.group)

    def _synced(self):
        import torch.distributed as dist
        if self.group is None or not (dist.is_available() and dist.is_initialized()):
            return False
        return dist.get_world_size(None if self.group is True else self.group) > 1

    def fwd(self, y_raw, out=None, stats=None):
        bn = self.bn
        N, D, H, W, C = y_raw.shape
        cnt = N * D * H * W
        if bn.training or not bn.track_running_stats:
            s = stats.sum(0, keepdim=True) if stats is not None else hip.channel_stats(_merge_batch(y_raw))
            total = cnt
            if self._synced():
                pack = torch.cat([s.reshape(-1), torch.full((1,), float(cnt), device=s.device)])
                self._all_reduce(pack)
                total = float(pack[-1])
                s = (pack[:-1] * (cnt / total)).reshape(1, C, 2)
            if bn.training and bn.track_running_stats:
                with torch.no_grad():
                    bn.num_batches_tracked.add_(1)
                    mean = s[0, :, 0] / cnt
                    var = (s[0, :, 1] / cnt - mean * mean).clamp_(min=0) * (total / max(total - 1, 1))
                    if bn.momentum is None:
                        m = 1.0 / bn.num_batches_tracked.to(torch.float32)
                        bn.running_mean.add_((mean - bn.running_mean) * m)
                        bn.running_var.add_((var - bn.running_var) * m)
                    else:
                        bn.running_mean.mul_(1 - bn.momentum).add_(mean, alpha=bn.momentum)
                        bn.running_var.mul_(1 - bn.momentum).add_(var, alpha=bn.momentum)
        else:
            eps = self.inner.eps
            rstd = torch.rsqrt(bn.running_var.double() + eps)
            g = self.inner.gamma.detach().double() if self.inner.gamma is not None else torch.ones_like(rstd)
            bta = self.inner.beta.detach().double() if self.inner.beta is not None else torch.zeros_like(rstd)
            scale = g * rstd
            shift = bta - bn.running_mean.double() * scale
            s = torch.zeros(1, C, 2, dtype=torch.float32, device=y_raw.device)
            s[0, :, 1] = (1.0 - eps) * cnt
            a = out if out is not None else torch.empty(y_raw.shape, dtype=y_raw.dtype, device=y_raw.device)
            hip.instnorm_act_fwd(_merge_batch(y_raw), s, scale.float().contiguous(), shift.float().contiguous(),
                                 _merge_batch(a), self.inner.slope, eps, None)
            return a, s
# ... 39 lines not shown
```

Measured before the change: 542.1 vol/s.

## Fuse InstanceNorm+LeakyReLU backward apply into k3 and stem weight-gradient kernels

The InstanceNorm/activation backward elementwise apply now runs inside the conv weight-gradient kernels. Per-channel coefficients are precomputed into LDS, and dy is computed on the fly from da and yraw while loading tiles. The kblk==0 workgroups write dy out for the dgrad pass. This removes a separate full-volume read/write pass over da and yraw. The cost is extra global loads of yraw in the wgrad kernel, a check that the tile schedule covers each voxel once, and the wgrad must now run inline rather than on the side stream.

```diff
diff --git a/include/msseg.h b/include/msseg.h
--- a/include/msseg.h
+++ b/include/msseg.h
@@ -126,6 +126,17 @@
 int msseg_conv3d_k3_wgrad(const void* x, long long ldx, const void* dy, long long lddy, float* dw,
                           int N, int D, int H, int W, int Cin, int Cout, int accumulate,
                           void* workspace, size_t workspace_bytes, int dtype, msseg_stream_t stream);
+int msseg_conv3d_k3_wgrad_inbwd_ok(int N, int D, int H, int W, int Cin, int Cout, int dtype);
+int msseg_conv3d_k3_wgrad_inbwd(const void* x, long long ldx, const void* da, long long ldda, const void* yraw,
+                                long long ldyraw, const float* stats, const float* gamma, const float* beta,
+                                const float* red, void* dy, long long lddy, float* dw, int N, int D, int H, int W, int Cin,
+                                int Cout, float eps, float slope, int accumulate, void* workspace, size_t workspace_bytes,
+                                int dtype, msseg_stream_t stream);
+int msseg_conv3d_stem_wgrad_inbwd_ok(int N, int Cout, int dtype);
+int msseg_conv3d_stem_wgrad_inbwd(const void* x, long long ldx, const void* da, long long ldda, const void* yraw,
+                                  long long ldyraw, const float* stats, const float* gamma, const float* beta,
+                                  const float* red, float* dw, int N, int D, int H, int W, int Cout, float eps, float slope,
+                                  int accumulate, void* workspace, size_t workspace_bytes, int dtype, msseg_stream_t stream);
 int msseg_conv3d_k1_wgrad(const void* x, long long ldx, const void* dy, long long lddy, float* dw,
                           long long NV, int Cin, int Cout, int accumulate,
                           void* workspace, size_t workspace_bytes, int dtype, msseg_stream_t stream);
diff --git a/medicalsemseg_amd/csrc/conv3d_k3_wgrad_pp.hip b/medicalsemseg_amd/csrc/conv3d_k3_wgrad_pp.hip
--- a/medicalsemseg_amd/csrc/conv3d_k3_wgrad_pp.hip
+++ b/medicalsemseg_amd/csrc/conv3d_k3_wgrad_pp.hip
@@ -1,4 +1,5 @@
 #include "k3pp.h"
+#include "instnorm_bwd.h"
 
 #include <stdlib.h>
 
@@ -47,7 +48,7 @@
 
 constexpr int ks_row(int ks) { return ((ks / TH) * PH + ks % TH) * PWP; }
 
-template <int TIMING>
+template <int TIMING, int FUSED>
 __global__ __launch_bounds__(NTHREADS, 1) void k3wg_pp_kernel(const K3WgParams p) {
     extern __shared__ __attribute__((aligned(256))) unsigned char smem[];
     const int tid = threadIdx.x, lane = tid & 63;
@@ -100,6 +101,48 @@
     }
     const bool p_cok = mblk * 32 + lchunk * 8 < p.M, q_cok = kblk * 32 + lchunk * 8 < p.K;
     const bool chunks_full = (mblk + 1) * 32 <= p.M && (kblk + 1) * 32 <= p.K;
+    const unsigned char* yg = (const unsigned char*)p.in_yraw + mblk * 64;
+    unsigned char* og = (unsigned char*)p.in_dy + mblk * 64;
+    const float* ctab = (const float*)(smem + 2 * GRP_BYTES) + lchunk * 8;
+    const bool emit = kblk == 0;
+    auto load_p_fused = [&](const TileCo& tc, const long long pvox, auto&& issue_q) {
+        const unsigned char* ab = pg + pvox * p.ldp * 2;
+        const unsigned char* yb = yg + pvox * p.ldp * 2;
+        unsigned char* ob = og + pvox * p.ldp * 2;
+        u32x4_t dav[NIP_W], yv[NIP_W];
+        bool inb[NIP_W];
+#pragma unroll
+        for (int j = 0; j < NIP_W; ++j) {
+            inb[j] = tc.d0 + j < p.D && tc.h0 + wq < p.H && tc.w0 + lrow < p.W;
+            const unsigned off = inb[j] ? p_off[j] : (unsigned)(lchunk * 16);
+            dav[j] = *(const u32x4_t*)(ab + off);
+            yv[j] = *(const u32x4_t*)(yb + off);
+        }
+        __builtin_amdgcn_sched_barrier(0);
+        issue_q();
+        __builtin_amdgcn_sched_barrier(0);
+        const float* ct = ctab + tc.n * (INBWD_NCOEF * 32);
+#pragma unroll
+        for (int e2 = 0; e2 < 4; ++e2) {
+            __builtin_amdgcn_sched_barrier(0);
+            float k[INBWD_NCOEF][2];
+#pragma unroll
+            for (int q = 0; q < INBWD_NCOEF; ++q) {
+                const float2 v = *(const float2*)(ct + q * 32 + 2 * e2);
+                k[q][0] = v.x; k[q][1] = v.y;
+            }
+#pragma unroll
+            for (int j = 0; j < NIP_W; ++j) dav[j][e2] = inbwd_apply_pair_bf16(dav[j][e2], yv[j][e2], p.in_slope, k);
+        }
+#pragma unroll
+        for (int j = 0; j < NIP_W; ++j) {
+            u32x4_t o = dav[j];
+            if (!inb[j]) o = u32x4_t{0u, 0u, 0u, 0u};
+            *(u32x4_t*)(ldsP + (wq + 4 * j) * 1024 + lane * 16) = o;
+            if (emit && inb[j]) *(u32x4_t*)(ob + p_off[j]) = o;
+        }
+        asm volatile("s_waitcnt lgkmcnt(0)" ::: "memory");
+    };
     auto load_tile = [&](const TileCo& tc) {
         const int dB = tc.d0 - 1, hB = tc.h0 - 1, wB = tc.w0 - 1;
         const long long qvox = (((long long)tc.n * p.D + dB) * p.H + hB) * p.W + wB;
@@ -107,25 +150,35 @@
         const unsigned char* qb = qg + qvox * p.ldq * 2;
         const unsigned char* pb = pg + pvox * p.ldp * 2;
         const bool interior = chunks_full && dB >= 0 && dB + PD <= p.D && hB >= 0 && hB + PH <= p.H && wB >= 0 && wB + PW <= p.W;
+        const unsigned char* zsrc = (const unsigned char*)&g_wg_zero_chunk;
+        auto issue_q = [&]() {
+            if (interior) {
+#pragma unroll
+                for (int j = 0; j < NIQ_W; ++j) {
+                    if (q_off[j] != SKIP) glds16(qb + q_off[j], ldsQ + (wq + 4 * j) * 1024);
+                }
+            } else {
+#pragma unroll
+                for (int j = 0; j < NIQ_W; ++j) {
+                    const int it = wq + 4 * j;
+                    const int hv = it * 16 + lrow;
+                    const int hd = hv / (PH * PWP), rem = hv - hd * (PH * PWP), hh = rem / PWP, hw = rem - hh * PWP;
+                    const bool inb = q_cok && (unsigned)(dB + hd) < (unsigned)p.D && (unsigned)(hB + hh) < (unsigned)p.H &&
+                                     (unsigned)(wB + hw) < (unsigned)p.W;
+                    const unsigned char* src = inb ? qb + q_off[j] : zsrc;
+                    if (q_off[j] != SKIP) glds16(src, ldsQ + it * 1024);
+                }
+            }
+        };
+        if constexpr (FUSED) {
+            load_p_fused(tc, pvox, issue_q);
+            return;
+        }
+        issue_q();
         if (interior) {
-#pragma unroll
-            for (int j = 0; j < NIQ_W; ++j) {
-                if (q_off[j] != SKIP) glds16(qb + q_off[j], ldsQ + (wq + 4 * j) * 1024);
-            }
 #pragma unroll
             for (int j = 0; j < NIP_W; ++j) glds16(pb + p_off[j], ldsP + (wq + 4 * j) * 1024);
         } else {
-            const unsigned char* zsrc = (const unsigned char*)&g_wg_zero_chunk;
-#pragma unroll
-            for (int j = 0; j < NIQ_W; ++j) {
-                const int it = wq + 4 * j;
-                const int hv = it * 16 + lrow;
-                const int hd = hv / (PH * PWP), rem = hv - hd * (PH * PWP), hh = rem / PWP, hw = rem - hh * PWP;
-                const bool inb = q_cok && (unsigned)(dB + hd) < (unsigned)p.D && (unsigned)(hB + hh) < (unsigned)p.H &&
-                                 (unsigned)(wB + hw) < (unsigned)p.W;
-                const unsigned char* src = inb ? qb + q_off[j] : zsrc;
-                if (q_off[j] != SKIP) glds16(src, ldsQ + it * 1024);
-            }
 #pragma unroll
             for (int j = 0; j < NIP_W; ++j) {
                 const int tv = (wq + 4 * j) * 16 + lrow;
@@ -187,6 +240,16 @@
         }
     };
 
+    if constexpr (FUSED) {
+        float* tab = (float*)(smem + 2 * GRP_BYTES);
+        for (int i = tid; i < p.N * 32; i += NTHREADS) {
+            const int n = i >> 5, c = i & 31;
+            const InBwdCoef k = inbwd_coef(p.in_stats, p.in_gamma, p.in_beta, p.in_red, n, p.M, mblk * 32 + c, p.in_S, p.in_eps);
+            float* t = tab + n * (INBWD_NCOEF * 32) + c;
+            t[0] = k.mean; t[32] = k.rstd; t[64] = k.sc; t[96] = k.sh; t[128] = k.k0; t[160] = k.k1;
+        }
+        __syncthreads();
+    }
     if (grp == 0 && n_my > 0) load_tile(tile_of(0));
     asm volatile("s_waitcnt vmcnt(0)" ::: "memory");
     __syncthreads();
@@ -268,18 +331,52 @@
     return gx;
 }
 
+bool msseg_k3wg_pp_inbwd_shape_ok(int N, int M, int K) { return N >= 1 && N <= K3WG_INBWD_NMAX && M % 32 == 0 && K % 32 == 0; }
+
+static bool schedule_covers_once(int ntiles, int gx) {
+    long long seen = 0;
+    for (int bx = 0; bx < gx; ++bx) {
+        int t_first, t_step, t_end;
+        if ((gx & 7) == 0) {
+            const int chunk = (ntiles + 7) >> 3, xcd = bx & 7;
+            t_first = xcd * chunk + (bx >> 3); t_step = gx >> 3; t_end = ntiles < (xcd + 1) * chunk ? ntiles : (xcd + 1) * chunk;
+            if (t_step > chunk && (bx >> 3) >= chunk) continue;
+        } else {
+            t_first = bx; t_step = gx; t_end = ntiles;
+        }
+        if (t_first < t_end) seen += (t_end - t_first + t_step - 1) / t_step;
+    }
+    return seen == ntiles;
+}
+
 int msseg_k3wg_pp_launch(const K3WgParams& p, int gx, hipStream_t stream) {
     static const bool timing = getenv("MSSEG_K3PP_TIMING") != nullptr;
     static const bool noload = getenv("MSSEG_K3PP_NOLOAD") != nullptr;
     K3WgParams pl = p;
     pl.dbg_noload = noload ? 1 : 0;
+    const int pairs = ceil_div(p.M, 32) * ceil_div(p.K, 32);
+    if (p.in_yraw != nullptr) {
+        if (!msseg_k3wg_pp_inbwd_shape_ok(p.N, p.M, p.K) || !p.in_dy || !p.in_stats || !p.in_red ||
+            (((uintptr_t)p.in_yraw | (uintptr_t)p.in_dy) & 15))
+            MSSEG_FAIL(MSSEG_EINVAL, "conv3d_k3_wgrad_pp: shape or operands not eligible for the InstanceNorm-backward form");
+        const int ntiles = p.N * ceil_div(p.D, TD) * ceil_div(p.H, TH) * ceil_div(p.W, TW);
+        if (!schedule_covers_once(ntiles, gx))
+            MSSEG_FAIL(MSSEG_EINVAL, "conv3d_k3_wgrad_pp: tile schedule (%d tiles, %d workgroups) does not cover dy once", ntiles, gx);
+        const int ldsf = 2 * GRP_BYTES + p.N * INBWD_NCOEF * 32 * 4;
+        static msseg_lds_attr_once fattr;
+        if (!fattr.ensure((const void*)k3wg_pp_kernel<0, 1>, 2 * GRP_BYTES + K3WG_INBWD_NMAX * INBWD_NCOEF * 32 * 4))
+            MSSEG_FAIL(MSSEG_ELAUNCH, "conv3d_k3_wgrad_pp: cannot set dynamic LDS size");
+        MSSEG_KTIMED("k3wg_pp_inbwd_kernel", stream,
+                     hipLaunchKernelGGL((k3wg_pp_kernel<0, 1>), dim3(gx, pairs, 1), dim3(NTHREADS), ldsf, stream, pl));
+        MSSEG_CHECK_LAUNCH("conv3d_k3_wgrad_pp_inbwd");
+        return MSSEG_OK;
+    }
     const int lds = 2 * GRP_BYTES;
     static msseg_lds_attr_once attr[2];
-    if (!attr[0].ensure((const void*)k3wg_pp_kernel<0>, lds) || !attr[1].ensure((const void*)k3wg_pp_kernel<1>, lds))
+    if (!attr[0].ensure((const void*)k3wg_pp_kernel<0, 0>, lds) || !attr[1].ensure((const void*)k3wg_pp_kernel<1, 0>, lds))
         MSSEG_FAIL(MSSEG_ELAUNCH, "conv3d_k3_wgrad_pp: cannot set dynamic LDS size %d", lds);
-    const int pairs = ceil_div(p.M, 32) * ceil_div(p.K, 32);
-    if (timing) hipLaunchKernelGGL(k3wg_pp_kernel<1>, dim3(gx, pairs, 1), dim3(NTHREADS), lds, stream, pl);
-    else MSSEG_KTIMED("k3wg_pp_kernel", stream, hipLaunchKernelGGL(k3wg_pp_kernel<0>, dim3(gx, pairs, 1), dim3(NTHREADS), lds, stream, pl));
+    if (timing) hipLaunchKernelGGL((k3wg_pp_kernel<1, 0>), dim3(gx, pairs, 1), dim3(NTHREADS), lds, stream, pl);
+    else MSSEG_KTIMED("k3wg_pp_kernel", stream, hipLaunchKernelGGL((k3wg_pp_kernel<0, 0>), dim3(gx, pairs, 1), dim3(NTHREADS), lds, stream, pl));
     MSSEG_CHECK_LAUNCH("conv3d_k3_wgrad_pp");
     return MSSEG_OK;
 }
diff --git a/medicalsemseg_amd/csrc/elementwise.hip b/medicalsemseg_amd/csrc/elementwise.hip
--- a/medicalsemseg_amd/csrc/elementwise.hip
+++ b/medicalsemseg_amd/csrc/elementwise.hip
@@ -1,4 +1,5 @@
 #include "common.h"
+#include "instnorm_bwd.h"
 
 #include <stdarg.h>
 #include <string.h>
@@ -349,15 +350,6 @@
     float* ws; unsigned int* counter; float* dgamma; float* dbeta; int accumulate;
 };
 
-MSSEG_DEVFN void mean_rstd(const float* stats, int n, int C, int c, long long S, float eps, float& mean, float& rstd) {
-    const float inv = 1.0f / (float)S;
-    const float s = stats[((long long)n * C + c) * 2 + 0], s2 = stats[((long long)n * C + c) * 2 + 1];
-    mean = s * inv;
-    float var = s2 * inv - mean * mean;
-    var = var > 0.f ? var : 0.f;
-    rstd = rsqrtf(var + eps);
-}
-
 template <typename T, bool VEC, int MODE>
 __global__ __launch_bounds__(MODE == 1 ? RED_THREADS : 256) void instnorm_kernel(const NormParams p) {
     constexpr int W = VEC ? DT<T>::EPC : 1;
@@ -390,8 +382,8 @@
             sh[e] = (p.beta ? p.beta[c] : 0.f) - mean[e] * sc[e];
             a0[e] = a1[e] = 0.f;
             if constexpr (MODE == 2) {
-                k0[e] = p.red[((long long)n * p.C + c) * 2 + 0] * invS;
-                k1[e] = p.red[((long long)n * p.C + c) * 2 + 1] * invS;
+                const InBwdCoef k = inbwd_coef(p.stats, p.gamma, p.beta, p.red, n, p.C, c, p.S, p.eps);
+                mean[e] = k.mean; rstd[e] = k.rstd; sc[e] = k.sc; sh[e] = k.sh; k0[e] = k.k0; k1[e] = k.k1;
             }
         }
         if (act && rl < p.rows_par) {
@@ -442,21 +434,22 @@
                             for (int e = 0; e < W; ++e) yv[e] = c.v[e];
                         } else {
 #pragma unroll
-                            for (int e = 0; e < W; ++e) yv[e] = xv[e] * sc[e] + sh[e];
+                            for (int e = 0; e < W; ++e) yv[e] = inbwd_preact(xv[e], sc[e], sh[e]);
                         }
                     } else {
                         dv[0] = DT<T>::ld(dyn + r * p.lddy + gg);
-                        yv[0] = (yn != nullptr) ? DT<T>::ld(yn + r * p.ldy + gg) : xv[0] * sc[0] + sh[0];
+                        yv[0] = (yn != nullptr) ? DT<T>::ld(yn + r * p.ldy + gg) : inbwd_preact(xv[0], sc[0], sh[0]);
                     }
 #pragma unroll
                     for (int e = 0; e < W; ++e) {
-                        const float dz = yv[e] > 0.f ? dv[e] : dv[e] * p.slope;
-                        const float xh = (xv[e] - mean[e]) * rstd[e];
                         if constexpr (MODE == 1) {
+                            const float dz = yv[e] > 0.f ? dv[e] : dv[e] * p.slope;
+                            const float xh = (xv[e] - mean[e]) * rstd[e];
                             a0[e] += dz;
                             a1[e] += dz * xh;
                         } else {
-                            o[e] = sc[e] * (dz - k0[e] - xh * k1[e]);
+                            float dz;
+                            o[e] = inbwd_apply(xv[e], yv[e], dv[e], p.slope, mean[e], rstd[e], sc[e], k0[e], k1[e], dz);
                             dv[e] = dz;
                         }
                     }
diff --git a/medicalsemseg_amd/csrc/igemm_wgrad.hip b/medicalsemseg_amd/csrc/igemm_wgrad.hip
--- a/medicalsemseg_amd/csrc/igemm_wgrad.hip
+++ b/medicalsemseg_amd/csrc/igemm_wgrad.hip
@@ -583,6 +583,99 @@
                               : launch_wg_k3<bf16_t>(p, rp, workspace, workspace_bytes, (hipStream_t)stream);
 }
 
+static bool wgrad_inbwd_on() {
+    static const bool off = getenv("MSSEG_NO_WGRAD_INBWD") != nullptr;
+    return !off;
+}
+
+static bool k3_inbwd_kernel_ok(int N, int D, int H, int W, int Cin, int Cout, int dtype) {
+    if (!wgrad_inbwd_on() || dtype != MSSEG_BF16 || !msseg_k3wg_pp_inbwd_shape_ok(N, Cout, Cin)) return false;
+    static const int pp_min_dim = getenv("MSSEG_K3WG_MINDIM") ? atoi(getenv("MSSEG_K3WG_MINDIM")) : 8;
+    const int mnd = D < H ? (D < W ? D : W) : (H < W ? H : W);
+    return mnd >= pp_min_dim && msseg_conv3d_k3_wgrad_kernel(N, D, H, W, Cin, Cout, dtype) == 3;
+}
+
+int msseg_conv3d_k3_wgrad_inbwd_ok(int N, int D, int H, int W, int Cin, int Cout, int dtype) {
+    if (!k3_inbwd_kernel_ok(N, D, H, W, Cin, Cout, dtype) || Cin > 64) return 0;
+    K3WgParams pp{};
+    pp.N = N; pp.D = D; pp.H = H; pp.W = W; pp.M = Cout; pp.K = Cin;
+    const long long tiles = (long long)N * ceil_div(D, 4) * ceil_div(H, 4) * ceil_div(W, 16);
+    return tiles >= 3LL * msseg_k3wg_pp_grid(pp) ? 1 : 0;
+}
+
+int msseg_conv3d_k3_wgrad_inbwd(const void* x, long long ldx, const void* da, long long ldda, const void* yraw,
+                                long long ldyraw, const float* stats, const float* gamma, const float* beta,
+                                const float* red, void* dy, long long lddy, float* dw, int N, int D, int H, int W, int Cin,
+                                int Cout, float eps, float slope, int accumulate, void* workspace, size_t workspace_bytes,
+                                int dtype, msseg_stream_t stream) {
+    int rc = wg_check(x, ldx, da, ldda, dw, workspace, dtype);
+    if (rc) return rc;
+    if (!yraw || !stats || !red || !dy) MSSEG_FAIL(MSSEG_EINVAL, "conv3d_k3_wgrad_inbwd: null pointer");
+    K3WgParams pe{};
+    pe.pten = da; pe.ldp = ldda; pe.qten = x; pe.ldq = ldx;
+    pe.N = N; pe.D = D; pe.H = H; pe.W = W; pe.M = Cout; pe.K = Cin; pe.kblks = ceil_div(Cin, 32);
+    if (!k3_inbwd_kernel_ok(N, D, H, W, Cin, Cout, dtype) || ldyraw != ldda || lddy != ldda ||
+        (((uintptr_t)yraw | (uintptr_t)dy) & 15) || !msseg_k3wg_pp_eligible(pe)) {
+        rc = msseg_instnorm_act_bwd_apply(yraw, ldyraw, stats, gamma, beta, nullptr, 0, da, ldda, red, dy, lddy, nullptr, 0, N,
+                                          (long long)D * H * W, Cout, eps, slope, dtype, stream);
+        if (rc) return rc;
+        return msseg_conv3d_k3_wgrad(x, ldx, dy, lddy, dw, N, D, H, W, Cin, Cout, accumulate, workspace, workspace_bytes, dtype,
+                                     stream);
+    }
+    K3WgParams pp{};
+    pp.pten = da; pp.ldp = ldda; pp.qten = x; pp.ldq = ldx;
+    pp.N = N; pp.D = D; pp.H = H; pp.W = W; pp.M = Cout; pp.K = Cin; pp.kblks = Cin / 32;
+    pp.in_yraw = yraw; pp.in_dy = dy; pp.in_stats = stats; pp.in_gamma = gamma; pp.in_beta = beta; pp.in_red = red;
+    pp.in_eps = eps; pp.in_slope = slope; pp.in_S = (long long)D * H * W;
+    if (!msseg_k3wg_pp_eligible(pp)) MSSEG_FAIL(MSSEG_EINVAL, "conv3d_k3_wgrad_inbwd: operands not eligible (alignment / strides)");
+    const int pairs = (Cout / 32) * (Cin / 32);
+    int gx = msseg_k3wg_pp_grid(pp);
+    const long long fit = (long long)(workspace_bytes / ((size_t)27 * 32 * 32 * 4 * pairs));
+    if (fit < 8) MSSEG_FAIL(MSSEG_EWORKSPACE, "conv3d_k3_wgrad_inbwd: workspace %zu B too small", workspace_bytes);
+    if (gx > fit) gx = (int)(fit & ~7LL);
+    pp.slabs = (float*)workspace;
+    rc = msseg_k3wg_pp_launch(pp, gx, (hipStream_t)stream);
+    if (rc) return rc;
+    ReduceParams rp{};
+    rp.dw = dw; rp.M = Cout; rp.M0 = Cout; rp.T = 27; rp.K = Cin; rp.K0 = Cin;
+    rp.s_m1 = 0; rp.s_m0 = (long long)Cin * 27; rp.s_t = 1; rp.s_k1 = 0; rp.s_k0 = 27; rp.accumulate = accumulate;
+    rp.slabs = pp.slabs; rp.mblks = Cout / 32; rp.kblks = Cin / 32; rp.nslots = gx; rp.cbw = 32;
+    return launch_reduce(rp, (hipStream_t)stream);
+}
+
+int msseg_conv3d_stem_wgrad_inbwd_ok(int N, int Cout, int dtype) {
+    static const bool no_stem = getenv("MSSEG_NO_STEM") != nullptr;
+    return wgrad_inbwd_on() && !no_stem && dtype == MSSEG_BF16 && N >= 1 && N <= K3WG_INBWD_NMAX && Cout % 32 == 0 && Cout <= 256;
+}
+
+int msseg_conv3d_stem_wgrad_inbwd(const void* x, long long ldx, const void* da, long long ldda, const void* yraw,
+                                  long long ldyraw, const float* stats, const float* gamma, const float* beta,
+                                  const float* red, float* dw, int N, int D, int H, int W, int Cout, float eps, float slope,
+                                  int accumulate, void* workspace, size_t workspace_bytes, int dtype, msseg_stream_t stream) {
+    if (!x || !da || !yraw || !stats || !red || !dw || !workspace) MSSEG_FAIL(MSSEG_EINVAL, "conv3d_stem_wgrad_inbwd: null pointer");
+    if (!msseg_conv3d_stem_wgrad_inbwd_ok(N, Cout, dtype) || D < 1 || H < 1 || W < 1 || (long long)N * D * H * W > 0x7fffffffLL)
+        MSSEG_FAIL(MSSEG_EINVAL, "conv3d_stem_wgrad_inbwd: shape not eligible (see msseg_conv3d_stem_wgrad_inbwd_ok)");
+    if (((uintptr_t)da & 15) || ((uintptr_t)yraw & 15) || (ldda % 8) || ldyraw != ldda || ldx < 1)
+        MSSEG_FAIL(MSSEG_EINVAL, "conv3d_stem_wgrad_inbwd: da / yraw need 16-byte aligned rows of one voxel stride");
+    if ((long long)(TD_STEM_ROWS + 1) * H * W * ldda * 2 >= 0x7fffffffLL) MSSEG_FAIL(MSSEG_EINVAL, "conv3d_stem_wgrad_inbwd: plane too large");
+    StemWgParams sp{};
+    sp.x = x; sp.ldx = ldx; sp.dy = da; sp.lddy = ldda; sp.N = N; sp.D = D; sp.H = H; sp.W = W; sp.M = Cout;
+    sp.in_yraw = yraw; sp.in_stats = stats; sp.in_gamma = gamma; sp.in_beta = beta; sp.in_red = red;
+    sp.in_eps = eps; sp.in_slope = slope; sp.in_S = (long long)D * H * W;
+    int gx = msseg_stem_wgrad_grid(sp);
+    const long long fit = (long long)(workspace_bytes / ((size_t)4096 * (Cout / 32)));
+    if (fit < 8) MSSEG_FAIL(MSSEG_EWORKSPACE, "conv3d_stem_wgrad_inbwd: workspace %zu B too small", workspace_bytes);
+    if (gx > fit) gx = (int)(fit & ~7LL);
+    sp.slabs = (float*)workspace;
+    int rc = msseg_stem_wgrad_launch(sp, gx, (hipStream_t)stream);
+    if (rc) return rc;
+    ReduceParams rq{};
+    rq.dw = dw; rq.M = Cout; rq.M0 = Cout; rq.T = 1; rq.K = 27; rq.K0 = 1;
+    rq.s_m0 = 27; rq.s_k1 = 1; rq.s_k0 = 27; rq.accumulate = accumulate;
+    rq.slabs = sp.slabs; rq.mblks = Cout / 32; rq.kblks = 1; rq.nslots = gx; rq.cbw = 32;
+    return launch_reduce(rq, (hipStream_t)stream);
+}
+
 int msseg_conv3d_k1_wgrad(const void* x, long long ldx, const void* dy, long long lddy, float* dw, long long NV, int Cin,
                           int Cout, int accumulate, void* workspace, size_t workspace_bytes, int dtype,
                           msseg_stream_t stream) {
diff --git a/medicalsemseg_amd/csrc/instnorm_bwd.h b/medicalsemseg_amd/csrc/instnorm_bwd.h
--- /dev/null
+++ b/medicalsemseg_amd/csrc/instnorm_bwd.h
@@ -0,0 +1,52 @@
+#pragma once
+#include "common.h"
+
+MSSEG_DEVFN void mean_rstd(const float* stats, int n, int C, int c, long long S, float eps, float& mean, float& rstd) {
+    const float inv = 1.0f / (float)S;
+    const float s = stats[((long long)n * C + c) * 2 + 0], s2 = stats[((long long)n * C + c) * 2 + 1];
+    mean = s * inv;
+    float var = s2 * inv - mean * mean;
+    var = var > 0.f ? var : 0.f;
+    rstd = rsqrtf(var + eps);
+}
+
+struct InBwdCoef {
+    float mean, rstd, sc, sh, k0, k1;
+};
+constexpr int INBWD_NCOEF = 6;
+
+MSSEG_DEVFN InBwdCoef inbwd_coef(const float* stats, const float* gamma, const float* beta, const float* red, int n, int C,
+                                 int c, long long S, float eps) {
+    InBwdCoef k;
+    const float invS = 1.0f / (float)S;
+    mean_rstd(stats, n, C, c, S, eps, k.mean, k.rstd);
+    const float ga = gamma ? gamma[c] : 1.f;
+    k.sc = k.rstd * ga;
+    k.sh = (beta ? beta[c] : 0.f) - k.mean * k.sc;
+    k.k0 = red[((long long)n * C + c) * 2 + 0] * invS;
+    k.k1 = red[((long long)n * C + c) * 2 + 1] * invS;
+    return k;
+}
+
+MSSEG_DEVFN float inbwd_preact(float yraw, float sc, float sh) { return __builtin_fmaf(yraw, sc, sh); }
+
+MSSEG_DEVFN float inbwd_apply(float yraw, float pre, float da, float slope, float mean, float rstd, float sc, float k0,
+                              float k1, float& dz) {
+    dz = pre > 0.f ? da : da * slope;
+    const float xh = (yraw - mean) * rstd;
+    return sc * __builtin_fmaf(-xh, k1, dz - k0);
+}
+
+typedef __attribute__((ext_vector_type(2))) __bf16 inbwd_bf16x2_t;
+MSSEG_DEVFN uint32_t inbwd_apply_pair_bf16(uint32_t da, uint32_t yraw, float slope, const float (&k)[INBWD_NCOEF][2]) {
+    const inbwd_bf16x2_t d = __builtin_bit_cast(inbwd_bf16x2_t, da), y = __builtin_bit_cast(inbwd_bf16x2_t, yraw);
+    inbwd_bf16x2_t o;
+#pragma unroll
+    for (int e = 0; e < 2; ++e) {
+        const float yv = (float)y[e];
+        float dz;
+        o[e] = (bf16_t)inbwd_apply(yv, inbwd_preact(yv, k[2][e], k[3][e]), (float)d[e], slope, k[0][e], k[1][e], k[2][e],
+                                   k[4][e], k[5][e], dz);
+    }
+    return __builtin_bit_cast(uint32_t, o);
+}
diff --git a/medicalsemseg_amd/csrc/k3pp.h b/medicalsemseg_amd/csrc/k3pp.h
--- a/medicalsemseg_amd/csrc/k3pp.h
+++ b/medicalsemseg_amd/csrc/k3pp.h
@@ -43,7 +43,12 @@
     float* slabs;
     int N, D, H, W, M, K, kblks;
     int dbg_noload;
+    const void* in_yraw; void* in_dy;
+    const float* in_stats; const float* in_gamma; const float* in_beta; const float* in_red;
+    float in_eps, in_slope; long long in_S;
 };
+constexpr int K3WG_INBWD_NMAX = 16;
+bool msseg_k3wg_pp_inbwd_shape_ok(int N, int M, int K);
 bool msseg_k3wg_pp_eligible(const K3WgParams& p);
 int msseg_k3wg_pp_grid(const K3WgParams& p);
 int msseg_k3wg_pp_launch(const K3WgParams& p, int gx, hipStream_t stream);
@@ -63,9 +68,13 @@
     const void* dy; long long lddy;
     float* slabs;
     int N, D, H, W, M;
+    const void* in_yraw;
+    const float* in_stats; const float* in_gamma; const float* in_beta; const float* in_red;
+    float in_eps, in_slope; long long in_S;
 };
 bool msseg_stem_eligible(int dtype, int Cin, int Cout, int k, int s, int pd, long long ldx, long long ldy, const void* y);
 int msseg_stem_fwd_launch(const StemParams& p, hipStream_t stream);
+constexpr int TD_STEM_ROWS = 4;
 int msseg_stem_wgrad_grid(const StemWgParams& p);
 int msseg_stem_wgrad_launch(const StemWgParams& p, int gx, hipStream_t stream);
 
diff --git a/medicalsemseg_amd/csrc/stem_conv.hip b/medicalsemseg_amd/csrc/stem_conv.hip
--- a/medicalsemseg_amd/csrc/stem_conv.hip
+++ b/medicalsemseg_amd/csrc/stem_conv.hip
@@ -1,4 +1,5 @@
 #include "k3pp.h"
+#include "instnorm_bwd.h"
 
 namespace {
 
@@ -229,6 +230,7 @@
     return __builtin_amdgcn_ds_read_tr16_b64_v4bf16((__attribute__((address_space(3))) bf16x4_t*)p);
 }
 
+template <int FUSED>
 __global__ __launch_bounds__(W_THREADS) void stem_wgrad_kernel(const StemWgParams p) {
     extern __shared__ __attribute__((aligned(256))) unsigned char smem[];
     constexpr int BUF_BYTES = P_BYTES + 3 * XS_ELEMS * 2 + 64;
@@ -249,6 +251,11 @@
         p_off[j] = (unsigned)((((long long)td * p.H + th) * p.W + tw) * p.lddy * 2 + (lane & 3) * 16);
     }
     unsigned short st[3];
+    const unsigned char* yg = (const unsigned char*)p.in_yraw + mblk * 64;
+    const float* ctab = (const float*)(smem + 2 * BUF_BYTES) + (lane & 3) * 8;
+    u32x4_t dav[4], yv[4];
+    bool inb[4];
+    int tile_n = 0;
     auto load_tile = [&](const TileCo& tc, int buf) {
         unsigned char* base = smem + buf * BUF_BYTES;
         const long long pvox = (((long long)tc.n * p.D + tc.d0) * p.H + tc.h0) * p.W + tc.w0;
@@ -256,8 +263,19 @@
         const bool full = tc.d0 + TD <= p.D && tc.h0 + TH <= p.H && tc.w0 + TW <= p.W;
         const unsigned char* zsrc = (const unsigned char*)&g_stem_zero_chunk;
         const bool ch_ok = mblk * 32 + (lane & 3) * 8 < p.M;
-#pragma unroll
-        for (int j = 0; j < 4; ++j) {
+        if constexpr (FUSED) {
+            const unsigned char* yb = yg + pvox * p.lddy * 2;
+            tile_n = tc.n;
+#pragma unroll
+            for (int j = 0; j < 4; ++j) {
+                inb[j] = tc.d0 + j < p.D && tc.h0 + wave < p.H && tc.w0 + (lane >> 2) < p.W;
+                const unsigned off = inb[j] ? p_off[j] : (unsigned)((lane & 3) * 16);
+                dav[j] = *(const u32x4_t*)(pb + off);
+                yv[j] = *(const u32x4_t*)(yb + off);
+            }
+        }
+#pragma unroll
+        for (int j = 0; j < (FUSED ? 0 : 4); ++j) {
             const unsigned char* src = pb + p_off[j];
             if (!ch_ok) src = zsrc;
             if (!full) {
@@ -277,6 +295,26 @@
         }
     };
     auto commit_x = [&](int buf) {
+        if constexpr (FUSED) {
+            const float* ct = ctab + tile_n * (INBWD_NCOEF * 32);
+#pragma unroll
+            for (int e2 = 0; e2 < 4; ++e2) {
+                float k[INBWD_NCOEF][2];
+#pragma unroll
+                for (int q = 0; q < INBWD_NCOEF; ++q) {
+                    const float2 v = *(const float2*)(ct + q * 32 + 2 * e2);
+                    k[q][0] = v.x; k[q][1] = v.y;
+                }
+#pragma unroll
+                for (int j = 0; j < 4; ++j) dav[j][e2] = inbwd_apply_pair_bf16(dav[j][e2], yv[j][e2], p.in_slope, k);
+            }
+#pragma unroll
+            for (int j = 0; j < 4; ++j) {
+                u32x4_t o = dav[j];
+                if (!inb[j]) o = u32x4_t{0u, 0u, 0u, 0u};
+                *(u32x4_t*)(smem + buf * BUF_BYTES + (wave + 4 * j) * 1024 + lane * 16) = o;
+            }
+        }
         unsigned short* xs = (unsigned short*)(smem + buf * BUF_BYTES + P_BYTES);
 #pragma unroll
         for (int it = 0; it < 3; ++it) {
@@ -305,6 +343,16 @@
 #pragma unroll
     for (int e = 0; e < 16; ++e) acc[e] = 0.f;
 
+    if constexpr (FUSED) {
+        float* tab = (float*)(smem + 2 * BUF_BYTES);
+        for (int i = tid; i < p.N * 32; i += W_THREADS) {
+            const int n = i >> 5, c = i & 31;
+            const InBwdCoef k = inbwd_coef(p.in_stats, p.in_gamma, p.in_beta, p.in_red, n, p.M, mblk * 32 + c, p.in_S, p.in_eps);
+            float* t = tab + n * (INBWD_NCOEF * 32) + c;
+            t[0] = k.mean; t[32] = k.rstd; t[64] = k.sc; t[96] = k.sh; t[128] = k.k0; t[160] = k.k1;
+        }
+        __syncthreads();
+    }
     if (sc.n_my > 0) {
         load_tile(sc.tile(0), 0);
         commit_x(0);
@@ -386,9 +434,21 @@
 
 int msseg_stem_wgrad_launch(const StemWgParams& p, int gx, hipStream_t stream) {
     const int lds = 2 * (P_BYTES + 3 * XS_ELEMS * 2 + 64);
+    if (p.in_yraw != nullptr) {
+        if (p.N < 1 || p.N > K3WG_INBWD_NMAX || p.M % 32 || !p.in_stats || !p.in_red || ((uintptr_t)p.in_yraw & 15))
+            MSSEG_FAIL(MSSEG_EINVAL, "stem_wgrad: shape or operands not eligible for the InstanceNorm-backward form");
+        const int ldsf = lds + p.N * INBWD_NCOEF * 32 * 4;
+        static msseg_lds_attr_once fattr;
+        if (!fattr.ensure((const void*)stem_wgrad_kernel<1>, lds + K3WG_INBWD_NMAX * INBWD_NCOEF * 32 * 4))
+            MSSEG_FAIL(MSSEG_ELAUNCH, "stem_wgrad: cannot set dynamic LDS size");
+        MSSEG_KTIMED("stem_wgrad_inbwd_kernel", stream,
+                     hipLaunchKernelGGL(stem_wgrad_kernel<1>, dim3(gx, p.M / 32), dim3(W_THREADS), ldsf, stream, p));
+        MSSEG_CHECK_LAUNCH("stem_wgrad_inbwd");
+        return MSSEG_OK;
+    }
     static msseg_lds_attr_once attr;
-    if (!attr.ensure((const void*)stem_wgrad_kernel, lds)) MSSEG_FAIL(MSSEG_ELAUNCH, "stem_wgrad: cannot set dynamic LDS size %d", lds);
-    hipLaunchKernelGGL(stem_wgrad_kernel, dim3(gx, ceil_div(p.M, 32)), dim3(W_THREADS), lds, stream, p);
+    if (!attr.ensure((const void*)stem_wgrad_kernel<0>, lds)) MSSEG_FAIL(MSSEG_ELAUNCH, "stem_wgrad: cannot set dynamic LDS size %d", lds);
+    hipLaunchKernelGGL(stem_wgrad_kernel<0>, dim3(gx, ceil_div(p.M, 32)), dim3(W_THREADS), lds, stream, p);
     MSSEG_CHECK_LAUNCH("stem_wgrad");
     return MSSEG_OK;
 }
diff --git a/medicalsemseg_amd/hip.py b/medicalsemseg_amd/hip.py
--- a/medicalsemseg_amd/hip.py
+++ b/medicalsemseg_amd/hip.py
@@ -96,6 +96,12 @@
     "msseg_wgrad_workspace_bytes": ([_i, _i, _i], _sz),
     "msseg_conv3d_k3_wgrad_kernel": ([_i, _i, _i, _i, _i, _i, _i], _i),
     "msseg_conv3d_k3_wgrad": ([_vp, _ll, _vp, _ll, _vp, _i, _i, _i, _i, _i, _i, _i, _vp, _sz, _i, _vp], _i),
+    "msseg_conv3d_k3_wgrad_inbwd_ok": ([_i, _i, _i, _i, _i, _i, _i], _i),
+    "msseg_conv3d_k3_wgrad_inbwd": ([_vp, _ll, _vp, _ll, _vp, _ll, _vp, _vp, _vp, _vp, _vp, _ll, _vp, _i, _i, _i, _i, _i, _i,
+                                     _f, _f, _i, _vp, _sz, _i, _vp], _i),
+    "msseg_conv3d_stem_wgrad_inbwd_ok": ([_i, _i, _i], _i),
+    "msseg_conv3d_stem_wgrad_inbwd": ([_vp, _ll, _vp, _ll, _vp, _ll, _vp, _vp, _vp, _vp, _vp, _i, _i, _i, _i, _i, _f, _f,
+                                       _i, _vp, _sz, _i, _vp], _i),
     "msseg_conv3d_k1_wgrad": ([_vp, _ll, _vp, _ll, _vp, _ll, _i, _i, _i, _vp, _sz, _i, _vp], _i),
     "msseg_conv3d_gather_wgrad": ([_vp, _ll, _vp, _ll, _vp, _i, _i, _i, _i, _i, _i, _i, _i, _i, _i, _vp, _sz, _i, _vp], _i),
     "msseg_deconv_k2s2_wgrad": ([_vp, _ll, _vp, _ll, _vp, _i, _i, _i, _i, _i, _i, _i, _vp, _sz, _i, _vp], _i),
@@ -763,6 +769,46 @@
     TIMER.launch(key, 2.0 * nv * 27 * cin * cout, nv * (cin + cout) * x.element_size() + 27 * cin * cout * 4, go)
 
 
+def conv3d_k3_wgrad_inbwd_ok(x, da, yraw, cin, cout) -> bool:
+    if not (x.is_cuda and x.dim() == 5 and x.dtype == da.dtype == yraw.dtype == torch.bfloat16):
+        return False
+    if ld(da) != ld(yraw) or ld(da) != cout or (_p(da) | _p(yraw) | _p(x)) % 16 or ld(x) % 8:
+        return False
+    return bool(lib().msseg_conv3d_k3_wgrad_inbwd_ok(*x.shape[:4], cin, cout, BF16))
+
+
+def conv3d_k3_wgrad_inbwd(x, da, yraw, stats, gamma, beta, red, dy, dw, cin, cout, slope, eps=1e-5, accumulate=False):
+    _need_gpu(x, da, yraw, dy, dw)
+    N, D, H, W = x.shape[:4]
+    ws = _wg_ws(cout, 27, cin, x.device)
+    nv = N * D * H * W
+    TIMER.launch("conv3d_k3_wgrad_inbwd", 2.0 * nv * 27 * cin * cout,
+                 nv * (cin + 3 * cout) * x.element_size() + 27 * cin * cout * 4,
+                 lambda: _ck(lib().msseg_conv3d_k3_wgrad_inbwd(
+                     _p(x), ld(x), _p(da), ld(da), _p(yraw), ld(yraw), _p(stats), _p(gamma), _p(beta), _p(red), _p(dy), ld(dy),
+                     _p(dw), N, D, H, W, cin, cout, eps, slope, int(accumulate), _p(ws), ws.numel(), dt(x), _stream()),
+                     "conv3d_k3_wgrad_inbwd"))
+
+
+def conv3d_stem_wgrad_inbwd_ok(x, da, yraw, cout) -> bool:
+    if not (x.is_cuda and x.dim() == 5 and x.shape[-1] == 1 and x.dtype == da.dtype == yraw.dtype == torch.bfloat16):
+        return False
+    if ld(da) != ld(yraw) or ld(da) % 8 or (_p(da) | _p(yraw)) % 16:
+        return False
+    return bool(lib().msseg_conv3d_stem_wgrad_inbwd_ok(x.shape[0], cout, BF16))
+
+
+def conv3d_stem_wgrad_inbwd(x, da, yraw, stats, gamma, beta, red, dw, cout, slope, eps=1e-5, accumulate=False):
+    _need_gpu(x, da, yraw, dw)
+    N, D, H, W = x.shape[:4]
+    ws = _wg_ws(cout, 1, 27, x.device)
+    TIMER.launch("conv3d_stem_wgrad_inbwd", 0.0, _nbytes(x, da, yraw),
+                 lambda: _ck(lib().msseg_conv3d_stem_wgrad_inbwd(
+                     _p(x), ld(x), _p(da), ld(da), _p(yraw), ld(yraw), _p(stats), _p(gamma), _p(beta), _p(red), _p(dw),
+                     N, D, H, W, cout, eps, slope, int(accumulate), _p(ws), ws.numel(), dt(x), _stream()),
+                     "conv3d_stem_wgrad_inbwd"))
+
+
 def conv3d_k1_wgrad(x, dy, dw, cin, cout, accumulate=False):
     _need_gpu(x, dy, dw)
     nv = x.numel() // x.shape[-1]
diff --git a/medicalsemseg_amd/layers.py b/medicalsemseg_amd/layers.py
--- a/medicalsemseg_amd/layers.py
+++ b/medicalsemseg_amd/layers.py
@@ -288,9 +288,29 @@
         vol = tuple(dy.shape[:4])
         return hip.lib().msseg_conv3d_k3_kernel(*vol, self.cout, self.cin, hip.BF16) == (4 if self.cout == 48 else 3)
 
-    def bwd(self, x, dy, need_dx=True, dx_out=None, bias_grad_is_zero=False, next_norm=None, accumulate_dx=False):
+    def wgrad_inbwd_ok(self, x, da, yraw, need_dx) -> bool:
+        if not self.w.requires_grad or (WGRAD_SIDE.active is not None and WGRAD_SIDE.mode != WGRAD_SIDE.INLINE):
+            return False
+        if self._gather(x.dtype):
+            return not need_dx and self.cin == 1 and hip.conv3d_stem_wgrad_inbwd_ok(x, da, yraw, self.cout)
+        return hip.conv3d_k3_wgrad_inbwd_ok(x, da, yraw, self.cin, self.cout)
+
+    def bwd(self, x, dy, need_dx=True, dx_out=None, bias_grad_is_zero=False, next_norm=None, accumulate_dx=False,
+            unit_bwd=None):
         dtype = x.dtype
-        if self.w.requires_grad:
+        if unit_bwd is not None:
+            assert bias_grad_is_zero
+            nrm, yraw, stats, red = unit_bwd
+            da = dy
+            g, acc = _grad_buf(self.w)
+            if self._gather(dtype):
+                dy = None
+                hip.conv3d_stem_wgrad_inbwd(x, da, yraw, stats, nrm.gamma, nrm.beta, red, g, self.cout, nrm.slope, nrm.eps, acc)
+            else:
+                dy = torch.empty(yraw.shape, dtype=yraw.dtype, device=yraw.device)
+                hip.conv3d_k3_wgrad_inbwd(x, da, yraw, stats, nrm.gamma, nrm.beta, red, dy, g, self.cin, self.cout,
+                                          nrm.slope, nrm.eps, acc)
+        elif self.w.requires_grad:
             g, acc = _grad_buf(self.w)
             if self._gather(dtype):
                 WGRAD_SIDE.run(lambda: hip.conv3d_gather_wgrad(x, dy, g, self.cin, self.cout, 3, 1, 1, acc), x, dy)
@@ -609,11 +629,15 @@
 
     def bwd(self, saved, da, need_dx=True, red=None, next_saved=None, next_cna=None):
         x, y, stats, a = saved
-        dy = self.norm.bwd(y, stats, a, da, red=red)
+        unit = None
+        if red is not None and red is not APPLIED and self.conv.wgrad_inbwd_ok(x, da, y, need_dx):
+            unit, dy = (self.norm, y, stats, red), da
+        else:
+            dy = self.norm.bwd(y, stats, a, da, red=red)
         if next_cna is not None and need_dx:
             nx, ny, nstats, na = next_saved
-            return self.conv.bwd(x, dy, True, bias_grad_is_zero=True, next_norm=(next_cna.norm, ny, nstats, na))
-        return self.conv.bwd(x, dy, need_dx, bias_grad_is_zero=True)
+            return self.conv.bwd(x, dy, True, bias_grad_is_zero=True, next_norm=(next_cna.norm, ny, nstats, na), unit_bwd=unit)
+        return self.conv.bwd(x, dy, need_dx, bias_grad_is_zero=True, unit_bwd=unit)
 
 
 def maxpool_fwd(x):
```

Result: slower. 500.8 vol/s (-7.6%).
